# ActiveVisionLab/NeFeS

Hardware: AMD Instinct MI355X
Metric: rays/s (fwd+bwd) at 640x480x(64+128) samples, 8x256 MLP (higher is better)
Workload: dtype f32; 1 GPU; BASELINE configs[1]: 7-Scenes-stairs geometry, 64+128 samples, 8x256 MLP + 16-ch feature head; 640x480, random seed-0 weights, fwd + bwd to the 3x4 pose; parallelism=rows/1

## Files before the change

### include/nefes_hip.h

```cpp
#ifndef NEFES_HIP_H
#define NEFES_HIP_H
#include <stddef.h>
#include <stdint.h>

#ifdef __cplusplus
extern "C" {
#endif

#define NEFES_ABI_VERSION 16

#define NEFES_E_BADARG (-1)
#define NEFES_E_UNSUPPORTED (-2)
#define NEFES_E_BADBLOB (-3)

typedef struct NefesNetDesc {
    int32_t width;
    int32_t feat_dim;
    int32_t has_transient;
    int32_t xyz_encoding;
} NefesNetDesc;
#define NEFES_XYZ_FREQ10 0
#define NEFES_XYZ_EXTERNAL32 1

typedef struct NefesStreamInfo {
    uint64_t slab_off;
    uint32_t n_slabs;
    uint32_t bias_floats;
    uint64_t bias_off;
    uint32_t scale_off;
    uint32_t scale_count;
} NefesStreamInfo;

typedef struct NefesBlobInfo {
    uint64_t total_bytes;
    NefesStreamInfo stream[13];
} NefesBlobInfo;

#define NEFES_COMP_TRANSIENT 1u
#define NEFES_COMP_STATIC_ONLY 2u
#define NEFES_COMP_SIGMA_ONLY 4u
#define NEFES_COMP_WHITE_BKGD 8u
#define NEFES_COMP_FEAT_WEIGHTS_ONLY 16u

#define NEFES_FIELD_SIGMA 0
#define NEFES_FIELD_STATIC 1
#define NEFES_FIELD_FULL 2

int nefes_version(void);

int nefes_blob_info(const NefesNetDesc* desc, NefesBlobInfo* info);
size_t nefes_stream_slab_bytes(const NefesNetDesc* desc, int stream);
int nefes_pack_weights(const NefesNetDesc* desc, const float* const* tensors, int n_tensors, void* blob,
// ... 211 lines not shown
```

### nefes_amd/csrc/field_bwd_h3.hip

```cpp
#if defined(NEFES_TU_PART) && NEFES_TU_PART >= 2 && NEFES_TU_PART % 2 == 0
#define NEFES_SLAB_KIB 16
#define NEFES_ASM_READS_ACC
#define NEFES_ACC_VGPR_FORM
#define NEFES_FENCE_TILES
#else
#define NEFES_SLAB_KIB 32
#if !defined(NEFES_TU_PART) || NEFES_TU_PART == 0 || NEFES_TU_PART == 1 || NEFES_TU_PART == 5
#define H3B_WIDE
#define H3_ACC_READ_ASM
#define NEFES_ASM_READS_ACC
#define NEFES_FENCE_TILES
#define H3_WIDE_ENTRY_FENCE
#else
#define NEFES_H3_WIDE_MIN 99
#endif
#endif
#define NEFES_B_BATCH 2
#define NEFES_B_BATCH_NT8 4
#include "field_common.h"
#include "field_x6.h"
#include "field_h3.h"
#include "hashgrid.h"
#include "../../include/nefes_hip.h"
#define NEFES_XYZ_HASHGRID_FUSED 2
#ifndef H3B_WIDE_LAYERS
#define H3B_WIDE_LAYERS 0x1ff
#endif
#ifndef NEFES_H3B_WG128
#define NEFES_H3B_WG128 2
#endif
#define NEFES_H3B_WG_PER_CU(W) ((W) == 128 ? NEFES_H3B_WG128 : 1)
#define NEFES_H3B_SLOTS 2

struct FieldBwdH3Args {
    const char* stream;
    const int* tab;
    uint32_t n_slabs;
    const float* rays_o;
    const float* rays_d;
    const float* z;
// ... 17 lines not shown
};

template <class Inner>
struct StoringSplitH {
    Inner in;
    float* p;
    float inv;
    __device__ __forceinline__ void stage_a(PairRegs& s, int q, int pp) const {
        in.stage_a(s, q, pp);
        const int e = 8 * q + 2 * pp;
#ifndef NEFES_TRAIN_NO_STORES
        __builtin_nontemporal_store(s.x0 * inv, &p[(e >> 4) * 4096 + nefes_rho(0, e & 15) * 16]);
        __builtin_nontemporal_store(s.x1 * inv, &p[((e + 1) >> 4) * 4096 + nefes_rho(0, (e + 1) & 15) * 16]);
#endif
    }
    __device__ __forceinline__ void stage_b(PairRegs& s) const { in.stage_b(s); }
    template <bool NOP>
    __device__ __forceinline__ void stage_c(Split2& o, int pp, const PairRegs& s) const { in.template stage_c<NOP>(o, pp, s); }
    __device__ __forceinline__ void stage_c1(Split2& o, int pp, const PairRegs& s) const { in.stage_c1(o, pp, s); }
    template <bool NOP>
    __device__ __forceinline__ void stage_c2(Split2& o, int pp, const PairRegs& s) const { in.template stage_c2<NOP>(o, pp, s); }
};
template <bool ON, class Inner>
__device__ __forceinline__ auto wrap_store_h3(const Inner& in, float* p, float inv) {
    if constexpr (ON) return StoringSplitH<Inner>{in, p, inv};
    else return in;
}

template <typename T>
__device__ __forceinline__ T ld_stream(const T* p) {
    return __builtin_nontemporal_load(p);
}

template <int W, int KR16, int ENC, bool HAS_T = true, bool TRAIN = false, bool FH = false>
__global__ __launch_bounds__(256, NEFES_H3B_WG_PER_CU(W)) void field_bwd_h3_kernel(FieldBwdH3Args a) {
    constexpr int NTW = W / 32, NTH = W / 64, HS = W / 2, GS = W / 4;
    constexpr int MW = 8 * (W / 64) + 4 * (W / 128);
    constexpr int WT = (NTW + 1) / 2, WH = (NTH + 1) / 2;
    constexpr int MW_TRUNK = 8 * WT;
    constexpr int NTR = KR16 <= 2 ? 1 : 5;
    constexpr int WIDE_LAYERS = ENC == NEFES_XYZ_HASHGRID_FUSED ? 0 : H3B_WIDE_LAYERS;
    static_assert(KR16 == 2 || KR16 == 9, "head classes of layout.h (nefes_head_kr16 / nefes_head_ntr)");
    const int C3 = 3 + a.C;
    static_assert(MW % 4 == 0, "mask words are staged as 16-byte groups");
    extern __shared__ __attribute__((aligned(16))) char smem[];
    const int lane = threadIdx.x & 63;
    const int wave = __builtin_amdgcn_readfirstlane(threadIdx.x >> 6);
    const int j = lane & 31, h = lane >> 5;
    constexpr int SX = ENC == NEFES_XYZ_HASHGRID_FUSED ? 24 : 8;
    int* tab_i = (int*)(smem + NEFES_H3B_SLOTS * NEFES_SLAB_BYTES + (size_t)4 * (MW + SX) * 256);
    const float* tab_f = (const float*)tab_i;
    if (threadIdx.x < 2 * (HAS_T ? NEFES_H3B_N : NEFES_H3B_N_STATIC)) tab_i[threadIdx.x] = a.tab[threadIdx.x];
    HgGeom* hg_lds = (HgGeom*)(tab_i + 64);
    if constexpr (ENC == NEFES_XYZ_HASHGRID_FUSED) {
        if (threadIdx.x == 0) *hg_lds = a.hg;
    }
    auto wexp = [&](int seg) { return tab_i[nefes_h3_tab_exp(nefes_h3b_seg(HAS_T, seg))]; };
    auto rowb = [&](int seg) { return tab_f[nefes_h3_tab_bound(nefes_h3b_seg(HAS_T, seg))]; };
    StagedRing ring;
    ring.init(a.stream, a.n_slabs, smem, wave, lane);
    const char* ring_lane = smem + lane * 16;
    ring.prime(ring_lane);
    uint32_t* mlds = (uint32_t*)(smem + NEFES_H3B_SLOTS * NEFES_SLAB_BYTES) + wave * ((MW + SX) * 64) + lane * 4;
    auto MASKW = [&](int w) { return mlds[(w >> 2) * 256 + (w & 3)]; };
    float* stash = (float*)mlds;
    auto STASH = [&](int k) -> float& { return stash[((MW + k) >> 2) * 256 + ((MW + k) & 3)]; };

#pragma unroll 1
    for (int tile = blockIdx.x; tile < a.n_tiles; tile += gridDim.x) {
        const long long m_raw = (long long)tile * 128 + wave * 32 + j;
        const bool valid = m_raw < a.M;
        const long long m = valid ? m_raw : a.M - 1;
        const int ray = (int)(m / a.S);
        const int smp = (int)(m - (long long)ray * a.S);
        const size_t chan0 = (size_t)ray * a.R * a.S + smp;

        float in_o[3] = {0.f, 0.f, 0.f}, in_d[3] = {0.f, 0.f, 0.f}, in_z = 0.f, v[3];
        if constexpr (ENC == NEFES_XYZ_EXTERNAL32) {
        } else if (a.pts) {
#pragma unroll
            for (int c = 0; c < 3; ++c) in_o[c] = a.pts[m * 3 + c];
        } else {
            in_z = a.z[m];
#pragma unroll
            for (int c = 0; c < 3; ++c) { in_o[c] = a.rays_o[ray * 3 + c]; in_d[c] = a.rays_d[ray * 3 + c]; }
        }
#pragma unroll
        for (int c = 0; c < 3; ++c) v[c] = a.viewdirs[ray * 3 + c];
        const int cT = C3 + 1;
        float y_th[3] = {0.f, 0.f, 0.f}, g_th[3] = {0.f, 0.f, 0.f}, y_sg, g_sg, dr[8 * KR16];
        if constexpr (HAS_T) {
// ... 163 lines not shown
            load_dg(dgv);
            if constexpr (HAS_T) {
                load_bits(bh, MW_TRUNK + WH, WH);
                mma_run_h3<NTW + 1, GS / 8, 1, true>(ring, ring_lane, wrap_store_h3<TRAIN>(MaskedSplitH<NTH, WH, 0>{T3, bh, pow2i(tau - es3), mt}, gptr(NEFES_TB_T0), pow2i(-es3)), ZeroInit{}, XA);
            }
            load_bits(bh, MW_TRUNK, WH);
#ifdef NEFES_FH_VARIANT_VALU_UPDATE
            if constexpr (FH) {
#pragma unroll
                for (int e = 0; e < 16 * NTH; ++e) G2[e >> 4][e & 15] += dgv[e] * pow2i(es_g2);
                mma_run_h3<NTW + 1, GS / 8, 1, !HAS_T>(ring, ring_lane, MaskedSplitH<NTH, WH, 0>{G2, bh, pow2i(tau - es_g2), mg}, ZeroInit{}, XA);
            } else
#else
            if constexpr (FH)
                mma_run_h3<NTW + 1, GS / 8, 1, !HAS_T>(ring, ring_lane, MaskedAddSplitH<NTH, WH, 0, 16 * NTH>{G2, bh, pow2i(tau - es_g2), mg, dgv, pow2i(es_g2)}, ZeroInit{}, XA);
            else
#endif
            mma_run_h3<NTW + 1, GS / 8, 1, !HAS_T>(ring, ring_lane, wrap_store_h3<TRAIN>(MaskedSplitH<NTH, WH, 0>{G2, bh, pow2i(tau - es_g2), mg}, gptr(NEFES_TB_DIR), pow2i(-es_g2)), ZeroInit{}, XA);
            M = (HAS_T ? rowb(NEFES_H3B_T0) * (pair_max(mt) * pow2i(-es3)) : 0.f) + rowb(NEFES_H3B_DIR) * (pair_max(mg) * pow2i(-es_g2));
        }
        float gv[3];
        {
            float dDv[16], v3[3];
            const float inv = pow2i(-es_dt);
#pragma unroll
            for (int r = 0; r < 16; ++r) dDv[r] = XA[1][r] * inv;
#pragma unroll
            for (int c = 0; c < 3; ++c) v3[c] = STASH(3 + c);
            embed_slots_bwd<NEFES_N_FREQ_DIR>(gv, dDv, v3, h);
            if constexpr (ENC == NEFES_XYZ_HASHGRID_FUSED) {
#pragma unroll
                for (int c = 0; c < 3; ++c) STASH(3 + c) = gv[c];
            }
        }
        int es_b;
        {
            const int ew = wexp(NEFES_H3B_FINAL), tau = tau_of(M, ew);
            float mx = 0.f;
            es_b = tau + ew;
            mma_run_h3<NTW, W / 16, 2, true, 2, (WIDE_LAYERS & 1) != 0>(ring, ring_lane, wrap_store_h3<TRAIN>(IdentSplitH<NTW + 2, 2>{XA, pow2i(tau - es_dt), mx}, gptr(NEFES_TB_FINAL), pow2i(-es_dt)), ZeroInit{}, XB);
            const float dsig = STASH(6);
            float dsg[1];
            dsg[0] = dsig * pow2i(es_b);
#if defined(H3B_WIDE) && defined(H3_WIDE_ENTRY_FENCE)
            mma_run<NTW, 1, 2, false, ((WIDE_LAYERS >> 8) & 1) == 0 || (NTW < NEFES_H3_WIDE_MIN)>(ring, ring_lane, ArrayIn<1>{dsg}, ZeroInit{}, XB);
#else
            mma_run<NTW, 1, 2, false>(ring, ring_lane, ArrayIn<1>{dsg}, ZeroInit{}, XB);
#endif
            M = rowb(NEFES_H3B_FINAL) * (pair_max(mx) * pow2i(-es_dt)) + rowb(NEFES_H3B_SIG) * pair_max(fabsf(dsig));
        }
        int es_a = 0, es_e = 0;
#define NEFES_BWD_LAYER(L, SRC, DST, ES_SRC, ES_DST, NTILES, T0)                                                       \
        {                                                                                                           \
            load_bits(bt, ((L) - 1) * WT, WT);                                                                      \
            const int ew = wexp(NEFES_H3B_L8 + 8 - (L)), tau = tau_of(M, ew);                                       \
            float mx = 0.f;                                                                                         \
            ES_DST = tau + ew;                                                                                      \
            mma_run_h3<NTILES, W / 16, T0, true, 2, ((WIDE_LAYERS >> (L)) & 1) != 0>(ring, ring_lane, wrap_store_h3<TRAIN>(MaskedSplitH<NTW + 2, WT, 2>{SRC, bt, pow2i(tau - ES_SRC), mx}, gptr(NEFES_TB_L1 + (L) - 1), pow2i(-(ES_SRC))), ZeroInit{}, DST); \
            M = rowb(NEFES_H3B_L8 + 8 - (L)) * (pair_max(mx) * pow2i(-(ES_SRC)));                                   \
        }
        NEFES_BWD_LAYER(8, XB, XA, es_b, es_a, NTW, 2)
        NEFES_BWD_LAYER(7, XA, XB, es_a, es_b, NTW, 2)
        NEFES_BWD_LAYER(6, XB, XA, es_b, es_a, NTW, 2)
        NEFES_BWD_LAYER(5, XA, XB, es_a, es_b, NTW + 2, 0)
        es_e = es_b;
        float gx[3] = {0.f, 0.f, 0.f};
        float ge[ENC != NEFES_XYZ_FREQ10 ? NEFES_X_STEPS : 1];
        {
            const float inv = pow2i(-es_e);
            if constexpr (ENC != NEFES_XYZ_FREQ10) {
#pragma unroll
                for (int s_ = 0; s_ < NEFES_X_STEPS; ++s_) ge[s_] = XB[0][s_] * inv;
            } else {
                float dE[32], x3[3];
#pragma unroll
                for (int t = 0; t < 2; ++t)
#pragma unroll
                    for (int r = 0; r < 16; ++r) dE[t * 16 + r] = XB[t][r] * inv;
#pragma unroll
                for (int c = 0; c < 3; ++c) x3[c] = STASH(c);
                embed_slots_bwd<NEFES_N_FREQ_XYZ>(gx, dE, x3, h);
                ge[0] = 0.f;
            }
        }
        NEFES_BWD_LAYER(4, XB, XA, es_b, es_a, NTW, 2)
        NEFES_BWD_LAYER(3, XA, XB, es_a, es_b, NTW, 2)
        NEFES_BWD_LAYER(2, XB, XA, es_b, es_a, NTW, 2)
#undef NEFES_BWD_LAYER
        int es_1;
        {
            load_bits(bt, 0, WT);
            const int ew = wexp(NEFES_H3B_L1), tau = tau_of(M, ew);
            float mx = 0.f;
            es_1 = tau + ew;
            mma_run_h3<2, W / 16, 0, true>(ring, ring_lane, wrap_store_h3<TRAIN>(MaskedSplitH<NTW + 2, WT, 2>{XA, bt, pow2i(tau - es_a), mx}, gptr(NEFES_TB_L1), pow2i(-es_a)), ZeroInit{}, XB);
        }
        const float inv1 = pow2i(-es_1);
        if constexpr (ENC == NEFES_XYZ_HASHGRID_FUSED) {
            float x3[3];
#pragma unroll
            for (int s_ = 0; s_ < NEFES_X_STEPS; ++s_) STASH(8 + s_) = ge[s_] + XB[0][s_] * inv1;
#pragma unroll
            for (int c = 0; c < 3; ++c) x3[c] = STASH(c);
            asm volatile("" : "+v"(x3[0]), "+v"(x3[1]), "+v"(x3[2]));
            hg_encode_slots_bwd(gx, [&](int s_) { return STASH(8 + s_); }, x3, h, *hg_lds, a.hg_table);
#pragma unroll
            for (int c = 0; c < 3; ++c) gv[c] = STASH(3 + c);
        } else if constexpr (ENC == NEFES_XYZ_EXTERNAL32) {
#pragma unroll
            for (int s_ = 0; s_ < NEFES_X_STEPS; ++s_) ge[s_] += XB[0][s_] * inv1;
            if (valid) {
                float* gp = a.g_enc + m * 32 + h;
#pragma unroll
                for (int s_ = 0; s_ < NEFES_X_STEPS; ++s_) gp[2 * s_] = ge[s_];
            }
        } else {
            float dE[32], x3[3], g1[3];
#pragma unroll
            for (int t = 0; t < 2; ++t)
#pragma unroll
                for (int r = 0; r < 16; ++r) dE[t * 16 + r] = XB[t][r] * inv1;
#pragma unroll
            for (int c = 0; c < 3; ++c) x3[c] = STASH(c);
            embed_slots_bwd<NEFES_N_FREQ_XYZ>(g1, dE, x3, h);
#pragma unroll
            for (int c = 0; c < 3; ++c) gx[c] += g1[c];
        }
#pragma unroll
        for (int c = 0; c < 3; ++c) {
            gx[c] += __shfl_xor(gx[c], 32);
            gv[c] += __shfl_xor(gv[c], 32);
        }
        if (valid && h == 0) {
#pragma unroll
            for (int c = 0; c < 3; ++c) {
                if (ENC != NEFES_XYZ_EXTERNAL32) a.g_pts[m * 3 + c] = gx[c];
                a.g_vs[m * 3 + c] = gv[c];
            }
        }
    }
    ring.drain();
}

template <int W, int KR16, int ENC, bool HAS_T = true, bool TRAIN = false, bool FH = false>
static int launch_bwd_h3(const FieldBwdH3Args& a, hipStream_t st) {
    const size_t lds = (size_t)NEFES_H3B_SLOTS * NEFES_SLAB_BYTES
                       + (size_t)4 * (8 * (W / 64) + 4 * (W / 128) + (ENC == NEFES_XYZ_HASHGRID_FUSED ? 24 : 8)) * 256 + 256
                       + (ENC == NEFES_XYZ_HASHGRID_FUSED ? 512 : 0);
    static_assert(sizeof(HgGeom) <= 512 && 2 * NEFES_H3B_N <= 64, "scale table (256 bytes) + the level geometry's LDS slot");
    auto k = field_bwd_h3_kernel<W, KR16, ENC, HAS_T, TRAIN, FH>;
    hipError_t e = hipFuncSetAttribute((const void*)k, hipFuncAttributeMaxDynamicSharedMemorySize, (int)lds);
    if (e != hipSuccess) return (int)e;
    int dev = 0, cus = 256;
    (void)hipGetDevice(&dev);
    (void)hipDeviceGetAttribute(&cus, hipDeviceAttributeMultiprocessorCount, dev);
    const int slots = cus * NEFES_H3B_WG_PER_CU(W);
    int grid = a.n_tiles < slots ? a.n_tiles : slots;
    if (grid < 1) grid = 1;
    hipLaunchKernelGGL(k, dim3(grid), dim3(256), lds, st, a);
    return (int)hipGetLastError();
}

#ifndef NEFES_TU_PART
#define NEFES_TU_PART 0
#endif
enum { BWD_H3_EXT = 0, BWD_H3_FULL, BWD_H3_TRAIN_STATIC, BWD_H3_TRAIN_FULL, BWD_H3_STATIC, BWD_H3_HG, BWD_H3_FH, BWD_H3_TRAIN_EXT_STATIC,
       BWD_H3_TRAIN_EXT_FULL };
int nefes_bwd_h3_launch_part1(int which, const FieldBwdH3Args& a, hipStream_t st);
int nefes_bwd_h3_launch_part2(int which, const FieldBwdH3Args& a, hipStream_t st);
int nefes_bwd_h3_launch_part3(int which, const FieldBwdH3Args& a, hipStream_t st);
int nefes_bwd_h3_launch_part4(int which, const FieldBwdH3Args& a, hipStream_t st);
int nefes_bwd_h3_launch_part5(int which, const FieldBwdH3Args& a, hipStream_t st);
int nefes_bwd_h3_launch_part6(int which, const FieldBwdH3Args& a, hipStream_t st);
int nefes_bwd_h3_launch_part7(int which, const FieldBwdH3Args& a, hipStream_t st);
int nefes_bwd_h3_launch_part8(int which, const FieldBwdH3Args& a, hipStream_t st);

#if NEFES_TU_PART == 1
int nefes_bwd_h3_launch_part1(int which, const FieldBwdH3Args& a, hipStream_t st) {
    if (which == BWD_H3_EXT) return launch_bwd_h3<256, 2, NEFES_XYZ_EXTERNAL32>(a, st);
    if (which == BWD_H3_STATIC) return launch_bwd_h3<256, 2, NEFES_XYZ_FREQ10, false>(a, st);
    if (which == BWD_H3_HG) return launch_bwd_h3<256, 2, NEFES_XYZ_HASHGRID_FUSED>(a, st);
    return NEFES_E_UNSUPPORTED;
}
#elif NEFES_TU_PART == 2
int nefes_bwd_h3_launch_part2(int which, const FieldBwdH3Args& a, hipStream_t st) {
    if (which == BWD_H3_FULL) return launch_bwd_h3<128, 9, NEFES_XYZ_FREQ10>(a, st);
    if (which == BWD_H3_STATIC) return launch_bwd_h3<128, 9, NEFES_XYZ_FREQ10, false>(a, st);
    return NEFES_E_UNSUPPORTED;
}
#elif NEFES_TU_PART == 3
int nefes_bwd_h3_launch_part3(int which, const FieldBwdH3Args& a, hipStream_t st) {
    if (which == BWD_H3_TRAIN_STATIC) return launch_bwd_h3<256, 2, NEFES_XYZ_FREQ10, false, true>(a, st);
    if (which == BWD_H3_TRAIN_FULL) return launch_bwd_h3<256, 2, NEFES_XYZ_FREQ10, true, true>(a, st);
    if (which == BWD_H3_TRAIN_EXT_STATIC) return launch_bwd_h3<256, 2, NEFES_XYZ_EXTERNAL32, false, true>(a, st);
    if (which == BWD_H3_TRAIN_EXT_FULL) return launch_bwd_h3<256, 2, NEFES_XYZ_EXTERNAL32, true, true>(a, st);
    return NEFES_E_UNSUPPORTED;
}
#elif NEFES_TU_PART == 4
int nefes_bwd_h3_launch_part4(int which, const FieldBwdH3Args& a, hipStream_t st) {
    if (which == BWD_H3_TRAIN_STATIC) return launch_bwd_h3<128, 9, NEFES_XYZ_FREQ10, false, true>(a, st);
    if (which == BWD_H3_TRAIN_FULL) return launch_bwd_h3<128, 9, NEFES_XYZ_FREQ10, true, true>(a, st);
    return NEFES_E_UNSUPPORTED;
}
#elif NEFES_TU_PART == 5
int nefes_bwd_h3_launch_part5(int which, const FieldBwdH3Args& a, hipStream_t st) {
    if (which == BWD_H3_FULL) return launch_bwd_h3<256, 9, NEFES_XYZ_FREQ10>(a, st);
    if (which == BWD_H3_STATIC) return launch_bwd_h3<256, 9, NEFES_XYZ_FREQ10, false>(a, st);
    return NEFES_E_UNSUPPORTED;
}
#elif NEFES_TU_PART == 6
int nefes_bwd_h3_launch_part6(int which, const FieldBwdH3Args& a, hipStream_t st) {
    if (which == BWD_H3_FULL) return launch_bwd_h3<128, 2, NEFES_XYZ_FREQ10>(a, st);
    if (which == BWD_H3_STATIC) return launch_bwd_h3<128, 2, NEFES_XYZ_FREQ10, false>(a, st);
    if (which == BWD_H3_FH) return launch_bwd_h3<128, 2, NEFES_XYZ_FREQ10, true, false, true>(a, st);
    return NEFES_E_UNSUPPORTED;
}
#elif NEFES_TU_PART == 7
int nefes_bwd_h3_launch_part7(int which, const FieldBwdH3Args& a, hipStream_t st) {
    if (which == BWD_H3_TRAIN_STATIC) return launch_bwd_h3<256, 9, NEFES_XYZ_FREQ10, false, true>(a, st);
    if (which == BWD_H3_TRAIN_FULL) return launch_bwd_h3<256, 9, NEFES_XYZ_FREQ10, true, true>(a, st);
    return NEFES_E_UNSUPPORTED;
}
#elif NEFES_TU_PART == 8
int nefes_bwd_h3_launch_part8(int which, const FieldBwdH3Args& a, hipStream_t st) {
    if (which == BWD_H3_TRAIN_STATIC) return launch_bwd_h3<128, 2, NEFES_XYZ_FREQ10, false, true>(a, st);
    if (which == BWD_H3_TRAIN_FULL) return launch_bwd_h3<128, 2, NEFES_XYZ_FREQ10, true, true>(a, st);
    return NEFES_E_UNSUPPORTED;
}
#else

extern "C" int nefes_field_bwd_train_h3(const NefesNetDesc* desc, const void* packed, int mode, int N, int S, const float* rays_o,
                                        const float* rays_d, const float* z, const float* viewdirs, const float* raw_t,
                                        const float* g_raw_t, const uint32_t* masks, float* dacts, float* g_pts,
                                        float* g_viewdirs_s, void* stream) {
    if (!desc || !packed || !viewdirs || !raw_t || !g_raw_t || !masks || !dacts || !g_pts || !g_viewdirs_s || N <= 0 || S <= 0)
        return NEFES_E_BADARG;
    if (!(rays_o && rays_d && z)) return NEFES_E_BADARG;
    if (mode != NEFES_FIELD_STATIC && mode != NEFES_FIELD_FULL) return NEFES_E_BADARG;
    const bool full = mode == NEFES_FIELD_FULL;
    if (full && !desc->has_transient) return NEFES_E_UNSUPPORTED;
    const int cls = nefes_head_class(desc->feat_dim);
    if ((desc->width != 256 && desc->width != 128) || cls < 0 || desc->xyz_encoding != NEFES_XYZ_FREQ10) return NEFES_E_UNSUPPORTED;
    NefesBlobInfo info;
    int rc = nefes_blob_info(desc, &info);
    if (rc) return rc;
    const NefesStreamInfo& si = info.stream[full ? NEFES_STREAM_BWD_FULL_H3 : NEFES_STREAM_BWD_STATIC_H3];
    if (si.n_slabs == 0 || si.scale_count < 2 * (uint32_t)(full ? NEFES_H3B_N : NEFES_H3B_N_STATIC)) return NEFES_E_UNSUPPORTED;
    FieldBwdH3Args a;
    a.stream = (const char*)packed + si.slab_off;
    a.tab = (const int*)((const char*)packed + si.bias_off) + si.scale_off;
    a.n_slabs = si.n_slabs;
    a.rays_o = rays_o; a.rays_d = rays_d; a.z = z; a.pts = nullptr; a.viewdirs = viewdirs;
    a.raw_t = raw_t; a.g_raw_t = g_raw_t; a.masks = masks; a.g_pts = g_pts; a.g_enc = nullptr; a.g_vs = g_viewdirs_s;
    a.N = N; a.S = S; a.C = desc->feat_dim; a.R = 3 + a.C + (full ? 6 : 1);
    a.M = (long long)N * S;
    a.n_tiles = (int)((a.M + 127) / 128);
    a.dacts = dacts; a.gout = 0; a.hg_table = nullptr; a.g_gmap = nullptr;
    a.rows = nefes_train_row(desc->width, desc->feat_dim, NEFES_TB_END);
    const int which = full ? BWD_H3_TRAIN_FULL : BWD_H3_TRAIN_STATIC;
    hipStream_t st = (hipStream_t)stream;
    if (desc->width == 256) return cls == 0 ? nefes_bwd_h3_launch_part3(which, a, st) : nefes_bwd_h3_launch_part7(which, a, st);
    return cls == 1 ? nefes_bwd_h3_launch_part4(which, a, st) : nefes_bwd_h3_launch_part8(which, a, st);
}

extern "C" int nefes_field_bwd_train_h3_ext(const NefesNetDesc* desc, const void* packed, int mode, int N, int S, const float* viewdirs,
                                            const float* raw_t, const float* g_raw_t, const uint32_t* masks, float* dacts,
                                            float* g_xyz_enc, float* g_viewdirs_s, void* stream) {
    if (!desc || !packed || !viewdirs || !raw_t || !g_raw_t || !masks || !dacts || !g_xyz_enc || !g_viewdirs_s || N <= 0 || S <= 0)
        return NEFES_E_BADARG;
    if (mode != NEFES_FIELD_STATIC && mode != NEFES_FIELD_FULL) return NEFES_E_BADARG;
    const bool full = mode == NEFES_FIELD_FULL;
    if (full && !desc->has_transient) return NEFES_E_UNSUPPORTED;
    if (desc->width != 256 || nefes_head_class(desc->feat_dim) != 0 || desc->xyz_encoding != NEFES_XYZ_EXTERNAL32) return NEFES_E_UNSUPPORTED;
    NefesBlobInfo info;
    int rc = nefes_blob_info(desc, &info);
    if (rc) return rc;
    const NefesStreamInfo& si = info.stream[full ? NEFES_STREAM_BWD_FULL_H3 : NEFES_STREAM_BWD_STATIC_H3];
    if (si.n_slabs == 0 || si.scale_count < 2 * (uint32_t)(full ? NEFES_H3B_N : NEFES_H3B_N_STATIC)) return NEFES_E_UNSUPPORTED;
    FieldBwdH3Args a;
    a.stream = (const char*)packed + si.slab_off;
    a.tab = (const int*)((const char*)packed + si.bias_off) + si.scale_off;
    a.n_slabs = si.n_slabs;
    a.rays_o = nullptr; a.rays_d = nullptr; a.z = nullptr; a.pts = nullptr; a.viewdirs = viewdirs;
    a.raw_t = raw_t; a.g_raw_t = g_raw_t; a.masks = masks; a.g_pts = nullptr; a.g_enc = g_xyz_enc; a.g_vs = g_viewdirs_s;
    a.N = N; a.S = S; a.C = desc->feat_dim; a.R = 3 + a.C + (full ? 6 : 1);
    a.M = (long long)N * S;
    a.n_tiles = (int)((a.M + 127) / 128);
    a.dacts = dacts; a.gout = 0; a.hg_table = nullptr; a.g_gmap = nullptr;
    a.rows = nefes_train_row(desc->width, desc->feat_dim, NEFES_TB_END);
    return nefes_bwd_h3_launch_part3(full ? BWD_H3_TRAIN_EXT_FULL : BWD_H3_TRAIN_EXT_STATIC, a, (hipStream_t)stream);
}

extern "C" int nefes_field_bwd_static_h3(const NefesNetDesc* desc, const void* packed, int N, int S, const float* rays_o,
                                         const float* rays_d, const float* z, const float* pts, const float* viewdirs,
                                         const float* raw_t, const float* g_raw_t, const uint32_t* masks, float* g_pts,
                                         float* g_viewdirs_s, void* stream) {
    if (!desc || !packed || !viewdirs || !raw_t || !g_raw_t || !masks || !g_pts || !g_viewdirs_s || N <= 0 || S <= 0)
        return NEFES_E_BADARG;
    if (!pts && !(rays_o && rays_d && z)) return NEFES_E_BADARG;
    const int cls = nefes_head_class(desc->feat_dim);
    if ((desc->width != 256 && desc->width != 128) || cls < 0 || desc->xyz_encoding != NEFES_XYZ_FREQ10) return NEFES_E_UNSUPPORTED;
    NefesBlobInfo info;
    int rc = nefes_blob_info(desc, &info);
    if (rc) return rc;
    const NefesStreamInfo& si = info.stream[NEFES_STREAM_BWD_STATIC_H3];
    if (si.n_slabs == 0 || si.scale_count < 2 * (uint32_t)NEFES_H3B_N_STATIC) return NEFES_E_UNSUPPORTED;
    FieldBwdH3Args a;
    a.stream = (const char*)packed + si.slab_off;
    a.tab = (const int*)((const char*)packed + si.bias_off) + si.scale_off;
    a.n_slabs = si.n_slabs;
    a.rays_o = rays_o; a.rays_d = rays_d; a.z = z; a.pts = pts; a.viewdirs = viewdirs;
    a.raw_t = raw_t; a.g_raw_t = g_raw_t; a.masks = masks; a.g_pts = g_pts; a.g_enc = nullptr; a.g_vs = g_viewdirs_s;
    a.N = N; a.S = S; a.C = desc->feat_dim; a.R = 3 + a.C + 1;
    a.M = (long long)N * S;
    a.n_tiles = (int)((a.M + 127) / 128);
    a.dacts = nullptr; a.rows = 0; a.gout = 0; a.hg_table = nullptr; a.g_gmap = nullptr;
    hipStream_t st = (hipStream_t)stream;
    if (desc->width == 256) return cls == 0 ? nefes_bwd_h3_launch_part1(BWD_H3_STATIC, a, st) : nefes_bwd_h3_launch_part5(BWD_H3_STATIC, a, st);
    return cls == 1 ? nefes_bwd_h3_launch_part2(BWD_H3_STATIC, a, st) : nefes_bwd_h3_launch_part6(BWD_H3_STATIC, a, st);
}

static int field_bwd_h3_impl(const NefesNetDesc* desc, const void* packed, int N, int S, const float* rays_o,
                                  const float* rays_d, const float* z, const float* pts, const float* viewdirs,
                                  const float* raw_t, const float* g_raw_t, const uint32_t* masks, float* g_pts,
                                  float* g_xyz_enc, float* g_viewdirs_s, void* stream, const NefesHashGridDesc* grid, const float* table,
                                  bool fh = false, const float* g_gmap = nullptr) {
    if (!desc || !packed || !viewdirs || !raw_t || !g_raw_t || !masks || !g_viewdirs_s || N <= 0 || S <= 0)
        return NEFES_E_BADARG;
    const bool ext = desc->xyz_encoding == NEFES_XYZ_EXTERNAL32;
    const bool fused_grid = ext && table != nullptr;
    if (fused_grid ? !(g_pts && grid && rays_o && rays_d && z) : (ext ? !g_xyz_enc : (!g_pts || (!pts && !(rays_o && rays_d && z))))) return NEFES_E_BADARG;
    if (!desc->has_transient) return NEFES_E_UNSUPPORTED;
    NefesBlobInfo info;
    int rc = nefes_blob_info(desc, &info);
    if (rc) return rc;
    const NefesStreamInfo& si = info.stream[NEFES_STREAM_BWD_FULL_H3];
    if (si.n_slabs == 0 || si.scale_count < 2 * NEFES_H3B_N) return NEFES_E_UNSUPPORTED;
    FieldBwdH3Args a;
    a.stream = (const char*)packed + si.slab_off;
    a.tab = (const int*)((const char*)packed + si.bias_off) + si.scale_off;
    a.n_slabs = si.n_slabs;
    a.rays_o = rays_o; a.rays_d = rays_d; a.z = z; a.pts = pts; a.viewdirs = viewdirs;
    a.raw_t = raw_t; a.g_raw_t = g_raw_t; a.masks = masks; a.g_pts = g_pts; a.g_enc = g_xyz_enc; a.g_vs = g_viewdirs_s;
    a.N = N; a.S = S; a.C = desc->feat_dim; a.R = 3 + a.C + 6;
    a.gout = 0; a.g_gmap = g_gmap;
    if (fh) {
        if (desc->feat_dim != 0 || desc->width != 128 || ext) return NEFES_E_UNSUPPORTED;
        a.gout = desc->width / 2;
        a.C = a.gout + 1;
        a.R = 3 + a.C + 6;
    }
    a.M = (long long)N * S;
    a.n_tiles = (int)((a.M + 127) / 128);
    a.dacts = nullptr; a.rows = 0;
    a.hg_table = (const float2*)table;
    if (fused_grid) {
        rc = hg_geometry(grid, &a.hg, nullptr);
        if (rc) return rc;
        if (a.hg.n_levels != 16) return NEFES_E_UNSUPPORTED;
    }
    hipStream_t st = (hipStream_t)stream;
    const int cls = nefes_head_class(desc->feat_dim);
    if (cls < 0) return NEFES_E_UNSUPPORTED;
    if (fh) return nefes_bwd_h3_launch_part6(BWD_H3_FH, a, st);
    if (desc->width == 256 && fused_grid) return cls == 0 ? nefes_bwd_h3_launch_part1(BWD_H3_HG, a, st) : NEFES_E_UNSUPPORTED;
    if (desc->width == 256 && ext) return cls == 0 ? nefes_bwd_h3_launch_part1(BWD_H3_EXT, a, st) : NEFES_E_UNSUPPORTED;
    if (desc->width == 256) return cls == 0 ? launch_bwd_h3<256, 2, NEFES_XYZ_FREQ10>(a, st) : nefes_bwd_h3_launch_part5(BWD_H3_FULL, a, st);
    if (desc->width == 128 && !ext) return cls == 1 ? nefes_bwd_h3_launch_part2(BWD_H3_FULL, a, st) : nefes_bwd_h3_launch_part6(BWD_H3_FULL, a, st);
    return NEFES_E_UNSUPPORTED;
}

extern "C" int nefes_field_bwd_h3(const NefesNetDesc* desc, const void* packed, int N, int S, const float* rays_o,
                                  const float* rays_d, const float* z, const float* pts, const float* viewdirs,
                                  const float* raw_t, const float* g_raw_t, const uint32_t* masks, float* g_pts,
                                  float* g_xyz_enc, float* g_viewdirs_s, void* stream) {
    return field_bwd_h3_impl(desc, packed, N, S, rays_o, rays_d, z, pts, viewdirs, raw_t, g_raw_t, masks, g_pts, g_xyz_enc, g_viewdirs_s, stream,
                             nullptr, nullptr);
}

extern "C" int nefes_field_bwd_h3_fh(const NefesNetDesc* desc, const void* packed, int N, int S, const float* rays_o, const float* rays_d,
                                     const float* z, const float* viewdirs, const float* raw_t, const float* g_raw_t, const float* g_gmap,
                                     const uint32_t* masks, float* g_pts, float* g_viewdirs_s, void* stream) {
    if (!rays_o || !rays_d || !z) return NEFES_E_BADARG;
    return field_bwd_h3_impl(desc, packed, N, S, rays_o, rays_d, z, nullptr, viewdirs, raw_t, g_raw_t, masks, g_pts, nullptr, g_viewdirs_s, stream,
                             nullptr, nullptr, true, g_gmap);
}

extern "C" int nefes_field_bwd_h3_hashgrid(const NefesNetDesc* desc, const void* packed, const NefesHashGridDesc* grid,
                                           const float* table, int N, int S, const float* rays_o, const float* rays_d, const float* z,
                                           const float* viewdirs, const float* raw_t, const float* g_raw_t, const uint32_t* masks,
                                           float* g_pts, float* g_viewdirs_s, void* stream) {
    if (!desc || desc->xyz_encoding != NEFES_XYZ_EXTERNAL32 || !grid || !table) return NEFES_E_BADARG;
    return field_bwd_h3_impl(desc, packed, N, S, rays_o, rays_d, z, nullptr, viewdirs, raw_t, g_raw_t, masks, g_pts, nullptr, g_viewdirs_s, stream,
                             grid, table);
}
#endif
```

### nefes_amd/csrc/field_fwd_h3.hip

```cpp
#if defined(NEFES_TU_PART) && NEFES_TU_PART >= 2 && NEFES_TU_PART % 2 == 0
#define NEFES_TU_W128
#define NEFES_SLAB_KIB 16
#else
#define NEFES_SLAB_KIB 32
#endif
#include <stdlib.h>
#if defined(NEFES_TU_W128) || !defined(H3_NO_ACC_READ_ASM)
#define NEFES_ASM_READS_ACC
#define NEFES_FENCE_TILES
#endif
#if defined(NEFES_TU_W128)
#define NEFES_ACC_VGPR_FORM
#endif

#ifndef NEFES_FWD_CONSUMER_BIAS
#define NEFES_FWD_CONSUMER_BIAS 1
#endif
#include "field_common.h"
#include "../../include/nefes_hip.h"

#include "field_x6.h"
#include "hashgrid.h"
#define NEFES_XYZ_HASHGRID_FUSED 2
#if !defined(NEFES_TU_W128) && !defined(H3_NO_ACC_READ_ASM)
// ... 9 lines not shown
    const float* rays_o;
    const float* rays_d;
    const float* z;
    const float* pts;
    const float* xyz_enc;
    const float* viewdirs;
    float* raw_t;
    uint32_t* masks;
    int N, S, R, C;
    long long M;
    int n_tiles;
    uint32_t s_magic, s_shift;
    float* acts;
    int rows;
    int z_row;
    const float2* hg_table;
    HgGeom hg;
    int gout;
};

template <int NT, int T0, int NX>
__device__ __forceinline__ void train_save_h3(float* tile_base, uint32_t voff, int row0, const f32x16 (&X)[NX], float inv) {
    float* p = tile_base + (size_t)(row0 >> 5) * 4096 + voff;
#pragma unroll
    for (int t = 0; t < NT; ++t)
#pragma unroll
        for (int r = 0; r < 16; ++r) {
#ifndef NEFES_TRAIN_NO_STORES
            __builtin_nontemporal_store(X[T0 + t][r] * inv, &p[t * 4096 + nefes_rho(0, r) * 16]);
#endif
        }
}

template <int MODE, int ENC, int W = 256, int NTR = 1, bool TRAIN = false, bool FH = false>
__global__ __launch_bounds__(256, W == 128 ? 2 : 1) void field_fwd_h3_kernel(FieldFwdH3Args a) {
    static_assert(NEFES_SLAB_KIB == (W == 128 ? NEFES_H3_FWD_SLAB_KIB_128 : NEFES_H3_FWD_SLAB_KIB), "ring slab size != the packer's for this width");
    constexpr int NTW = W / 32, NTH = W / 64;
    constexpr int ES = ENC != NEFES_XYZ_FREQ10 ? NEFES_X_STEPS : NEFES_E_STEPS;
    constexpr int MW = 8 * (W / 64) + 4 * (W / 128), WT = (NTW + 1) / 2, WH = (NTH + 1) / 2;
    constexpr int NSEG = MODE == NEFES_FIELD_SIGMA ? NEFES_H3F_SIG + 1 : (MODE == NEFES_FIELD_STATIC ? NEFES_H3F_N_STATIC : NEFES_H3F_N);
    extern __shared__ __attribute__((aligned(16))) char smem[];
    char* ring_base = smem;
    float* bias_lds = (float*)(smem + NEFES_H3_SLOTS * NEFES_SLAB_BYTES);
    float* e_lds = bias_lds + ((a.bias_floats + 63) / 64) * 64 + (threadIdx.x >> 6) * (ES * 64) + (threadIdx.x & 63);
    const int lane = threadIdx.x & 63;
    const int wave = __builtin_amdgcn_readfirstlane(threadIdx.x >> 6);
    const int j = lane & 31, h = lane >> 5;
    for (uint32_t i = threadIdx.x; i < a.bias_floats; i += 256) bias_lds[i] = a.bias[i];
    HgGeom* hg_lds = (HgGeom*)(bias_lds + ((a.bias_floats + 63) / 64) * 64 + 4 * ES * 64);
    if constexpr (ENC == NEFES_XYZ_HASHGRID_FUSED) {
        if (threadIdx.x == 0) *hg_lds = a.hg;
    }
    StagedRing ring;
    ring.init(a.stream, a.n_slabs, ring_base, wave, lane);
    const char* ring_lane = ring_base + lane * 16;
    const char* bias_half = (const char*)bias_lds + 16 * h;
    const int* tab_i = (const int*)(bias_lds + a.scale_off);
    const float* tab_f = bias_lds + a.scale_off;
    auto wexp = [&](int seg) { return tab_i[nefes_h3_tab_exp(seg)]; };
    auto rowb = [&](int seg) { return tab_f[nefes_h3_tab_bound(seg)]; };
    auto bmax = [&](int blk) { return tab_f[nefes_h3_tab_bias(NSEG, blk)]; };
    ring.prime(ring_lane);
    constexpr int B_SIG = 8 * W, B_FINAL = B_SIG + 32, B_DIR = B_FINAL + W, B_RGB = B_DIR + W / 2,
                  B_T0 = B_RGB + 32 * NTR, B_T1 = B_T0 + W / 2, B_T2 = B_T1 + W / 2, B_TH = B_T2 + W / 2;
#pragma unroll 1
    for (int tile = blockIdx.x; tile < a.n_tiles; tile += gridDim.x) {
        auto locate = [&](uint32_t& m, uint32_t& ray, uint32_t& smp) {
            const uint32_t m_raw = (uint32_t)tile * 128u + (uint32_t)(wave * 32 + j);
            const bool ok = m_raw < (uint32_t)a.M;
            m = ok ? m_raw : (uint32_t)a.M - 1u;
            ray = a.s_magic ? __umulhi(m, a.s_magic) >> a.s_shift : m;
            smp = m - ray * (uint32_t)a.S;
            return ok;
        };
        uint32_t m, ray, smp;
        locate(m, ray, smp);
        float in_o[3] = {0.f, 0.f, 0.f}, in_d[3] = {0.f, 0.f, 0.f}, in_z = 0.f;
        float E[ES];
        if constexpr (ENC == NEFES_XYZ_EXTERNAL32) {
#pragma unroll
            for (int s = 0; s < ES; ++s) E[s] = a.xyz_enc[(size_t)m * 32 + 2 * s + h];
        } else if (ENC != NEFES_XYZ_HASHGRID_FUSED && a.pts) {
#pragma unroll
            for (int c = 0; c < 3; ++c) in_o[c] = a.pts[(size_t)m * 3 + c];
        } else {
            in_z = a.z[a.z_row ? smp : m];
#pragma unroll
            for (int c = 0; c < 3; ++c) { in_o[c] = a.rays_o[ray * 3 + c]; in_d[c] = a.rays_d[ray * 3 + c]; }
        }
        float mE;
        if constexpr (ENC == NEFES_XYZ_EXTERNAL32) {
            mE = pair_max(array_max(E));
        } else if constexpr (ENC == NEFES_XYZ_HASHGRID_FUSED) {
            float x[3];
#pragma unroll
            for (int c = 0; c < 3; ++c) x[c] = add_rn(in_o[c], mul_rn(in_d[c], in_z));
// ... 63 lines not shown
                const int ch = (MODE == NEFES_FIELD_SIGMA) ? 0 : 3 + a.C;
                __builtin_nontemporal_store(softplus_ref(sg[0][0] * pow2i(-es)), &col[(size_t)ch * a.S]);
            }
        };
        int es_a, es_b = 0;
        float M;
        {
            const int tau = tau_of(mE, wexp(NEFES_H3F_L1));
            es_a = tau + wexp(NEFES_H3F_L1);
            if constexpr (CB) mma_run_h3<NTW, ES / 8, 0, true>(ring, ring_lane, LdsSplitH{e_lds, pow2i(tau)}, ZeroInit{}, A);
            else mma_run_h3<NTW, ES / 8, 0, true>(ring, ring_lane, LdsSplitH{e_lds, pow2i(tau)}, bias_at(0, es_a), A);
            M = rowb(NEFES_H3F_L1) * mE + bmax(NEFES_H3BB_L1);
            save_trunk(1, A, es_a);
        }
#define NEFES_FWD_EVEN_LAYER(L1_, SEG1_)                                                                                       \
        clear_bits();                                                                                                          \
        {                                                                                                                      \
            const int ew = wexp(SEG1_), tau = tau_of(M, ew);                                                                   \
            const float rb_ = rowb(SEG1_), bm_ = bmax((L1_) - 1);           \
            float mx = 0.f;                                                                                                    \
            if constexpr (CB) {                                                                                                \
                const char* bps = bias_half + ((L1_) - 2) * W * 4;                           \
                nbias = ReluBiasSplitH<CAP, NTW, WT>::prime(bps);                                                              \
                mma_run_h3<NTW, W / 16, 0, true>(ring, ring_lane, ReluBiasSplitH<CAP, NTW, WT>{A, bits, pow2i(tau - es_a), mx, bps, pow2i(es_a), nbias}, \
                                                 ZeroInit{}, B);                                                               \
            } else                                                                                                             \
            mma_run_h3<NTW, W / 16, 0, true>(ring, ring_lane, ReluSplitH<CAP, NTW, WT>{A, bits, pow2i(tau - es_a), mx},        \
                                             bias_at(((L1_) - 1) * W, tau + ew), B);                                           \
            M = rb_ * (pair_max(mx) * pow2i(-es_a)) + bm_;                                                                     \
            es_b = tau + ew;                                                                                                   \
            save_trunk(L1_, B, es_b);                                                                                          \
        }                                                                                                                      \
        put_masks(bits, WT);
        constexpr int NPAIRS = MODE == NEFES_FIELD_SIGMA ? 3 : 4;
#pragma unroll 1
        for (int p = 0; p < NPAIRS; ++p) {
            const int l1 = 2 + 2 * p, l2 = l1 + 1;
            const int seg1 = l1 <= 5 ? l1 - 1 : l1;
            const int seg2 = l2 <= 5 ? l2 - 1 : (l2 <= 8 ? l2 : NEFES_H3F_FINAL);
            NEFES_FWD_EVEN_LAYER(l1, seg1)
            clear_bits();
            {
                const int ew = wexp(seg2);
                const int tau = tau_of(p == 1 ? fmaxf(M, mE) : M, ew);
                if (p == 3) sigma_head(B, es_b, tau_of(M, wexp(NEFES_H3F_SIG)));
                const float rb_ = rowb(seg2), bm_ = bmax(l2 <= 8 ? l2 - 1 : NEFES_H3BB_FINAL);
                const float rbe_ = p == 1 ? rowb(NEFES_H3F_L5E) : 0.f;
                float mx = 0.f;
                if constexpr (CB) {
                    const char* bps = bias_half + (l1 - 1) * W * 4;
                    nbias = ReluBiasSplitH<CAP, NTW, WT>::prime(bps);
                    const ReluBiasSplitH<CAP, NTW, WT> src{B, bits, pow2i(tau - es_b), mx, bps, pow2i(es_b), nbias};
                    mma_run_h3<NTW, W / 16, 0, true>(ring, ring_lane, src, ZeroInit{}, A);
                } else
                mma_run_h3<NTW, W / 16, 0, true>(ring, ring_lane, ReluSplitH<CAP, NTW, WT>{B, bits, pow2i(tau - es_b), mx},
                                                 bias_at(l2 <= 8 ? (l2 - 1) * W : B_FINAL, tau + ew), A);
                if (p == 1) mma_run_h3<NTW, ES / 8, 0, false>(ring, ring_lane, LdsSplitH{e_lds, pow2i(tau)}, ZeroInit{}, A);
                M = rb_ * (pair_max(mx) * pow2i(-es_b)) + (p == 1 ? rbe_ * mE : 0.f) + bm_;
                es_a = tau + ew;
                save_trunk(l2, A, es_a);
            }
            put_masks(bits, WT);
        }
        if constexpr (MODE == NEFES_FIELD_SIGMA) { NEFES_FWD_EVEN_LAYER(8, NEFES_H3F_L8) }
#undef NEFES_FWD_EVEN_LAYER
        if constexpr (MODE == NEFES_FIELD_SIGMA) sigma_head(B, es_b, tau_of(M, wexp(NEFES_H3F_SIG)));
        if constexpr (MODE != NEFES_FIELD_SIGMA) {
            constexpr bool FULL = MODE == NEFES_FIELD_FULL;
            constexpr int NDT = FULL ? 2 * NTH : NTH;
            float v[3];
            {
                uint32_t mm, rr, ss;
                locate(mm, rr, ss);
#pragma unroll
                for (int c = 0; c < 3; ++c) v[c] = a.viewdirs[(size_t)rr * 3 + c];
            }
            float Dv[16];
            {
                float d14[NEFES_D_STEPS];
                embed_slots<NEFES_N_FREQ_DIR>(d14, v, h);
#pragma unroll
                for (int s = 0; s < 16; ++s) Dv[s] = s < NEFES_D_STEPS ? d14[s] : 0.f;
            }
            if constexpr (TRAIN) {
                float* pd = act_tile + (size_t)(nefes_train_row(W, 0, NEFES_TB_DV) >> 5) * 4096 + emb_off;
#pragma unroll
                for (int s = 0; s < NEFES_D_STEPS; ++s) __builtin_nontemporal_store(Dv[s], &pd[2 * s * 16]);
            }
            f32x16 dt[NDT];
            uint32_t bits2[WH];
            auto clear2 = [&]() {
#pragma unroll
                for (int w = 0; w < WH; ++w) bits2[w] = 0u;
            };
            struct Bias2 {
                BiasInitScaled a, b;
                __device__ __forceinline__ f32x16 operator()(int t) const { return t < NTH ? a(t) : b(t - NTH); }
            };
            int es_dt;
            {
                const int ew = wexp(NEFES_H3F_DT_H);
                const float mD = pair_max(array_max(Dv));
                const int tau = tau_of(fmaxf(M, mD), ew);
                float mx = 0.f;
                es_dt = tau + ew;
                if constexpr (CB) {
                    const char* bpf = bias_half + B_FINAL * 4;
                    nbias = ReluBiasSplitH<false, 1, 1>::prime(bpf);
                    const IdentBiasSplitH<NTW> srcf{A, pow2i(tau - es_a), mx, bpf, pow2i(es_a), nbias};
                    if constexpr (FULL) mma_run_h3<NDT, W / 16, 0, true>(ring, ring_lane, srcf, Bias2{bias_at(B_DIR, es_dt), bias_at(B_T0, es_dt)}, dt);
                    else mma_run_h3<NDT, W / 16, 0, true>(ring, ring_lane, srcf, bias_at(B_DIR, es_dt), dt);
                } else if constexpr (FULL)
                    mma_run_h3<NDT, W / 16, 0, true>(ring, ring_lane, IdentSplitH<NTW, 0>{A, pow2i(tau - es_a), mx},
                                                     Bias2{bias_at(B_DIR, es_dt), bias_at(B_T0, es_dt)}, dt);
                else
                    mma_run_h3<NDT, W / 16, 0, true>(ring, ring_lane, IdentSplitH<NTW, 0>{A, pow2i(tau - es_a), mx}, bias_at(B_DIR, es_dt), dt);
                mma_run_h3<NDT, 2, 0, false>(ring, ring_lane, ArraySplitH<16>{Dv, pow2i(tau)}, ZeroInit{}, dt);
                M = rowb(NEFES_H3F_DT_H) * (pair_max(mx) * pow2i(-es_a)) + rowb(NEFES_H3F_DT_D) * mD
                    + (FULL ? fmaxf(bmax(NEFES_H3BB_DIR), bmax(NEFES_H3BB_T0)) : bmax(NEFES_H3BB_DIR));
                if constexpr (TRAIN) {
                    train_save_h3<NTH, 0>(act_tile, act_voff, nefes_train_row(W, 0, NEFES_TB_DIR), dt, pow2i(-es_dt));
                    if constexpr (FULL) train_save_h3<NTH, NTH>(act_tile, act_voff, nefes_train_row(W, 0, NEFES_TB_T0), dt, pow2i(-es_dt));
                }
            }
            if constexpr (FH) {
                float* col = raw_col();
                if (col) {
                    int S_g = a.S;
                    asm volatile("" : "+s"(S_g));
                    const float inv = pow2i(-es_dt);
                    float* pg = col + (size_t)(3 + 4 * h) * S_g;
#pragma unroll
                    for (int t = 0; t < NTH; ++t)
// ... 101 lines not shown
    constexpr int ES_ = ENC != NEFES_XYZ_FREQ10 ? NEFES_X_STEPS : NEFES_E_STEPS;
    const size_t lds = (size_t)NEFES_H3_SLOTS * NEFES_SLAB_BYTES + ((a.bias_floats + 63) / 64) * 256 + (size_t)4 * ES_ * 64 * 4
                       + (ENC == NEFES_XYZ_HASHGRID_FUSED ? 512 : 0);
    static_assert(sizeof(HgGeom) <= 512, "the level geometry's LDS slot");
    auto k = field_fwd_h3_kernel<MODE, ENC, W, NTR, TRAIN, FH>;
    hipError_t e = hipFuncSetAttribute((const void*)k, hipFuncAttributeMaxDynamicSharedMemorySize, (int)lds);
    if (e != hipSuccess) return (int)e;
    int dev = 0, cus = 256;
    (void)hipGetDevice(&dev);
    (void)hipDeviceGetAttribute(&cus, hipDeviceAttributeMultiprocessorCount, dev);
    const int per_cu = W == 128 ? 2 : 1;
    int grid = a.n_tiles < cus * per_cu ? a.n_tiles : cus * per_cu;
    if (const char* cap = getenv("NEFES_DEBUG_MAX_GRID")) {
        const int c = atoi(cap);
        if (c > 0 && c < grid) grid = c;
    }
    hipLaunchKernelGGL(k, dim3(grid), dim3(256), lds, st, a);
    return (int)hipGetLastError();
}

#ifndef NEFES_TU_PART
#define NEFES_TU_PART 0
#endif
enum { H3_EXT_SIGMA = 0, H3_EXT_FULL, H3_SIGMA, H3_FULL, H3_TRAIN_STATIC, H3_TRAIN_FULL, H3_STATIC, H3_HG_SIGMA, H3_HG_FULL, H3_FH_FULL,
       H3_TRAIN_EXT_STATIC, H3_TRAIN_EXT_FULL };
int nefes_fwd_h3_launch_part1(int which, const FieldFwdH3Args& a, hipStream_t st);
int nefes_fwd_h3_launch_part2(int which, const FieldFwdH3Args& a, hipStream_t st);
int nefes_fwd_h3_launch_part3(int which, const FieldFwdH3Args& a, hipStream_t st);
int nefes_fwd_h3_launch_part4(int which, const FieldFwdH3Args& a, hipStream_t st);
int nefes_fwd_h3_launch_part5(int which, const FieldFwdH3Args& a, hipStream_t st);
int nefes_fwd_h3_launch_part6(int which, const FieldFwdH3Args& a, hipStream_t st);
int nefes_fwd_h3_launch_part7(int which, const FieldFwdH3Args& a, hipStream_t st);
int nefes_fwd_h3_launch_part8(int which, const FieldFwdH3Args& a, hipStream_t st);


#if NEFES_TU_PART == 1
int nefes_fwd_h3_launch_part1(int which, const FieldFwdH3Args& a, hipStream_t st) {
    switch (which) {
        case H3_EXT_SIGMA: return launch_h3<NEFES_FIELD_SIGMA, NEFES_XYZ_EXTERNAL32>(a, st);
        case H3_EXT_FULL: return launch_h3<NEFES_FIELD_FULL, NEFES_XYZ_EXTERNAL32>(a, st);
        case H3_STATIC: return launch_h3<NEFES_FIELD_STATIC, NEFES_XYZ_FREQ10, 256, 1>(a, st);
        case H3_HG_SIGMA: return launch_h3<NEFES_FIELD_SIGMA, NEFES_XYZ_HASHGRID_FUSED>(a, st);
        case H3_HG_FULL: return launch_h3<NEFES_FIELD_FULL, NEFES_XYZ_HASHGRID_FUSED>(a, st);
    }
    return NEFES_E_UNSUPPORTED;
}
#elif NEFES_TU_PART == 2
int nefes_fwd_h3_launch_part2(int which, const FieldFwdH3Args& a, hipStream_t st) {
    switch (which) {
        case H3_SIGMA: return launch_h3<NEFES_FIELD_SIGMA, NEFES_XYZ_FREQ10, 128, 5>(a, st);
        case H3_FULL: return launch_h3<NEFES_FIELD_FULL, NEFES_XYZ_FREQ10, 128, 5>(a, st);
        case H3_STATIC: return launch_h3<NEFES_FIELD_STATIC, NEFES_XYZ_FREQ10, 128, 5>(a, st);
    }
    return NEFES_E_UNSUPPORTED;
}
#elif NEFES_TU_PART == 3
int nefes_fwd_h3_launch_part3(int which, const FieldFwdH3Args& a, hipStream_t st) {
    switch (which) {
        case H3_TRAIN_STATIC: return launch_h3<NEFES_FIELD_STATIC, NEFES_XYZ_FREQ10, 256, 1, true>(a, st);
        case H3_TRAIN_FULL: return launch_h3<NEFES_FIELD_FULL, NEFES_XYZ_FREQ10, 256, 1, true>(a, st);
        case H3_TRAIN_EXT_STATIC: return launch_h3<NEFES_FIELD_STATIC, NEFES_XYZ_EXTERNAL32, 256, 1, true>(a, st);
        case H3_TRAIN_EXT_FULL: return launch_h3<NEFES_FIELD_FULL, NEFES_XYZ_EXTERNAL32, 256, 1, true>(a, st);
    }
    return NEFES_E_UNSUPPORTED;
}
#elif NEFES_TU_PART == 4
// ... 1 lines not shown
    switch (which) {
        case H3_TRAIN_STATIC: return launch_h3<NEFES_FIELD_STATIC, NEFES_XYZ_FREQ10, 128, 5, true>(a, st);
        case H3_TRAIN_FULL: return launch_h3<NEFES_FIELD_FULL, NEFES_XYZ_FREQ10, 128, 5, true>(a, st);
    }
    return NEFES_E_UNSUPPORTED;
}
#elif NEFES_TU_PART == 5
int nefes_fwd_h3_launch_part5(int which, const FieldFwdH3Args& a, hipStream_t st) {
    if (which == H3_FULL) return launch_h3<NEFES_FIELD_FULL, NEFES_XYZ_FREQ10, 256, 5>(a, st);
    if (which == H3_STATIC) return launch_h3<NEFES_FIELD_STATIC, NEFES_XYZ_FREQ10, 256, 5>(a, st);
    return NEFES_E_UNSUPPORTED;
}
#elif NEFES_TU_PART == 6
int nefes_fwd_h3_launch_part6(int which, const FieldFwdH3Args& a, hipStream_t st) {
    if (which == H3_FULL) return launch_h3<NEFES_FIELD_FULL, NEFES_XYZ_FREQ10, 128, 1>(a, st);
    if (which == H3_STATIC) return launch_h3<NEFES_FIELD_STATIC, NEFES_XYZ_FREQ10, 128, 1>(a, st);
    if (which == H3_FH_FULL) return launch_h3<NEFES_FIELD_FULL, NEFES_XYZ_FREQ10, 128, 1, false, true>(a, st);
    return NEFES_E_UNSUPPORTED;
}
#elif NEFES_TU_PART == 7
int nefes_fwd_h3_launch_part7(int which, const FieldFwdH3Args& a, hipStream_t st) {
    switch (which) {
        case H3_TRAIN_STATIC: return launch_h3<NEFES_FIELD_STATIC, NEFES_XYZ_FREQ10, 256, 5, true>(a, st);
        case H3_TRAIN_FULL: return launch_h3<NEFES_FIELD_FULL, NEFES_XYZ_FREQ10, 256, 5, true>(a, st);
    }
    return NEFES_E_UNSUPPORTED;
}
#elif NEFES_TU_PART == 8
int nefes_fwd_h3_launch_part8(int which, const FieldFwdH3Args& a, hipStream_t st) {
    switch (which) {
        case H3_TRAIN_STATIC: return launch_h3<NEFES_FIELD_STATIC, NEFES_XYZ_FREQ10, 128, 1, true>(a, st);
        case H3_TRAIN_FULL: return launch_h3<NEFES_FIELD_FULL, NEFES_XYZ_FREQ10, 128, 1, true>(a, st);
    }
    return NEFES_E_UNSUPPORTED;
}
#else

extern "C" int nefes_field_fwd_train_h3(const NefesNetDesc* desc, const void* packed, int mode, int N, int S, const float* rays_o,
                                        const float* rays_d, const float* z, const float* pts, const float* viewdirs,
                                        float* raw_t, float* acts, uint32_t* masks, void* stream) {
    if (!desc || !packed || !raw_t || !acts || !viewdirs || N <= 0 || S <= 0) return NEFES_E_BADARG;
    if (!pts && !(rays_o && rays_d && z)) return NEFES_E_BADARG;
    if (mode != NEFES_FIELD_STATIC && mode != NEFES_FIELD_FULL) return NEFES_E_UNSUPPORTED;
    if (mode == NEFES_FIELD_FULL && !desc->has_transient) return NEFES_E_BADARG;
    const int cls = nefes_head_class(desc->feat_dim);
    if ((desc->width != 256 && desc->width != 128) || cls < 0 || desc->xyz_encoding != NEFES_XYZ_FREQ10) return NEFES_E_UNSUPPORTED;
    NefesBlobInfo info;
    int rc = nefes_blob_info(desc, &info);
    if (rc) return rc;
    const NefesStreamInfo& si = info.stream[mode == NEFES_FIELD_STATIC ? NEFES_STREAM_FWD_STATIC_H3 : NEFES_STREAM_FWD_FULL_H3];
    if (si.n_slabs == 0) return NEFES_E_UNSUPPORTED;
    FieldFwdH3Args a;
    a.stream = (const char*)packed + si.slab_off;
    a.bias = (const float*)((const char*)packed + si.bias_off);
    a.n_slabs = si.n_slabs; a.bias_floats = si.bias_floats; a.scale_off = si.scale_off;
    a.rays_o = rays_o; a.rays_d = rays_d; a.z = z; a.pts = pts; a.xyz_enc = nullptr; a.viewdirs = viewdirs; a.raw_t = raw_t; a.masks = masks;
    a.N = N; a.S = S; a.C = desc->feat_dim; a.R = 3 + a.C + (mode == NEFES_FIELD_STATIC ? 1 : 6);
    a.M = (long long)N * S;
    if (a.M >= (1ll << 31) - 256) return NEFES_E_UNSUPPORTED;
    a.n_tiles = (int)((a.M + 127) / 128);
    a.acts = acts;
    a.rows = nefes_train_row(desc->width, desc->feat_dim, NEFES_TB_END);
    a.z_row = 0; a.gout = 0; a.hg_table = nullptr;
    magic_div((uint32_t)S, a.s_magic, a.s_shift);
    const int which = mode == NEFES_FIELD_STATIC ? H3_TRAIN_STATIC : H3_TRAIN_FULL;
    hipStream_t st = (hipStream_t)stream;
    if (desc->width == 256) return cls == 0 ? nefes_fwd_h3_launch_part3(which, a, st) : nefes_fwd_h3_launch_part7(which, a, st);
    return cls == 1 ? nefes_fwd_h3_launch_part4(which, a, st) : nefes_fwd_h3_launch_part8(which, a, st);
}

extern "C" int nefes_field_fwd_train_h3_ext(const NefesNetDesc* desc, const void* packed, int mode, int N, int S, const float* xyz_enc,
                                            const float* viewdirs, float* raw_t, float* acts, uint32_t* masks, void* stream) {
    if (!desc || !packed || !xyz_enc || !raw_t || !acts || !viewdirs || N <= 0 || S <= 0) return NEFES_E_BADARG;
    if (mode != NEFES_FIELD_STATIC && mode != NEFES_FIELD_FULL) return NEFES_E_UNSUPPORTED;
    if (mode == NEFES_FIELD_FULL && !desc->has_transient) return NEFES_E_BADARG;
    if (desc->width != 256 || nefes_head_class(desc->feat_dim) != 0 || desc->xyz_encoding != NEFES_XYZ_EXTERNAL32) return NEFES_E_UNSUPPORTED;
    NefesBlobInfo info;
    int rc = nefes_blob_info(desc, &info);
    if (rc) return rc;
    const NefesStreamInfo& si = info.stream[mode == NEFES_FIELD_STATIC ? NEFES_STREAM_FWD_STATIC_H3 : NEFES_STREAM_FWD_FULL_H3];
    if (si.n_slabs == 0) return NEFES_E_UNSUPPORTED;
    FieldFwdH3Args a;
    a.stream = (const char*)packed + si.slab_off;
    a.bias = (const float*)((const char*)packed + si.bias_off);
    a.n_slabs = si.n_slabs; a.bias_floats = si.bias_floats; a.scale_off = si.scale_off;
    a.rays_o = nullptr; a.rays_d = nullptr; a.z = nullptr; a.pts = nullptr; a.xyz_enc = xyz_enc; a.viewdirs = viewdirs; a.raw_t = raw_t;
    a.masks = masks;
    a.N = N; a.S = S; a.C = desc->feat_dim; a.R = 3 + a.C + (mode == NEFES_FIELD_STATIC ? 1 : 6);
    a.M = (long long)N * S;
    if (a.M >= (1ll << 31) - 256) return NEFES_E_UNSUPPORTED;
    a.n_tiles = (int)((a.M + 127) / 128);
    a.acts = acts;
    a.rows = nefes_train_row(desc->width, desc->feat_dim, NEFES_TB_END);
    a.z_row = 0; a.gout = 0; a.hg_table = nullptr;
    magic_div((uint32_t)S, a.s_magic, a.s_shift);
    return nefes_fwd_h3_launch_part3(mode == NEFES_FIELD_STATIC ? H3_TRAIN_EXT_STATIC : H3_TRAIN_EXT_FULL, a, (hipStream_t)stream);
}

static int field_fwd_h3_impl(const NefesNetDesc* desc, const void* packed, int mode, int N, int S, const float* rays_o,
                             const float* rays_d, const float* z, int z_row, const float* pts, const float* xyz_enc,
                             const float* viewdirs, float* raw_t, uint32_t* masks, void* stream,
                             const NefesHashGridDesc* grid = nullptr, const float* table = nullptr, bool fh = false) {
    if (!desc || !packed || !raw_t || N <= 0 || S <= 0) return NEFES_E_BADARG;
    const bool ext = desc->xyz_encoding == NEFES_XYZ_EXTERNAL32;
    const bool fused_grid = ext && table != nullptr;
    if (fused_grid ? !(rays_o && rays_d && z && grid) : (ext ? !xyz_enc : (!pts && !(rays_o && rays_d && z)))) return NEFES_E_BADARG;
    if (mode != NEFES_FIELD_SIGMA && mode != NEFES_FIELD_FULL && mode != NEFES_FIELD_STATIC) return NEFES_E_UNSUPPORTED;
    if (mode == NEFES_FIELD_FULL && (!viewdirs || !desc->has_transient)) return NEFES_E_BADARG;
    if (mode == NEFES_FIELD_STATIC && (!viewdirs || ext)) return ext ? NEFES_E_UNSUPPORTED : NEFES_E_BADARG;
    const int cls = nefes_head_class(desc->feat_dim);
    const bool big = desc->width == 256, small = desc->width == 128 && !ext;
    if (!(big || small) || cls < 0 || (ext && cls != 0) || (desc->xyz_encoding != NEFES_XYZ_FREQ10 && !ext)) return NEFES_E_UNSUPPORTED;
    NefesBlobInfo info;
    int rc = nefes_blob_info(desc, &info);
    if (rc) return rc;
    const NefesStreamInfo& si = info.stream[mode == NEFES_FIELD_SIGMA ? NEFES_STREAM_FWD_SIGMA_H3
                                            : (mode == NEFES_FIELD_STATIC ? NEFES_STREAM_FWD_STATIC_H3 : NEFES_STREAM_FWD_FULL_H3)];
    if (si.n_slabs == 0) return NEFES_E_UNSUPPORTED;
    FieldFwdH3Args a;
    a.stream = (const char*)packed + si.slab_off;
    a.bias = (const float*)((const char*)packed + si.bias_off);
    a.n_slabs = si.n_slabs; a.bias_floats = si.bias_floats; a.scale_off = si.scale_off;
    a.rays_o = rays_o; a.rays_d = rays_d; a.z = z; a.pts = pts; a.xyz_enc = xyz_enc; a.viewdirs = viewdirs; a.raw_t = raw_t; a.masks = masks;
    a.acts = nullptr; a.rows = 0; a.z_row = z_row;
    a.hg_table = (const float2*)table;
    if (fused_grid) {
        rc = hg_geometry(grid, &a.hg, nullptr);
        if (rc) return rc;
        if (a.hg.n_levels != 16) return NEFES_E_UNSUPPORTED;
    }
    a.N = N; a.S = S; a.C = desc->feat_dim; a.R = mode == NEFES_FIELD_SIGMA ? 1 : 3 + a.C + (mode == NEFES_FIELD_STATIC ? 1 : 6);
    a.gout = 0;
    if (fh) {
        if (desc->feat_dim != 0 || desc->width != 128 || ext || mode != NEFES_FIELD_FULL) return NEFES_E_UNSUPPORTED;
        a.gout = desc->width / 2;
        a.C = a.gout + 1;
        a.R = 3 + a.C + 6;
    }
    a.M = (long long)N * S;
    if (a.M >= (1ll << 31) - 256) return NEFES_E_UNSUPPORTED;
    a.n_tiles = (int)((a.M + 127) / 128);
    magic_div((uint32_t)S, a.s_magic, a.s_shift);
    hipStream_t st = (hipStream_t)stream;
    if (fh) return nefes_fwd_h3_launch_part6(H3_FH_FULL, a, st);
    if (mode == NEFES_FIELD_STATIC) {
        if (big) return cls == 0 ? nefes_fwd_h3_launch_part1(H3_STATIC, a, st) : nefes_fwd_h3_launch_part5(H3_STATIC, a, st);
        return cls == 1 ? nefes_fwd_h3_launch_part2(H3_STATIC, a, st) : nefes_fwd_h3_launch_part6(H3_STATIC, a, st);
    }
    if (fused_grid) return nefes_fwd_h3_launch_part1(mode == NEFES_FIELD_SIGMA ? H3_HG_SIGMA : H3_HG_FULL, a, st);
    if (ext) return nefes_fwd_h3_launch_part1(mode == NEFES_FIELD_SIGMA ? H3_EXT_SIGMA : H3_EXT_FULL, a, st);
    if (small) {
        if (mode == NEFES_FIELD_SIGMA) return nefes_fwd_h3_launch_part2(H3_SIGMA, a, st);
        return cls == 1 ? nefes_fwd_h3_launch_part2(H3_FULL, a, st) : nefes_fwd_h3_launch_part6(H3_FULL, a, st);
    }
    if (mode == NEFES_FIELD_SIGMA) return launch_h3<NEFES_FIELD_SIGMA, NEFES_XYZ_FREQ10>(a, st);
    return cls == 0 ? launch_h3<NEFES_FIELD_FULL, NEFES_XYZ_FREQ10>(a, st) : nefes_fwd_h3_launch_part5(H3_FULL, a, st);
}

extern "C" int nefes_field_fwd_h3(const NefesNetDesc* desc, const void* packed, int mode, int N, int S, const float* rays_o,
                                  const float* rays_d, const float* z, const float* pts, const float* xyz_enc,
                                  const float* viewdirs, float* raw_t, uint32_t* masks, void* stream) {
    return field_fwd_h3_impl(desc, packed, mode, N, S, rays_o, rays_d, z, 0, pts, xyz_enc, viewdirs, raw_t, masks, stream);
}

extern "C" int nefes_field_fwd_h3_hashgrid(const NefesNetDesc* desc, const void* packed, const NefesHashGridDesc* grid,
                                           const float* table, int mode, int N, int S, const float* rays_o, const float* rays_d,
                                           const float* z, int z_is_row, const float* viewdirs, float* raw_t, uint32_t* masks,
                                           void* stream) {
    if (!desc || desc->xyz_encoding != NEFES_XYZ_EXTERNAL32 || !grid || !table) return NEFES_E_BADARG;
    return field_fwd_h3_impl(desc, packed, mode, N, S, rays_o, rays_d, z, z_is_row ? 1 : 0, nullptr, nullptr, viewdirs, raw_t, masks, stream,
                             grid, table);
}

extern "C" int nefes_field_fwd_h3_fh(const NefesNetDesc* desc, const void* packed, int mode, int N, int S, const float* rays_o,
                                     const float* rays_d, const float* z, const float* viewdirs, float* raw_t, uint32_t* masks,
                                     void* stream) {
    if (!rays_o || !rays_d || !z) return NEFES_E_BADARG;
    return field_fwd_h3_impl(desc, packed, mode, N, S, rays_o, rays_d, z, 0, nullptr, nullptr, viewdirs, raw_t, masks, stream, nullptr, nullptr, true);
}

extern "C" int nefes_field_fwd_h3_zrow(const NefesNetDesc* desc, const void* packed, int mode, int N, int S, const float* rays_o,
                                       const float* rays_d, const float* z_row, const float* viewdirs, float* raw_t, uint32_t* masks,
                                       void* stream) {
    if (!rays_o || !rays_d || !z_row) return NEFES_E_BADARG;
    if (desc && desc->xyz_encoding != NEFES_XYZ_FREQ10) return NEFES_E_UNSUPPORTED;
    return field_fwd_h3_impl(desc, packed, mode, N, S, rays_o, rays_d, z_row, 1, nullptr, nullptr, viewdirs, raw_t, masks, stream);
}
#endif
// ... 1 lines not shown
```

### nefes_amd/csrc/layout.h

```cpp
#pragma once
#include <stdint.h>

#if defined(__HIP__)
#define NEFES_HD __host__ __device__ inline __attribute__((always_inline))
#else
#define NEFES_HD inline
#endif

#ifndef NEFES_FWD_SLAB_KIB
#define NEFES_FWD_SLAB_KIB 32
#endif
#ifndef NEFES_BWD_SLAB_KIB
#define NEFES_BWD_SLAB_KIB 32
#endif
#define NEFES_FRAGS_OF_KIB(kib) ((kib) * 4)
#define NEFES_SLAB_BYTES (NEFES_SLAB_KIB * 1024)
#define NEFES_SLAB_FRAGS NEFES_FRAGS_OF_KIB(NEFES_SLAB_KIB)
#define NEFES_SLAB_PIECES (NEFES_SLAB_BYTES / 4096)
#define NEFES_RING_SLOTS (128 / NEFES_FWD_SLAB_KIB)
#define NEFES_BWD_SLOTS (96 / NEFES_BWD_SLAB_KIB)
#define NEFES_N_FREQ_XYZ 10
#define NEFES_N_FREQ_DIR 4
#define NEFES_E_STEPS 32
#define NEFES_D_STEPS 14
// ... 24 lines not shown
       NEFES_STREAM_FWD_SIGMA_H3 = 8, NEFES_STREAM_FWD_FULL_H3 = 9, NEFES_STREAM_BWD_FULL_H3 = 10,
       NEFES_STREAM_FWD_STATIC_H3 = 11, NEFES_STREAM_BWD_STATIC_H3 = 12,
       NEFES_N_STREAMS = 13 };
#define NEFES_X6_SLAB_KIB 48
#define NEFES_H3_FWD_SLAB_KIB 32
#define NEFES_H3_FWD_SLAB_KIB_128 16
#define NEFES_H3_BWD_SLAB_KIB 32
#define NEFES_H3_BWD_SLAB_KIB_128 16
#define NEFES_H3_TARGET_EXP 14
NEFES_HD int nefes_stream_slab_kib(int stream, int width) {
    if (stream == NEFES_STREAM_BWD_FULL || stream == NEFES_STREAM_BWD_FULL_X6 || stream == NEFES_STREAM_BWD_STATIC) return NEFES_BWD_SLAB_KIB;
    if (stream == NEFES_STREAM_BWD_FULL_H3 || stream == NEFES_STREAM_BWD_STATIC_H3) return width == 128 ? NEFES_H3_BWD_SLAB_KIB_128 : NEFES_H3_BWD_SLAB_KIB;
    if (stream == NEFES_STREAM_FWD_SIGMA_H3 || stream == NEFES_STREAM_FWD_FULL_H3 || stream == NEFES_STREAM_FWD_STATIC_H3)
        return width == 128 ? NEFES_H3_FWD_SLAB_KIB_128 : NEFES_H3_FWD_SLAB_KIB;
    return stream >= NEFES_STREAM_FWD_SIGMA_X6 ? NEFES_X6_SLAB_KIB : NEFES_FWD_SLAB_KIB;
}
#define NEFES_PACK_KEEP 0xffffffffu
#define NEFES_BLOB_HEADER_BYTES 512

enum { NEFES_H3F_L1 = 0, NEFES_H3F_L2, NEFES_H3F_L3, NEFES_H3F_L4, NEFES_H3F_L5H, NEFES_H3F_L5E, NEFES_H3F_L6, NEFES_H3F_L7,
       NEFES_H3F_L8, NEFES_H3F_SIG, NEFES_H3F_FINAL, NEFES_H3F_DT_H, NEFES_H3F_DT_D, NEFES_H3F_RGB, NEFES_H3F_T1, NEFES_H3F_T2,
       NEFES_H3F_TH, NEFES_H3F_N };
NEFES_HD int nefes_h3_tab_exp(int seg) { return 2 * seg; }
NEFES_HD int nefes_h3_tab_bound(int seg) { return 2 * seg + 1; }
NEFES_HD int nefes_h3_tab_bias(int n_segs, int block) { return 2 * n_segs + block; }
enum { NEFES_H3BB_L1 = 0, NEFES_H3BB_SIG = 8, NEFES_H3BB_FINAL, NEFES_H3BB_DIR, NEFES_H3BB_RGB, NEFES_H3BB_T0, NEFES_H3BB_T1,
       NEFES_H3BB_T2, NEFES_H3BB_TH };
enum { NEFES_H3B_RGB = 0, NEFES_H3B_TH, NEFES_H3B_T2, NEFES_H3B_T1, NEFES_H3B_T0, NEFES_H3B_DIR, NEFES_H3B_FINAL, NEFES_H3B_SIG,
       NEFES_H3B_L8, NEFES_H3B_L7, NEFES_H3B_L6, NEFES_H3B_L5, NEFES_H3B_L4, NEFES_H3B_L3, NEFES_H3B_L2, NEFES_H3B_L1,
       NEFES_H3B_N };
#define NEFES_H3F_N_STATIC (NEFES_H3F_RGB + 1)
#define NEFES_H3B_N_STATIC (NEFES_H3B_N - 4)
NEFES_HD int nefes_h3b_seg(int has_transient, int seg) { return (has_transient || seg == NEFES_H3B_RGB) ? seg : seg - 4; }

NEFES_HD int nefes_mask_words(int W) { return 8 * (W / 64) + 4 * (W / 128); }

enum { NEFES_TB_E = 0, NEFES_TB_DV = 1, NEFES_TB_L1 = 2 , NEFES_TB_FINAL = 10, NEFES_TB_DIR = 11,
       NEFES_TB_T0 = 12, NEFES_TB_T1 = 13, NEFES_TB_T2 = 14, NEFES_TB_RGB = 15, NEFES_TB_SIG = 16, NEFES_TB_TH = 17,
       NEFES_TB_END = 18 };
NEFES_HD size_t nefes_train_off(int row, int sample) {
    return ((size_t)(row >> 5) * 8 + (size_t)(sample >> 4)) * 512 + (size_t)(row & 31) * 16 + (size_t)(sample & 15);
}
NEFES_HD uint32_t nefes_train_lane_off(int wave, int j, int h) { return (uint32_t)(((wave * 32 + j) >> 4) * 512 + 4 * h * 16 + (j & 15)); }
NEFES_HD int nefes_train_row(int W, int C, int block) {
    const int ntr = nefes_head_ntr(C);
    int r = 0;
    if (block == NEFES_TB_E) return r;
    r += 2 * NEFES_E_STEPS;
    if (block == NEFES_TB_DV) return r;
    r += 32;
    if (block >= NEFES_TB_L1 && block <= NEFES_TB_FINAL) return r + (block - NEFES_TB_L1) * W;
    r += 9 * W;
    if (block >= NEFES_TB_DIR && block <= NEFES_TB_T2) return r + (block - NEFES_TB_DIR) * (W / 2);
    r += 4 * (W / 2);
    if (block == NEFES_TB_RGB) return r;
    r += 32 * ntr;
    if (block == NEFES_TB_SIG) return r;
    r += 32;
    if (block == NEFES_TB_TH) return r;
    return r + 32;
}
```

### nefes_amd/csrc/pack.cpp

```cpp
#include <math.h>
#include <string.h>

#include <vector>

#include "../../include/nefes_hip.h"
#include "layout.h"

namespace {

enum { L_XYZ1 = 0, L_FINAL = 8, L_DIR = 9, L_SIGMA = 10, L_RGB = 11, L_T0 = 12, L_T1 = 13, L_T2 = 14, L_TSIGMA = 15,
       L_TRGB = 16, L_TBETA = 17 };

struct Seg {
    int nt = 0, ks = 0;
    std::vector<int> kidx;
    std::vector<int> ridx;
    const float* W = nullptr;
    int ld = 0;
    bool transposed = false;
    bool x6 = false;
    bool h3 = false;
    int wexp = 0;
    float at(int s, int t, int lane) const {
        const int i = lane & 31, h = lane >> 5;
// ... 58 lines not shown
    if (x >= 0x47800000u) return (uint16_t)(sign | (x > 0x7f800000u ? 0x7e00u : 0x7c00u));
    if (x < 0x38800000u) {
        float a;
        memcpy(&a, &x, 4);
        return (uint16_t)(sign | (uint32_t)nearbyintf(a * 16777216.0f));
    }
    const uint32_t mant = x & 0x7fffffu, e = (x >> 23) - 112u;
    uint32_t h = (e << 10) | (mant >> 13);
    const uint32_t rem = mant & 0x1fffu;
    if (rem > 0x1000u || (rem == 0x1000u && (h & 1u))) ++h;
    return (uint16_t)(sign | h);
}
static float f16_value(uint16_t h) {
    const int e = (h >> 10) & 31, m = h & 1023;
    float v = e == 0 ? ldexpf((float)m, -24) : ldexpf((float)(1024 + m), e - 25);
    return (h & 0x8000u) ? -v : v;
}
static void split_f16x2(float w, int e, uint16_t (&part)[2]) {
    const float y = ldexpf(w, e);
    part[0] = rne_f16(y);
    part[1] = rne_f16(y - f16_value(part[0]));
}
static int scale_exp(float amax) {
    if (!(amax > 0.f) || !isfinite(amax)) return 0;
    int e;
    frexpf(amax, &e);
    int r = NEFES_H3_TARGET_EXP + 1 - e;
    return r < -60 ? -60 : (r > 60 ? 60 : r);
}

struct BiasBlk {
    const float* b;
    std::vector<int> ridx;
};

struct Stream {
    std::vector<Seg> segs;
    std::vector<BiasBlk> bias;
    bool h3 = false;
    int n_slabs(int slab_frags) const {
        int n = 0;
        for (auto& s : segs) n += s.slabs(slab_frags);
        return n;
    }
    int bias_only() const {
        int n = 0;
        for (auto& b : bias) n += (int)b.ridx.size();
        return n;
    }
    int scale_count() const { return h3 ? (2 * (int)segs.size() + (int)bias.size() + 3) / 4 * 4 : 0; }
    int bias_floats() const { return bias_only() + scale_count(); }
};

std::vector<int> rows_natural(int nt, int limit) {
    std::vector<int> r(nt * 32);
    for (int i = 0; i < nt * 32; ++i) r[i] = i < limit ? i : -1;
    return r;
}
std::vector<int> k_natural(int ks, int base) {
    std::vector<int> k(ks * 2);
    for (int s = 0; s < ks; ++s)
        for (int h = 0; h < 2; ++h) k[s * 2 + h] = base + nefes_nat_slot(s, h);
    return k;
}
std::vector<int> k_emb(int L, int ks, int base) {
    std::vector<int> k(ks * 2);
// ... 1 lines not shown
        for (int h = 0; h < 2; ++h) {
            const int e = nefes_emb_slot(L, s, h);
            k[s * 2 + h] = e < 0 ? -1 : base + e;
        }
    return k;
}
std::vector<int> k_compact(int ks, int limit) {
    std::vector<int> k(ks * 2);
    for (int i = 0; i < ks * 2; ++i) k[i] = i < limit ? i : -1;
    return k;
}
std::vector<int> rows_emb(int L, int ntiles, int base) {
    std::vector<int> r(ntiles * 32);
    for (int t = 0; t < ntiles; ++t)
        for (int i = 0; i < 32; ++i) {
            const int e = nefes_emb_slot(L, 16 * t + nefes_row_reg(i), nefes_row_half(i));
            r[t * 32 + i] = e < 0 ? -1 : base + e;
        }
    return r;
}
std::vector<int> concat(std::vector<int> a, const std::vector<int>& b) {
    a.insert(a.end(), b.begin(), b.end());
    return a;
}

struct Net {
    int W, W2, C, NTW, NTH, NTR;
    bool transient;
    bool ext;
    int in_xyz, e_steps;
    const float* const* t;
    std::vector<float> th_w, th_b;
    std::vector<float> dt_w;
    const float* w(int l) const { return t[2 * l]; }
    const float* b(int l) const { return t[2 * l + 1]; }
};

Seg seg(int nt, int ks, std::vector<int> kidx, std::vector<int> ridx, const float* W, int ld, bool tr = false) {
    Seg s;
    s.nt = nt; s.ks = ks; s.kidx = std::move(kidx); s.ridx = std::move(ridx); s.W = W; s.ld = ld; s.transposed = tr;
    return s;
}

std::vector<int> k_xyz(const Net& n, int base) {
    return n.ext ? [&] { auto k = k_compact(n.e_steps, n.in_xyz); for (auto& v : k) if (v >= 0) v += base; return k; }()
                 : k_emb(10, n.e_steps, base);
}
std::vector<int> rows_xyz(const Net& n, int base) {
    if (!n.ext) return rows_emb(10, 2, base);
    std::vector<int> r(64, -1);
    for (int i = 0; i < 32; ++i) r[i] = base + 2 * nefes_row_reg(i) + nefes_row_half(i);
    return r;
}

static void mark(Seg& s, int kind) {
    s.x6 = kind != 0;
    s.h3 = kind == 2;
}

void add_trunk(const Net& n, Stream& st, int x6 = 0) {
    const int W = n.W, NT = n.NTW;
    for (int l = 0; l < 8; ++l) {
        if (l == 0) {
            st.segs.push_back(seg(NT, n.e_steps, k_xyz(n, 0), rows_natural(NT, W), n.w(0), n.in_xyz));
            mark(st.segs.back(), x6);
        } else if (l == 4) {
            st.segs.push_back(seg(NT, W / 2, k_natural(W / 2, n.in_xyz), rows_natural(NT, W), n.w(4), n.in_xyz + W));
            mark(st.segs.back(), x6);
            st.segs.push_back(seg(NT, n.e_steps, k_xyz(n, 0), rows_natural(NT, W), n.w(4), n.in_xyz + W));
            mark(st.segs.back(), x6);
        } else {
            st.segs.push_back(seg(NT, W / 2, k_natural(W / 2, 0), rows_natural(NT, W), n.w(l), W));
            mark(st.segs.back(), x6);
        }
        st.bias.push_back({n.b(l), rows_natural(NT, W)});
    }
    st.segs.push_back(seg(1, W / 2, k_natural(W / 2, 0), rows_natural(1, 1), n.w(L_SIGMA), W));
    mark(st.segs.back(), x6);
    st.bias.push_back({n.b(L_SIGMA), rows_natural(1, 1)});
}

void add_static_head(const Net& n, Stream& st, int x6 = 0) {
    const int W = n.W, W2 = n.W2;
    st.segs.push_back(seg(n.NTW, W / 2, k_natural(W / 2, 0), rows_natural(n.NTW, W), n.w(L_FINAL), W));
    mark(st.segs.back(), x6);
    st.bias.push_back({n.b(L_FINAL), rows_natural(n.NTW, W)});
    st.segs.push_back(seg(n.NTH, W / 2, k_natural(W / 2, 0), rows_natural(n.NTH, W2), n.w(L_DIR), W + 27));
    mark(st.segs.back(), x6);
    st.segs.push_back(seg(n.NTH, NEFES_D_STEPS, k_emb(4, NEFES_D_STEPS, W), rows_natural(n.NTH, W2), n.w(L_DIR), W + 27));
    st.bias.push_back({n.b(L_DIR), rows_natural(n.NTH, W2)});
    st.segs.push_back(seg(n.NTR, W2 / 2, k_natural(W2 / 2, 0), rows_natural(n.NTR, 3 + n.C), n.w(L_RGB), W2));
    st.bias.push_back({n.b(L_RGB), rows_natural(n.NTR, 3 + n.C)});
}

void add_static_head_h3(const Net& n, Stream& st) {
    const int W = n.W, W2 = n.W2;
    st.segs.push_back(seg(n.NTW, W / 2, k_natural(W / 2, 0), rows_natural(n.NTW, W), n.w(L_FINAL), W));
    mark(st.segs.back(), 2);
    st.bias.push_back({n.b(L_FINAL), rows_natural(n.NTW, W)});
    st.segs.push_back(seg(n.NTH, W / 2, k_natural(W / 2, 0), rows_natural(n.NTH, W2), n.w(L_DIR), W + 27));
    mark(st.segs.back(), 2);
    st.segs.push_back(seg(n.NTH, 16, k_emb(4, 16, W), rows_natural(n.NTH, W2), n.w(L_DIR), W + 27));
    mark(st.segs.back(), 2);
    st.bias.push_back({n.b(L_DIR), rows_natural(n.NTH, W2)});
    st.segs.push_back(seg(n.NTR, W2 / 2, k_natural(W2 / 2, 0), rows_natural(n.NTR, 3 + n.C), n.w(L_RGB), W2));
    mark(st.segs.back(), 2);
    st.bias.push_back({n.b(L_RGB), rows_natural(n.NTR, 3 + n.C)});
}

void add_heads_x6(const Net& n, Stream& st, int kind = 1) {
    const int W = n.W, W2 = n.W2;
    st.segs.push_back(seg(n.NTW, W / 2, k_natural(W / 2, 0), rows_natural(n.NTW, W), n.w(L_FINAL), W));
    mark(st.segs.back(), kind);
    st.bias.push_back({n.b(L_FINAL), rows_natural(n.NTW, W)});
    st.segs.push_back(seg(2 * n.NTH, W / 2, k_natural(W / 2, 0), rows_natural(2 * n.NTH, 2 * W2), n.dt_w.data(), W + 27));
    mark(st.segs.back(), kind);
    st.segs.push_back(seg(2 * n.NTH, 16, k_emb(4, 16, W), rows_natural(2 * n.NTH, 2 * W2), n.dt_w.data(), W + 27));
    mark(st.segs.back(), kind);
    st.bias.push_back({n.b(L_DIR), rows_natural(n.NTH, W2)});
    st.segs.push_back(seg(n.NTR, W2 / 2, k_natural(W2 / 2, 0), rows_natural(n.NTR, 3 + n.C), n.w(L_RGB), W2));
    mark(st.segs.back(), kind);
    st.bias.push_back({n.b(L_RGB), rows_natural(n.NTR, 3 + n.C)});
    st.bias.push_back({n.b(L_T0), rows_natural(n.NTH, W2)});
    for (int l = L_T1; l <= L_T2; ++l) {
        st.segs.push_back(seg(n.NTH, W2 / 2, k_natural(W2 / 2, 0), rows_natural(n.NTH, W2), n.w(l), W2));
        mark(st.segs.back(), kind);
        st.bias.push_back({n.b(l), rows_natural(n.NTH, W2)});
    }
    st.segs.push_back(seg(1, W2 / 2, k_natural(W2 / 2, 0), rows_natural(1, 5), n.th_w.data(), W2));
    mark(st.segs.back(), kind);
    st.bias.push_back({n.th_b.data(), rows_natural(1, 5)});
}

void add_transient_head(const Net& n, Stream& st, int x6 = 0) {
    const int W = n.W, W2 = n.W2;
    st.segs.push_back(seg(n.NTH, W / 2, k_natural(W / 2, 0), rows_natural(n.NTH, W2), n.w(L_T0), W + 27));
    st.segs.push_back(seg(n.NTH, NEFES_D_STEPS, k_emb(4, NEFES_D_STEPS, W), rows_natural(n.NTH, W2), n.w(L_T0), W + 27));
    st.bias.push_back({n.b(L_T0), rows_natural(n.NTH, W2)});
    for (int l = L_T1; l <= L_T2; ++l) {
        st.segs.push_back(seg(n.NTH, W2 / 2, k_natural(W2 / 2, 0), rows_natural(n.NTH, W2), n.w(l), W2));
        mark(st.segs.back(), x6);
        st.bias.push_back({n.b(l), rows_natural(n.NTH, W2)});
    }
    st.segs.push_back(seg(1, W2 / 2, k_natural(W2 / 2, 0), rows_natural(1, 5), n.th_w.data(), W2));
    st.bias.push_back({n.th_b.data(), rows_natural(1, 5)});
}

void add_backward(const Net& n, Stream& st, int x6 = 0, bool transient = true) {
    const int W = n.W, W2 = n.W2, NTW = n.NTW, NTH = n.NTH;
    if (x6 == 2) {
        const int ks = 8 * nefes_head_kr16(n.C);
        std::vector<int> k = k_natural(ks, 0);
        for (auto& v : k) if (v >= 3 + n.C) v = -1;
        st.segs.push_back(seg(NTH, ks, k, rows_natural(NTH, W2), n.w(L_RGB), W2, true));
        mark(st.segs.back(), 2);
    } else {
        const int kr = (3 + n.C + 1) / 2;
        st.segs.push_back(seg(NTH, kr, k_compact(kr, 3 + n.C), rows_natural(NTH, W2), n.w(L_RGB), W2, true));
    }
    if (transient) {
    st.segs.push_back(seg(NTH, 3, k_compact(3, 5), rows_natural(NTH, W2), n.th_w.data(), W2, true));
    st.segs.push_back(seg(NTH, W2 / 2, k_natural(W2 / 2, 0), rows_natural(NTH, W2), n.w(L_T2), W2, true));
    mark(st.segs.back(), x6);
    st.segs.push_back(seg(NTH, W2 / 2, k_natural(W2 / 2, 0), rows_natural(NTH, W2), n.w(L_T1), W2, true));
    mark(st.segs.back(), x6);
    }
    std::vector<int> rows_fd = concat(rows_emb(4, 1, W), rows_natural(NTW, W));
    if (transient) {
        st.segs.push_back(seg(NTW + 1, W2 / 2, k_natural(W2 / 2, 0), rows_fd, n.w(L_T0), W + 27, true));
        mark(st.segs.back(), x6);
    }
    st.segs.push_back(seg(NTW + 1, W2 / 2, k_natural(W2 / 2, 0), rows_fd, n.w(L_DIR), W + 27, true));
    mark(st.segs.back(), x6);
    st.segs.push_back(seg(NTW, W / 2, k_natural(W / 2, 0), rows_natural(NTW, W), n.w(L_FINAL), W, true));
    mark(st.segs.back(), x6);
    st.segs.push_back(seg(NTW, 1, k_compact(1, 1), rows_natural(NTW, W), n.w(L_SIGMA), W, true));
    for (int l = 7; l >= 0; --l) {
        if (l == 4) {
            const std::vector<int> re = rows_xyz(n, 0);
            std::vector<int> rows = concat(re, rows_natural(NTW, W));
            for (int i = (int)re.size(); i < (int)rows.size(); ++i) rows[i] += n.in_xyz;
            st.segs.push_back(seg(NTW + (int)re.size() / 32, W / 2, k_natural(W / 2, 0), rows, n.w(4), n.in_xyz + W, true));
            mark(st.segs.back(), x6);
        } else if (l == 0) {
            const std::vector<int> re = rows_xyz(n, 0);
            st.segs.push_back(seg((int)re.size() / 32, W / 2, k_natural(W / 2, 0), re, n.w(0), n.in_xyz, true));
            mark(st.segs.back(), x6);
        } else {
            st.segs.push_back(seg(NTW, W / 2, k_natural(W / 2, 0), rows_natural(NTW, W), n.w(l), W, true));
            mark(st.segs.back(), x6);
        }
    }
}

static size_t matrix_elems(const Net& n, const float* Wm) {
    if (Wm == n.th_w.data()) return n.th_w.size();
    if (Wm == n.dt_w.data()) return n.dt_w.size();
    const int W = n.W, W2 = n.W2;
    for (int l = 0; l < 18; ++l) {
        if (n.t[2 * l] != Wm) continue;
        if (l < 8) return (size_t)W * (l == 0 ? n.in_xyz : (l == 4 ? n.in_xyz + W : W));
        if (l == L_FINAL) return (size_t)W * W;
        if (l == L_DIR || l == L_T0) return (size_t)W2 * (W + 27);
        if (l == L_SIGMA) return (size_t)W;
        if (l == L_RGB) return (size_t)(3 + n.C) * W2;
        if (l == L_T1 || l == L_T2) return (size_t)W2 * W2;
        if (l == L_TRGB) return (size_t)3 * W2;
        return (size_t)W2;
    }
    return 0;
}
static float abs_max(const float* p, size_t cnt) {
    float m = 0.f;
    for (size_t i = 0; i < cnt; ++i) {
        const float a = fabsf(p[i]);
        if (a > m) m = a;
    }
    return m;
}
static void assign_weight_exponents(const Net& n, Stream (&st)[NEFES_N_STREAMS]) {
    const int e_dt = n.transient ? scale_exp(abs_max(n.dt_w.data(), n.dt_w.size())) : 0;
    for (auto& stream : st)
        for (auto& sg : stream.segs) {
            if (!sg.h3 || !sg.W) continue;
            const bool dt = sg.W == n.dt_w.data() || (n.transient && (sg.W == n.w(L_DIR) || sg.W == n.w(L_T0)));
            sg.wexp = dt ? e_dt : scale_exp(abs_max(sg.W, matrix_elems(n, sg.W)));
        }
}

static int group_of(const Net& n, const float* Wm) {
    if (!Wm) return -1;
    if (Wm == n.th_w.data()) return L_TRGB;
    if (Wm == n.dt_w.data()) return L_DIR;
    for (int l = 0; l < 18; ++l)
        if (n.t[2 * l] == Wm) return (n.transient && l == L_T0) ? (int)L_DIR : ((l == L_TSIGMA || l == L_TBETA) ? (int)L_TRGB : l);
    return -1;
}

bool build(const NefesNetDesc* d, const float* const* tensors, Net& n, Stream (&st)[NEFES_N_STREAMS]) {
    if (!d) return false;
    if (d->width != 128 && d->width != 256) return false;
    if (nefes_head_class(d->feat_dim) < 0) return false;
    n.W = d->width; n.W2 = n.W / 2; n.C = d->feat_dim;
    n.NTW = n.W / 32; n.NTH = n.W2 / 32; n.NTR = nefes_head_ntr(n.C);
    n.transient = d->has_transient != 0;
    n.ext = d->xyz_encoding == NEFES_XYZ_EXTERNAL32;
    if (d->xyz_encoding != NEFES_XYZ_FREQ10 && !n.ext) return false;
    n.in_xyz = n.ext ? 32 : 63;
    n.e_steps = n.ext ? NEFES_X_STEPS : NEFES_E_STEPS;
    n.t = tensors;
    if (tensors && n.transient) {
        n.th_w.assign((size_t)5 * n.W2, 0.f);
        n.th_b.assign(5, 0.f);
        memcpy(&n.th_w[0], n.w(L_TRGB), sizeof(float) * 3 * n.W2);
        memcpy(&n.th_w[(size_t)3 * n.W2], n.w(L_TSIGMA), sizeof(float) * n.W2);
        memcpy(&n.th_w[(size_t)4 * n.W2], n.w(L_TBETA), sizeof(float) * n.W2);
        memcpy(&n.th_b[0], n.b(L_TRGB), sizeof(float) * 3);
        n.th_b[3] = n.b(L_TSIGMA)[0];
        n.th_b[4] = n.b(L_TBETA)[0];
        n.dt_w.resize((size_t)2 * n.W2 * (n.W + 27));
        memcpy(&n.dt_w[0], n.w(L_DIR), sizeof(float) * n.W2 * (n.W + 27));
        memcpy(&n.dt_w[(size_t)n.W2 * (n.W + 27)], n.w(L_T0), sizeof(float) * n.W2 * (n.W + 27));
    } else {
        n.dt_w.assign((size_t)2 * n.W2 * (n.W + 27), 0.f);
        n.th_w.assign((size_t)5 * n.W2, 0.f);
        n.th_b.assign(5, 0.f);
    }
    static const float* dummy[36] = {nullptr};
    if (!tensors) n.t = dummy;
    add_trunk(n, st[NEFES_STREAM_FWD_SIGMA]);
    add_trunk(n, st[NEFES_STREAM_FWD_STATIC]);
    add_static_head(n, st[NEFES_STREAM_FWD_STATIC]);
    add_backward(n, st[NEFES_STREAM_BWD_STATIC], false, false);
    if (n.transient) {
        add_trunk(n, st[NEFES_STREAM_FWD_FULL]);
        add_static_head(n, st[NEFES_STREAM_FWD_FULL]);
        add_transient_head(n, st[NEFES_STREAM_FWD_FULL]);
        add_backward(n, st[NEFES_STREAM_BWD_FULL]);
    }
    const bool big = n.W == 256, small = n.W == 128 && n.C == 128 && !n.ext;
    const bool h3_shape = !n.ext || (n.W == 256 && nefes_head_class(n.C) == 0);
    if (big || small) add_trunk(n, st[NEFES_STREAM_FWD_SIGMA_X6], 1);
    if (n.transient && (big || small) && (small || n.C == 16)) {
        add_trunk(n, st[NEFES_STREAM_FWD_FULL_X6], 1);
        add_heads_x6(n, st[NEFES_STREAM_FWD_FULL_X6]);
        add_backward(n, st[NEFES_STREAM_BWD_FULL_X6], 1);
    }
    if (h3_shape) {
        add_trunk(n, st[NEFES_STREAM_FWD_SIGMA_H3], 2);
        st[NEFES_STREAM_FWD_SIGMA_H3].h3 = true;
        {
            add_trunk(n, st[NEFES_STREAM_FWD_STATIC_H3], 2);
            add_static_head_h3(n, st[NEFES_STREAM_FWD_STATIC_H3]);
            add_backward(n, st[NEFES_STREAM_BWD_STATIC_H3], 2, false);
            st[NEFES_STREAM_FWD_STATIC_H3].h3 = st[NEFES_STREAM_BWD_STATIC_H3].h3 = true;
        }
        if (n.transient) {
            add_trunk(n, st[NEFES_STREAM_FWD_FULL_H3], 2);
            add_heads_x6(n, st[NEFES_STREAM_FWD_FULL_H3], 2);
// ... 58 lines not shown
    else if (l == L_TRGB) { out = 3; in = n.W2; }
    else { out = 1; in = n.W2; }
    return bias ? out : (int64_t)out * in;
}

static int pack_walk(const NefesNetDesc* desc, const Net& n, char* base, uint32_t* map, const NefesBlobInfo& info,
                     Stream (&st)[NEFES_N_STREAMS]) {
    auto code = [](float v, int part) { return v == 0.f ? 0u : (((uint32_t)v) << 3 | (uint32_t)part); };
    auto code16 = [](float v, int part, int group) { return v == 0.f ? 0u : ((uint32_t)group << 27 | ((uint32_t)v) << 3 | (uint32_t)part); };
    for (int k = 0; k < NEFES_N_STREAMS; ++k) {
        const NefesStreamInfo& si = info.stream[k];
        if (si.n_slabs == 0) continue;
        uint64_t boff = si.bias_off;
        for (auto& bb : st[k].bias)
            for (int r : bb.ridx) {
                const float v = r < 0 ? 0.f : bb.b[r];
                if (base) memcpy(base + boff, &v, 4);
                if (map) { map[boff / 2] = code(v, 0); map[boff / 2 + 1] = code(v, 1); }
                boff += 4;
            }
        if (st[k].h3) {
            const int ns = (int)st[k].segs.size(), nb = (int)st[k].bias.size();
            for (int i = 0; i < st[k].scale_count(); ++i) {
                uint32_t word = 0;
                if (!map && i < 2 * ns) {
                    const Seg& sg = st[k].segs[i / 2];
                    if (i % 2 == 0) { const int32_t e = sg.wexp; memcpy(&word, &e, 4); }
                    else { const float b = sg.row_bound(); memcpy(&word, &b, 4); }
                } else if (!map && i < 2 * ns + nb) {
                    const BiasBlk& bb = st[k].bias[i - 2 * ns];
                    float m = 0.f;
                    for (int r : bb.ridx)
                        if (r >= 0 && fabsf(bb.b[r]) > m) m = fabsf(bb.b[r]);
                    memcpy(&word, &m, 4);
                }
                if (base) memcpy(base + boff, &word, 4);
                if (map) {
                    uint32_t lo = 0, hi = 0;
                    if (i < 2 * ns && i % 2 == 0) {
                        const Seg& sg = st[k].segs[i / 2];
                        const int g = sg.h3 ? group_of(n, sg.W) : -1;
                        if (g >= 0) { lo = (uint32_t)g << 27 | 1u << 3 | 7u; hi = (uint32_t)g << 27 | 2u << 3 | 7u; }
                    } else if (i < 2 * ns + nb) {
                        lo = hi = NEFES_PACK_KEEP;
                    }
                    map[boff / 2] = lo; map[boff / 2 + 1] = hi;
                }
                boff += 4;
            }
        }
        uint64_t soff = si.slab_off;
        const int frags = NEFES_FRAGS_OF_KIB(nefes_stream_slab_kib(k, desc->width));
        const uint64_t slab_bytes = (uint64_t)frags * 256;
        for (auto& sg : st[k].segs) {
            if (sg.h3) {
                const int ups = (frags / 4) / 2;
                for (int sl = 0; sl < sg.slabs(frags); ++sl, soff += slab_bytes) {
                    for (int uu = 0; uu < ups && sl * ups + uu < sg.units(); ++uu) {
                        const int u = sl * ups + uu, q = u / sg.nt, t = u % sg.nt;
                        const uint64_t grp = soff + (uint64_t)uu * 2048;
                        for (int lane = 0; lane < 64; ++lane)
                            for (int i = 0; i < 8; ++i) {
                                const float v = sg.at16(q, i, t, lane);
                                uint16_t part[2] = {0, 0};
                                if (!map) split_f16x2(v, sg.wexp, part);
                                for (int pp = 0; pp < 2; ++pp) {
// ... 49 lines not shown
extern "C" int nefes_pack_weights(const NefesNetDesc* desc, const float* const* tensors, int n_tensors, void* blob,
                                  size_t blob_bytes) {
    if (!desc || !tensors || !blob) return NEFES_E_BADARG;
    const int need = desc->has_transient ? 36 : 24;
    if (n_tensors < need) return NEFES_E_BADARG;
    for (int i = 0; i < need; ++i)
        if (!tensors[i]) return NEFES_E_BADARG;
    Net n;
    Stream st[NEFES_N_STREAMS];
    if (!build(desc, tensors, n, st)) return NEFES_E_UNSUPPORTED;
    NefesBlobInfo info;
    fill_info(st, desc->width, &info);
    if (blob_bytes < info.total_bytes) return NEFES_E_BADBLOB;
    char* base = (char*)blob;
    memset(base, 0, info.total_bytes);
    uint32_t* hdr = (uint32_t*)base;
    hdr[0] = 0x5346454eu;
    hdr[1] = NEFES_ABI_VERSION;
    memcpy(hdr + 2, desc, sizeof(*desc));
    memcpy(hdr + 8, &info, sizeof(info));
    return pack_walk(desc, n, base, nullptr, info, st);
}

struct Indexed {
    std::vector<std::vector<float>> idx;
    const float* ptrs[36] = {nullptr};
    int64_t off[37] = {0};
    int need = 0;
    Net n;
    Stream st[NEFES_N_STREAMS];
    NefesBlobInfo info;
};
static int build_indexed(const NefesNetDesc* desc, Indexed& x, int64_t* tensor_elems_out) {
    {
        Stream tmp[NEFES_N_STREAMS];
        if (!build(desc, nullptr, x.n, tmp)) return NEFES_E_UNSUPPORTED;
    }
    x.need = desc->has_transient ? 36 : 24;
    x.idx.resize(x.need);
    int64_t flat = 0;
    for (int i = 0; i < x.need; ++i) {
        const int64_t ne = tensor_elems(x.n, i);
        if (tensor_elems_out) tensor_elems_out[i] = ne;
        x.idx[i].resize((size_t)ne);
        for (int64_t e = 0; e < ne; ++e) x.idx[i][(size_t)e] = (float)(flat + e + 1);
        x.off[i] = flat;
        flat += ne;
        x.ptrs[i] = x.idx[i].data();
    }
    x.off[x.need] = flat;
    if (flat + 1 >= (1 << 24)) return NEFES_E_UNSUPPORTED;
    if (!build(desc, x.ptrs, x.n, x.st)) return NEFES_E_UNSUPPORTED;
    fill_info(x.st, desc->width, &x.info);
    return 0;
}

extern "C" int nefes_pack_map(const NefesNetDesc* desc, uint32_t* map, size_t n_entries, int64_t* tensor_elems_out) {
    if (!desc || !map) return NEFES_E_BADARG;
    Indexed x;
    const int rc = build_indexed(desc, x, tensor_elems_out);
    if (rc) return rc;
    if (n_entries < x.info.total_bytes / 2) return NEFES_E_BADBLOB;
    memset(map, 0, sizeof(uint32_t) * (x.info.total_bytes / 2));
    return pack_walk(desc, x.n, nullptr, map, x.info, x.st);
}

// ... 68 lines not shown
```

### nefes_amd/field.py

```python
import os

import torch
import torch.nn as nn

from . import lib as L
from . import ops

FEATURE_DIM = 128


class FusionNet(nn.Module):
    mean = [0.485, 0.456, 0.406]
    std = [0.229, 0.224, 0.225]

    def __init__(self, f_dim, fusion_residule=False, no_BN=False):
        super().__init__()
        self.fusion_residule, self.no_BN = fusion_residule, no_BN
        layers = [nn.Conv2d(3 + f_dim, 64, 3, 1, 1), nn.ReLU(), nn.Conv2d(64, 64, 3, 1, 1), nn.ReLU(),
                  nn.Conv2d(64, 64, 3, 1, 1), nn.ReLU(), nn.Conv2d(64, f_dim, 5, 1, 2)]
        if not no_BN:
            layers.append(nn.BatchNorm2d(f_dim))
        self.net = nn.Sequential(*layers)
        self._norm = {}

# ... 108 lines not shown
        self.encode_transient = False if typ == 'coarse' else encode_transient
        self.beta_min = beta_min
        self.W_features = f_dim
        self.out_ch_size = out_ch_size + f_dim
        self.fusion_residule, self.no_BN = fusion_residule, no_BN
        for i in range(D):
            n_in = in_channels_xyz if i == 0 else (W + in_channels_xyz if i in self.skips else W)
            setattr(self, f"xyz_encoding_{i + 1}", nn.Sequential(nn.Linear(n_in, W), nn.ReLU(True)))
        self.xyz_encoding_final = nn.Linear(W, W)
        self.dir_encoding = nn.Sequential(nn.Linear(W + in_channels_dir, W // 2), nn.ReLU(True))
        self.static_sigma = nn.Sequential(nn.Linear(W, 1), nn.Softplus())
        if self.out_ch_size == 3:
            self.static_rgb = nn.Sequential(nn.Linear(W // 2, 3), nn.Sigmoid())
        else:
            self.static_rgb = nn.Sequential(nn.Linear(W // 2, self.out_ch_size))
        if self.encode_transient:
            self.transient_encoding = nn.Sequential(nn.Linear(W + in_channels_dir, W // 2), nn.ReLU(True),
                                                    nn.Linear(W // 2, W // 2), nn.ReLU(True),
                                                    nn.Linear(W // 2, W // 2), nn.ReLU(True))
            self.transient_sigma = nn.Sequential(nn.Linear(W // 2, 1), nn.Softplus())
            if out_ch_size == 3:
                self.transient_rgb = nn.Sequential(nn.Linear(W // 2, 3), nn.Sigmoid())
            else:
                self.transient_rgb = nn.Sequential(nn.Linear(W // 2, self.out_ch_size))
            self.transient_beta = nn.Sequential(nn.Linear(W // 2, 1), nn.Softplus())
        if typ == 'coarse':
            self.fusion_net = FusionNet(self.W_features, fusion_residule, no_BN)
            self.exposure_embedding = ExposureMLP(10, 12)
            self.sigmoid = nn.Sigmoid()
        self._pk = None
        self._pk_key = None
        self._pk_gen = None
        self._pk_gen_key = None

    def _supported(self):
        freq_xyz = self.in_channels_xyz in range(3, 64, 6)
        return (self.D == 8 and self.skips == [4] and (freq_xyz or self.in_channels_xyz == 32) and self.in_channels_dir in range(3, 28, 6)
                and self.W in (128, 256) and self.out_ch_size != 3 and 0 < self.W_features <= ops.HEAD_MAX_C
                and (freq_xyz or (self.W == 256 and ops.head_class(self.W_features) == 0)))

    def _embedding_columns(self):
        ex, ed, W = self.in_channels_xyz, self.in_channels_dir, self.W
        cols = []
        if ex != 32 and ex < 63:
            cols += [("xyz_encoding_1.0.weight", 0, ex, 63), ("xyz_encoding_5.0.weight", 0, ex, 63)]
        if ed < 27:
            cols += [("dir_encoding.0.weight", W, ed, 27)]
            if self.encode_transient:
                cols += [("transient_encoding.0.weight", W, ed, 27)]
        return cols

    def _kernel_params(self, sd):
        cols = self._embedding_columns()
        if not cols:
            return sd
        out = dict(sd)
        for name, at, have, want in cols:
            w = sd[name]
            out[name] = torch.cat([w[:, :at + have], w.new_zeros(w.shape[0], want - have), w[:, at + have:]], 1)
        return out

    def shrink_grads(self, g):
        for name, at, have, want in self._embedding_columns():
            if name in g:
                g[name] = torch.cat([g[name][:, :at + have], g[name][:, at + want:]], 1)
        return g
# ... 20 lines not shown
    def packed_generic(self) -> ops.PackedGeneric:
        if not self._generic_supported():
            raise RuntimeError(f"nefes_amd: no field kernel serves {self._shape()}.  Compiled: {ops.COMPILED_SET}")
        names = ops.PackedGeneric.layer_names(self.D, self.encode_transient)
        sd = dict(self.named_parameters())
        prm = [sd[n + s] for n in names for s in (".weight", ".bias")]
        key = tuple((p.data_ptr(), p._version, str(p.device)) for p in prm)
        if self._pk_gen is None or key != self._pk_gen_key:
            dev = prm[0].device if prm[0].is_cuda else torch.device("cuda")
            ksd = {n: p.detach() for n, p in sd.items()}
            for name, at, have, want in self._generic_embedding_columns():
                w = ksd[name]
                ksd[name] = torch.cat([w[:, :at + have], w.new_zeros(w.shape[0], want - have), w[:, at + have:]], 1)
            skip = 4 if (4 in self.skips and self.D > 4) else -1
            self._pk_gen = ops.PackedGeneric(ksd, self.W, self.D, skip, self.W_features, self.encode_transient, dev)
            self._pk_gen_key = key
        return self._pk_gen

    def uses_generic(self):
        if self._supported() and not (ops.FIELD_GENERIC and self._generic_supported()):
            return False
        return True

    def packed_any(self):
        return self.packed_generic() if self.uses_generic() else self.packed()

    def require_frozen_for_generic(self, what):
        raise NotImplementedError(f"nefes_amd: {what} is not built for the generic field kernels ({self._shape()}); they serve frozen "
                                  f"weights with the frequency embedding only.  Tuned instances: {ops.COMPILED_SET}")

    def invalidate_packed(self):
        self._pk_key = None
        self._pk_gen_key = None

    def packed(self) -> ops.PackedField:
        if not self._supported():
            raise RuntimeError(f"nefes_amd: the HIP field kernels are built for D=8, skips=[4], frequency encodings of up to 10 / 4 "
                               f"octaves (3 + 6k inputs, k <= 10 / 4) and a feature head (f_dim>0); got D={self.D}, skips={self.skips}, "
                               f"W={self.W}, f_dim={self.W_features}, in_channels_xyz={self.in_channels_xyz}, "
                               f"in_channels_dir={self.in_channels_dir}.  Compiled: {ops.COMPILED_SET}")
        names = ops.PackedField.LAYERS_FINE if self.encode_transient else ops.PackedField.LAYERS_COARSE
        sd = dict(self.named_parameters())
        prm = [sd[n + s] for n in names for s in (".weight", ".bias")]
        key = tuple((p.data_ptr(), p._version, str(p.device)) for p in prm)
        pad = bool(self._embedding_columns())
        if os.environ.get("NEFES_DEBUG_PACK_CHECKSUM", "0") == "1":
            key += (float(sum(p.detach().double().sum() for p in prm)),)
        if (self._pk is not None and key != self._pk_key and any(p.requires_grad for p in prm)
                and all(p.is_cuda and p.device == self._pk.blob.device for p in prm)):
            if pad:
                ksd = self._kernel_params(sd)
                self._pk.repack([ksd[n + s_] for n in names for s_ in (".weight", ".bias")])
            else:
                self._pk.repack(prm)
            self._pk_key = key
        elif self._pk is None or key != self._pk_key:
            dev = prm[0].device if prm[0].is_cuda else torch.device("cuda")
            enc = L.XYZ_EXTERNAL32 if self.in_channels_xyz == 32 else L.XYZ_FREQ10
            self._pk = ops.PackedField(self._kernel_params({n: p.detach() for n, p in sd.items()}), self.W, self.W_features,
                                       self.encode_transient, dev, enc)
            self._pk_key = key
        return self._pk

    def factored_head_ok(self):
        return (ops.FACTORED_HEAD and not ops.FIELD_GENERIC and self.encode_transient and self.W == 128 and self.in_channels_xyz != 32 and self._supported()
                and 3 + self.W_features > 3 + self.W // 2 + 1 and ops.SPLIT == "h3"
                and not any(p.requires_grad for n, p in self.named_parameters()
                            if not n.startswith(("fusion_net", "exposure_embedding"))))

    def packed_fh(self):
        names = ops.PackedField.LAYERS_FINE
        sd = dict(self.named_parameters())
        prm = [sd[n + s] for n in names for s in (".weight", ".bias")]
        key = tuple((p.data_ptr(), p._version, str(p.device)) for p in prm)
        if getattr(self, "_pk_fh", None) is None or key != self._pk_fh_key:
            dev = prm[0].device if prm[0].is_cuda else torch.device("cuda")
            ksd = dict(self._kernel_params({n: p.detach() for n, p in sd.items()}))
            w, b = ksd["static_rgb.0.weight"], ksd["static_rgb.0.bias"]
            ksd["static_rgb.0.weight"], ksd["static_rgb.0.bias"] = w[:3].contiguous(), b[:3].contiguous()
            pk = ops.PackedField(ksd, self.W, 0, True, dev, L.XYZ_FREQ10)
            w_f = w[3:].to(dev, torch.float32).contiguous()
            self._pk_fh = (pk, w_f, w_f.t().contiguous(), b[3:].to(dev, torch.float32).contiguous())
            self._pk_fh_key = key
        return self._pk_fh

    def forward(self, x, sigma_only=False, output_transient=True):
        if sigma_only:
            input_xyz = x
        else:
            input_xyz, input_dir_a = torch.split(x, [self.in_channels_xyz, self.in_channels_dir], dim=-1)
        h = input_xyz
        for i in range(self.D):
            if i in self.skips:
                h = torch.cat([input_xyz, h], 1)
            h = getattr(self, f"xyz_encoding_{i + 1}")(h)
        static_sigma = self.static_sigma(h)
        if sigma_only:
            return static_sigma
        final = self.xyz_encoding_final(h)
        head_in = torch.cat([final, input_dir_a], 1)
        static = torch.cat([self.static_rgb(self.dir_encoding(head_in)), static_sigma], 1)
# ... 81 lines not shown
```

### nefes_amd/lib.py

```python
import ctypes as C
import os

import torch

_HERE = os.path.dirname(os.path.abspath(__file__))
LIB_PATH = os.environ.get("NEFES_HIP_LIB") or os.path.join(_HERE, "libnefes_hip.so")


class NefesNetDesc(C.Structure):
    _fields_ = [("width", C.c_int32), ("feat_dim", C.c_int32), ("has_transient", C.c_int32), ("xyz_encoding", C.c_int32)]


class NefesGenericNetDesc(C.Structure):
    _fields_ = [("width", C.c_int32), ("depth", C.c_int32), ("skip", C.c_int32), ("feat_dim", C.c_int32), ("has_transient", C.c_int32)]


class NefesStreamInfo(C.Structure):
    _fields_ = [("slab_off", C.c_uint64), ("n_slabs", C.c_uint32), ("bias_floats", C.c_uint32), ("bias_off", C.c_uint64),
                ("scale_off", C.c_uint32), ("scale_count", C.c_uint32)]


class NefesBlobInfo(C.Structure):
    _fields_ = [("total_bytes", C.c_uint64), ("stream", NefesStreamInfo * 13)]


class NefesHashGridDesc(C.Structure):
    _fields_ = [("n_levels", C.c_int32), ("n_features", C.c_int32), ("log2_hashmap_size", C.c_int32),
                ("base_resolution", C.c_int32), ("per_level_scale", C.c_float), ("bound", C.c_float)]


ABI_VERSION = 16
STREAM_FWD_SIGMA, STREAM_FWD_STATIC, STREAM_FWD_FULL, STREAM_BWD_FULL, STREAM_FWD_SIGMA_X6, STREAM_FWD_FULL_X6, STREAM_BWD_FULL_X6, STREAM_BWD_STATIC = 0, 1, 2, 3, 4, 5, 6, 7
STREAM_FWD_SIGMA_H3, STREAM_FWD_FULL_H3, STREAM_BWD_FULL_H3, STREAM_FWD_STATIC_H3, STREAM_BWD_STATIC_H3 = 8, 9, 10, 11, 12
FIELD_SIGMA, FIELD_STATIC, FIELD_FULL = 0, 1, 2
XYZ_FREQ10, XYZ_EXTERNAL32 = 0, 1
(TB_E, TB_DV, TB_L1, TB_FINAL, TB_DIR, TB_T0, TB_T1, TB_T2, TB_RGB, TB_SIG, TB_TH, TB_END) = (0, 1, 2, 10, 11, 12, 13, 14, 15, 16,
                                                                                              17, 18)
COMP_TRANSIENT, COMP_STATIC_ONLY, COMP_SIGMA_ONLY, COMP_WHITE_BKGD, COMP_FEAT_WEIGHTS_ONLY = 1, 2, 4, 8, 16

_p, _i, _f, _u32, _sz = C.c_void_p, C.c_int, C.c_float, C.c_uint32, C.c_size_t
_desc = C.POINTER(NefesNetDesc)
_gdesc = C.POINTER(NefesGenericNetDesc)

SIGNATURES = {
    "nefes_version": (_i, []),
    "nefes_blob_info": (_i, [_desc, C.POINTER(NefesBlobInfo)]),
    "nefes_stream_slab_bytes": (_sz, [_desc, _i]),
    "nefes_fusion_input_fwd": (_i, [_i, _i, _i, _p, _p, _p, C.POINTER(_f), C.POINTER(_f), _p, _p, _p]),
    "nefes_fusion_input_bwd": (_i, [_i, _i, _i, _p, _p, _p, C.POINTER(_f), _p, _p, _p]),
    "nefes_upcos_loss_fwd": (_i, [_i, _i, _i, _i, _i, _i, _p, _p, _p, _p, _p]),
    "nefes_upcos_loss_bwd": (_i, [_i, _i, _i, _i, _i, _i, _p, _p, _p, _p, _p, _p, _p, _p, _p, _p, _i, _p, _p, _p]),
    "nefes_bicubic_gather_table": (_i, [_i, _i, _i, _i, _i, _p, _p, _p, _p]),
    "nefes_bicubic_gram": (_i, [_i, _i, _i, _i, _p, _p]),
    "nefes_bn_train_fwd": (_i, [_i, _i, C.c_int64, _i, _p, _p, _p, C.c_double, C.c_double, _p, _p, _p, _p, _p, _p]),
    "nefes_bn_train_bwd": (_i, [_i, _i, C.c_int64, _i, _p, _p, _p, _p, _p, _p]),
    "nefes_svd_reg_fwd": (_i, [_i, _p, _p, _p, _p]),
    "nefes_svd_reg_bwd": (_i, [_i, _p, _p, _p, _p]),
    "nefes_regressed_pose_fwd": (_i, [_i, _p, _i, _f, _f, _f, _f, _p, _p, _p]),
    "nefes_regressed_pose_bwd": (_i, [_i, _p, _i, _f, _p, _p, _p]),
    "nefes_upcos_prepare": (_i, [_i, _i, _i, _i, _i, _i, _p, _p, _p, _p, _p, _p, _p, _i, _p, _p, _p, _p]),
    "nefes_upcos_gram_fwd": (_i, [_i, _i, _i, _p, _p, _p, _p, _p, _i, _p, _p, _p, _p]),
    "nefes_upcos_gram_bwd": (_i, [_i, _i, _i, _p, _p, _p, _p, _p, _p]),
    "nefes_upcos_gram_lds_bytes": (_sz, [_i, _i, _i]),
    "nefes_adam_step": (_i, [_i, _p, _p, _p, _p, _p, _p, C.c_double, C.c_double, C.c_double, _p]),
# ... 106 lines not shown
```

### nefes_amd/ops.py

```python
import ctypes as C
from typing import Optional

import os

import torch

from . import lib as L


def _stream():
    return C.c_void_p(torch.cuda.current_stream().cuda_stream)


TIMERS = None


class _timed:
    def __init__(self, name):
        self.name = name

    def __enter__(self):
        if TIMERS is not None:
            self.t0 = torch.cuda.Event(enable_timing=True)
            self.t1 = torch.cuda.Event(enable_timing=True)
# ... 169 lines not shown
    with _timed("field_fwd[sigma,h3]"):
        L.check(L.load().nefes_field_fwd_h3_zrow(pk.desc, _chk(pk.blob, "blob", torch.uint8), L.FIELD_SIGMA, N, S, _chk(rays_o, "rays_o"),
                                                 _chk(rays_d, "rays_d"), _chk(z_row, "z_row"), None, _chk(raw_t, "raw_t"), None, _stream()),
                "nefes_field_fwd_h3_zrow")
    return raw_t


def coarse_sample(sigma, z, Ni, u=None, want_samples=True, want_weights=False):
    sigma, z = _f32(sigma), _f32(z)
    N, Nc = sigma.shape[0], sigma.shape[-1]
    dev = sigma.device
    if u is None:
        u = _linspace01(Ni, dev)
    u = _f32(u)
    z_fine = torch.empty(N, Nc + Ni, device=dev)
    z_samples = torch.empty(N, Ni, device=dev) if want_samples else None
    weights = torch.empty(N, Nc, device=dev) if want_weights else None
    with _timed("coarse_sample"):
        L.check(L.load().nefes_coarse_sample(N, Nc, Ni, _chk(sigma, "sigma"), _chk(z, "z"), 1 if z.dim() == 1 else 0, _chk(u, "u"),
                                             1 if u.dim() == 2 else 0, _chk(z_fine, "z_fine"), _chk(z_samples, "z_samples"),
                                             _chk(weights, "weights"), _stream()), "nefes_coarse_sample")
    _tap("z_fine", z_fine)
    _tap("z_samples", z_samples)
    return (z_fine, z_samples, weights) if want_weights else (z_fine, z_samples)


class PackedField:

    LAYERS_COARSE = [f"xyz_encoding_{i}.0" for i in range(1, 9)] + ["xyz_encoding_final", "dir_encoding.0",
                                                                    "static_sigma.0", "static_rgb.0"]
    LAYERS_FINE = LAYERS_COARSE + ["transient_encoding.0", "transient_encoding.2", "transient_encoding.4",
                                   "transient_sigma.0", "transient_rgb.0", "transient_beta.0"]

    def __init__(self, state_dict, width, feat_dim, has_transient, device, xyz_encoding=0):
        lib = L.load()
        self.desc = L.NefesNetDesc(int(width), int(feat_dim), 1 if has_transient else 0, int(xyz_encoding))
        self.xyz_encoding = int(xyz_encoding)
        self.width, self.feat_dim, self.has_transient = int(width), int(feat_dim), bool(has_transient)
        info = L.NefesBlobInfo()
        L.check(lib.nefes_blob_info(self.desc, info), "nefes_blob_info")
        names = self.LAYERS_FINE if has_transient else self.LAYERS_COARSE
        host = []
        for n in names:
            host.append(state_dict[n + ".weight"].detach().to("cpu", torch.float32).contiguous())
            host.append(state_dict[n + ".bias"].detach().to("cpu", torch.float32).contiguous())
        ptrs = (C.c_void_p * len(host))(*[t.data_ptr() for t in host])
        blob = torch.zeros(info.total_bytes, dtype=torch.uint8)
        L.check(lib.nefes_pack_weights(self.desc, ptrs, len(host), C.c_void_p(blob.data_ptr()), blob.numel()),
                "nefes_pack_weights")
        self.blob = blob.to(device)
        self.info = info
        self.generation = 0
        self.h3_valid = True
        self._map = None

    def repack(self, params):
        lib = L.load()
        if self._map is None:
            n = self.info.total_bytes // 2
            host_map = torch.zeros(n, dtype=torch.int32)
            elems = (C.c_int64 * 36)()
            L.check(lib.nefes_pack_map(self.desc, C.c_void_p(host_map.data_ptr()), n, C.cast(elems, C.c_void_p)), "nefes_pack_map")
            self._map = host_map.to(self.blob.device)
            self._elems = list(elems)[:36 if self.has_transient else 24]
            need = C.c_size_t(0)
            L.check(lib.nefes_pack_h3_plan(self.desc, None, 0, C.byref(need)), "nefes_pack_h3_plan")
            plan = torch.zeros(int(need.value), dtype=torch.int32)
            L.check(lib.nefes_pack_h3_plan(self.desc, C.c_void_p(plan.data_ptr()), plan.numel(), None), "nefes_pack_h3_plan")
            self._plan_jobs = int(plan[0])
            self._plan = plan.to(self.blob.device)
            self._plan_scratch = torch.zeros(32, dtype=torch.int32, device=self.blob.device)
        if [int(p.numel()) for p in params] != self._elems:
            raise RuntimeError("nefes_amd: parameter shapes do not match the packed network description")
        flat = torch.cat([p.detach().reshape(-1) for p in params]).to(torch.float32)
        h3 = REPACK_H3 and self._plan_jobs > 0
        L.check(lib.nefes_pack_device(flat.data_ptr(), flat.numel(), self._map.data_ptr(), self._map.numel(),
                                      self._plan.data_ptr() if h3 else None, self._plan_jobs if h3 else 0,
                                      self._plan_scratch.data_ptr() if h3 else None, self.blob.data_ptr(), _stream()),
                "nefes_pack_device")
        self.generation += 1
        if not h3:
            self.h3_valid = False

    def h3_byte_ranges(self):
        out = []
        for k in (L.STREAM_FWD_SIGMA_H3, L.STREAM_FWD_FULL_H3, L.STREAM_BWD_FULL_H3, L.STREAM_FWD_STATIC_H3, L.STREAM_BWD_STATIC_H3):
            si = self.info.stream[k]
            if si.n_slabs:
                slab = int(L.load().nefes_stream_slab_bytes(self.desc, k))
                out.append((int(si.slab_off), int(si.slab_off + si.n_slabs * slab)))
# ... 26 lines not shown
                                     _chk(rays_d, "rays_d"), _chk(z, "z"), _chk(pts, "pts"), _chk(xyz_enc, "xyz_enc"),
                                     _chk(viewdirs, "viewdirs"), _chk(raw_t, "raw_t"), _chk(masks, "masks", torch.int32),
                                     _stream()), "nefes_field_fwd")
    if masks is not None:
        _tap("masks", (masks, N, S, pk.width, mode))
    return raw_t, masks


SPLIT = os.environ.get("NEFES_SPLIT", "h3")
REPACK_H3 = os.environ.get("NEFES_REPACK_H3", "1") != "0"
USE_X6 = os.environ.get("NEFES_X6", "1") != "0"
FUSED_COARSE = os.environ.get("NEFES_FUSED_COARSE", "1") != "0"


HEAD_MAX_C = 141
COMPILED_SET = L.COMPILED_SET


def head_class(C):
    return -1 if C < 0 else (0 if 3 + C <= 32 else (1 if 3 + C <= 144 else -1))


def canonical_shape(pk: PackedField):
    return (pk.width == 256 and pk.feat_dim == 16) or (pk.width == 128 and pk.feat_dim == 128 and pk.xyz_encoding == L.XYZ_FREQ10)


def h3_shape(pk: PackedField):
    cls = head_class(pk.feat_dim)
    if pk.width not in (128, 256) or cls < 0:
        return False
    return True if pk.xyz_encoding == L.XYZ_FREQ10 else (pk.width == 256 and cls == 0)


def x6_supported(pk: PackedField, mode, forward=True):
    if mode == L.FIELD_STATIC:
        return static_h3(pk)
    ok = canonical_shape(pk) or (_h3(pk) and h3_shape(pk))
    return ok and (mode == L.FIELD_SIGMA or (mode == L.FIELD_FULL and pk.has_transient))


def static_h3(pk: PackedField):
    return _h3(pk) and h3_shape(pk) and pk.xyz_encoding == L.XYZ_FREQ10


def _h3(pk):
    if SPLIT not in ("h3", "x6", "f32"):
        raise ValueError("nefes_amd.ops.SPLIT must be 'h3', 'x6' or 'f32'")
    return SPLIT == "h3" and pk.h3_valid


def require_instance(pk: PackedField, what):
    if canonical_shape(pk) or (_h3(pk) and h3_shape(pk)):
        return
    raise RuntimeError(f"nefes_amd: no kernel instance serves {what} for W={pk.width}, f_dim={pk.feat_dim}, "
                       f"xyz_encoding={pk.xyz_encoding} with NEFES_SPLIT={SPLIT}"
                       f"{'' if pk.h3_valid else ' (fp16 streams stale: NEFES_REPACK_H3=0)'}.  Compiled: {COMPILED_SET}")


def field_fwd_x6(pk: PackedField, mode, N, S, rays_o=None, rays_d=None, z=None, viewdirs=None, want_masks=False, xyz_enc=None,
                 pts=None):
    dev = pk.blob.device
    raw_t = torch.empty(N, pk.n_raw(mode), S, device=dev)
    masks = torch.empty(pk.mask_bytes(N * S) // 4, dtype=torch.int32, device=dev) if want_masks else None
    h3 = _h3(pk) and h3_shape(pk) and N * S < (1 << 31) - 256
    if mode == L.FIELD_STATIC and not h3:
        return field_fwd(pk, mode, N, S, rays_o=rays_o, rays_d=rays_d, z=z, pts=pts, viewdirs=viewdirs, want_masks=want_masks, xyz_enc=xyz_enc)
    if not h3 and not canonical_shape(pk):
        raise RuntimeError(f"nefes_amd: {N * S} samples in one launch exceed the fp16 two-part kernels' 32-bit sample index and "
                           f"W={pk.width}, f_dim={pk.feat_dim} has no other instance; render fewer rays per launch")
    fn = L.load().nefes_field_fwd_h3 if h3 else L.load().nefes_field_fwd_x6
    with _timed(f"field_fwd[{('sigma', 'static', 'full')[mode]},{'h3' if h3 else 'x6'}]"):
        L.check(fn(pk.desc, _chk(pk.blob, "blob", torch.uint8), mode, N, S, _chk(rays_o, "rays_o"),
                                            _chk(rays_d, "rays_d"), _chk(z, "z"), _chk(pts, "pts"), _chk(xyz_enc, "xyz_enc"),
                                            _chk(viewdirs, "viewdirs"),
                                            _chk(raw_t, "raw_t"), _chk(masks, "masks", torch.int32), _stream()),
                "nefes_field_fwd_x6")
    if masks is not None:
        _tap("masks", (masks, N, S, pk.width, mode))
    return raw_t, masks


def field_bwd(pk: PackedField, N, S, raw_t, g_raw_t, masks, rays_o=None, rays_d=None, z=None, pts=None, viewdirs=None,
              mode=L.FIELD_FULL):
    dev = pk.blob.device
    ext = pk.xyz_encoding == L.XYZ_EXTERNAL32
    if mode == L.FIELD_STATIC and USE_X6 and SPLIT != "f32" and static_h3(pk) and N * S < (1 << 31) - 256:
        g_pts, g_vs = torch.empty(N * S, 3, device=dev), torch.empty(N * S, 3, device=dev)
        with _timed("field_bwd[static,h3]"):
            L.check(L.load().nefes_field_bwd_static_h3(pk.desc, _chk(pk.blob, "blob", torch.uint8), N, S, _chk(rays_o, "rays_o"),
                                                       _chk(rays_d, "rays_d"), _chk(z, "z"), _chk(pts, "pts"), _chk(viewdirs, "viewdirs"),
                                                       _chk(raw_t, "raw_t"), _chk(g_raw_t, "g_raw_t"), _chk(masks, "masks", torch.int32),
                                                       _chk(g_pts, "g_pts"), _chk(g_vs, "g_vs"), _stream()), "nefes_field_bwd_static_h3")
        return g_pts, g_vs
    if mode == L.FIELD_STATIC:
        if not canonical_shape(pk):
            raise RuntimeError(f"nefes_amd: the static-head backward of W={pk.width}, f_dim={pk.feat_dim} was routed to the fp32-MFMA "
                               f"instances (NEFES_SPLIT={SPLIT}), which exist for the canonical shapes only.  Compiled: {COMPILED_SET}")
        g_pts, g_vs = torch.empty(N * S, 3, device=dev), torch.empty(N * S, 3, device=dev)
        with _timed("field_bwd[static]"):
            L.check(L.load().nefes_field_bwd_static(pk.desc, _chk(pk.blob, "blob", torch.uint8), N, S, _chk(rays_o, "rays_o"),
                                                    _chk(rays_d, "rays_d"), _chk(z, "z"), _chk(pts, "pts"), _chk(viewdirs, "viewdirs"),
                                                    _chk(raw_t, "raw_t"), _chk(g_raw_t, "g_raw_t"), _chk(masks, "masks", torch.int32),
                                                    _chk(g_pts, "g_pts"), _chk(g_vs, "g_vs"), _stream()), "nefes_field_bwd_static")
        return g_pts, g_vs
    g_pts = None if ext else torch.empty(N * S, 3, device=dev)
    g_enc = torch.empty(N * S, 32, device=dev) if ext else None
    g_vs = torch.empty(N * S, 3, device=dev)
    if USE_X6 and SPLIT != "f32" and x6_supported(pk, L.FIELD_FULL, forward=False):
        h3 = _h3(pk)
        fn = L.load().nefes_field_bwd_h3 if h3 else L.load().nefes_field_bwd_x6
        with _timed("field_bwd[h3]" if h3 else "field_bwd[x6]"):
            L.check(fn(pk.desc, _chk(pk.blob, "blob", torch.uint8), N, S, _chk(rays_o, "rays_o"),
                                                _chk(rays_d, "rays_d"), _chk(z, "z"), _chk(pts, "pts"), _chk(viewdirs, "viewdirs"),
                                                _chk(raw_t, "raw_t"), _chk(g_raw_t, "g_raw_t"), _chk(masks, "masks", torch.int32),
                                                _chk(g_pts, "g_pts"), _chk(g_enc, "g_enc"), _chk(g_vs, "g_vs"), _stream()),
                    "nefes_field_bwd_x6")
        return (g_enc if ext else g_pts), g_vs
    with _timed("field_bwd"):
      L.check(L.load().nefes_field_bwd(pk.desc, _chk(pk.blob, "blob", torch.uint8), N, S, _chk(rays_o, "rays_o"),
                                     _chk(rays_d, "rays_d"), _chk(z, "z"), _chk(pts, "pts"), _chk(viewdirs, "viewdirs"),
                                     _chk(raw_t, "raw_t"), _chk(g_raw_t, "g_raw_t"), _chk(masks, "masks", torch.int32),
                                     _chk(g_pts, "g_pts"), _chk(g_enc, "g_enc"), _chk(g_vs, "g_vs"), _stream()),
              "nefes_field_bwd")
    return (g_enc if ext else g_pts), g_vs


def ray_grad_reduce(N, S, z, g_pts, g_vs):
    dev = g_pts.device
    g_o, g_d, g_v = (torch.empty(N, 3, device=dev) for _ in range(3))
    with _timed("ray_grad_reduce"):
      L.check(L.load().nefes_ray_grad_reduce(N, S, _chk(z, "z"), _chk(g_pts, "g_pts"), _chk(g_vs, "g_vs"), _chk(g_o, "g_o"),
                                           _chk(g_d, "g_d"), _chk(g_v, "g_v"), _stream()), "nefes_ray_grad_reduce")
    return g_o, g_d, g_v


class FieldFromRays(torch.autograd.Function):

    @staticmethod
    def forward(ctx, rays_o, rays_d, viewdirs, z, pk, mode):
        rays_o, rays_d, viewdirs, z = _f32(rays_o), _f32(rays_d), _f32(viewdirs), _f32(z)
        N, S = z.shape
        need = mode in (L.FIELD_FULL, L.FIELD_STATIC) and any(ctx.needs_input_grad[:3])
        if USE_X6 and SPLIT != "f32" and x6_supported(pk, mode):
            raw_t, masks = field_fwd_x6(pk, mode, N, S, rays_o, rays_d, z, viewdirs=viewdirs, want_masks=need)
# ... 1084 lines not shown
```

### nefes_amd/render.py

```python
import types

import torch

from . import lib as L
from . import ops

_DEV = "cuda"
MAX_RAYS_PER_LAUNCH = 1 << 22
MEMORY_FRACTION = 0.6


_STEP = {}
_PER_RAY = {}


def rays_per_launch(cfg, network_fn, network_fine, device, train=False):
    net = network_fine if (network_fine is not None and cfg.N_importance > 0) else network_fn
    S = cfg.N_samples + cfg.N_importance if not cfg.use_fine_only or cfg.N_importance == 0 else cfg.N_importance
    Wd, C = net.W, net.W_features
    dev = torch.device(device)
    key = (Wd, C, S, cfg.N_samples, bool(train), dev.type, dev.index)
    if key in _STEP:
        return _STEP[key]
    R = 3 + C + 6
# ... 114 lines not shown
    u = None if cfg.perturb == 0. else torch.rand(N, Ni, device=dev)
    z_fine, z_samples = ops.sample_pdf_merge(z, w0.detach(), Ni, u=u)
    return _fine_pass(rays_o, rays_d, viewdirs, z_fine, z_samples, network_fine, cfg, C, field, (rgb0, feat0, disp0, acc0))


def _noise(shape, device):
    return torch.randn(tuple(shape), device=device)


def _with_density_noise(raw, C, std):
    noise = torch.zeros_like(raw)
    noise[:, 3 + C] = _noise((raw.shape[0], raw.shape[2]), raw.device) * std
    return raw + noise


def _fine_pass(rays_o, rays_d, viewdirs, z_fine, z_samples, network_fine, cfg, C, field, coarse_maps):
    rgb0, feat0, disp0, acc0 = coarse_maps if coarse_maps is not None else (None, None, None, None)
    z_f = z_samples if cfg.use_fine_only else z_fine
    flags = 0
    if (cfg.test_time and cfg.NeRFW and cfg.nerfh_nff and cfg.xyz_encoder is None and cfg.raw_noise_std == 0.
            and z_f.shape[0] * z_f.shape[1] < (1 << 31) - 256 and network_fine.factored_head_ok()):
        pk_fh, w_f, w_f_t, b_f = network_fine.packed_fh()
        flags |= L.COMP_TRANSIENT
        if not cfg.transient_at_test:
            flags |= L.COMP_STATIC_ONLY
        if cfg.white_bkgd:
            flags |= L.COMP_WHITE_BKGD
        rgb, feat, disp, acc = ops.RenderFineFH.apply(rays_o, rays_d, viewdirs, z_f, pk_fh, w_f, w_f_t, b_f, flags, float(network_fine.beta_min),
                                                      cfg.feat_as_gmap)
        ret = {"rgb_map": rgb, "disp_map": disp, "acc_map": acc, "feat_map": feat}
        if cfg.feat_as_gmap:
            ret["feat_is_gmap"] = True
        return ret
    pk_f = network_fine.packed_any()
    mode = L.FIELD_FULL if cfg.NeRFW else L.FIELD_STATIC
    raw_f = field(network_fine, pk_f, mode, z_f)
    if cfg.raw_noise_std > 0. and not cfg.NeRFW:
        raw_f = _with_density_noise(raw_f, C, cfg.raw_noise_std)
    if cfg.NeRFW:
        flags |= L.COMP_TRANSIENT
        if cfg.test_time and not cfg.transient_at_test:
            flags |= L.COMP_STATIC_ONLY
    if cfg.white_bkgd:
        flags |= L.COMP_WHITE_BKGD
    rgb, feat, disp, acc, depth, weights, beta = ops.Composite.apply(raw_f, z_f, C, flags, float(network_fine.beta_min))
    ret = {"rgb_map": rgb, "disp_map": disp, "acc_map": acc}
    if cfg.nerfh_nff:
        ret["feat_map"] = feat
    if not cfg.test_time:
        ret["rgb0"], ret["disp0"], ret["acc0"] = rgb0, disp0, acc0
        ret["z_std"] = torch.std(z_samples, dim=-1, unbiased=False)
        if cfg.NeRFW:
            ret["transient_sigmas"] = raw_f[:, 3 + C + 4, :]
            ret["beta"] = beta
        if cfg.nerfh_nff and feat0 is not None:
            ret["feat0"] = feat0
    return ret


def render_rays(ray_batch, network_fn, network_query_fn=None, N_samples=64, retraw=False, lindisp=False, perturb=0.,
                N_importance=0, network_fine=None, white_bkgd=False, raw_noise_std=0., verbose=False, pytest=False,
                i_epoch=-1, embedding_a=None, embedding_t=None, test_time=False, args=None, volume=None):
    if ray_batch.shape[-1] < 11:
        raise NotImplementedError("nefes_amd: the NeFeS field always uses view directions (ray batch needs >= 11 columns)")
    ray_batch = ray_batch.to(_DEV, torch.float32)
    rays_o, rays_d = ray_batch[:, 0:3].contiguous(), ray_batch[:, 3:6].contiguous()
    viewdirs = ray_batch[:, 8:11].contiguous()
    cfg = _cfg(dict(N_samples=N_samples, N_importance=N_importance, perturb=perturb, lindisp=lindisp,
# ... 87 lines not shown
```

Baseline: 731,400 rays/s.

## Fold the linear final layer into downstream heads for frozen W=256 networks

Adds a 'fold_final' packing mode that pre-multiplies the trunk's linear final layer into the direction and transient head weights, so both the forward and backward h3 kernels skip one 256x256 GEMM per sample. New kernel instances (TU parts 9 and 11) and segment remapping handle the folded pack. The path is used only for frozen networks on the full fine pass, is on by default through NEFES_FOLD_FINAL, and cannot be re-packed on device. Running the folded product weights through fp16 can change numerics slightly.

Result: faster. 797,100 rays/s, median of 6 (+9.0%).

```diff
diff --git a/include/nefes_hip.h b/include/nefes_hip.h
--- a/include/nefes_hip.h
+++ b/include/nefes_hip.h
@@ -7,7 +7,7 @@
 extern "C" {
 #endif
 
-#define NEFES_ABI_VERSION 16
+#define NEFES_ABI_VERSION 17
 
 #define NEFES_E_BADARG (-1)
 #define NEFES_E_UNSUPPORTED (-2)
@@ -18,6 +18,7 @@
     int32_t feat_dim;
     int32_t has_transient;
     int32_t xyz_encoding;
+    int32_t fold_final;
 } NefesNetDesc;
 #define NEFES_XYZ_FREQ10 0
 #define NEFES_XYZ_EXTERNAL32 1
diff --git a/nefes_amd/csrc/field_bwd_h3.hip b/nefes_amd/csrc/field_bwd_h3.hip
--- a/nefes_amd/csrc/field_bwd_h3.hip
+++ b/nefes_amd/csrc/field_bwd_h3.hip
@@ -5,7 +5,7 @@
 #define NEFES_FENCE_TILES
 #else
 #define NEFES_SLAB_KIB 32
-#if !defined(NEFES_TU_PART) || NEFES_TU_PART == 0 || NEFES_TU_PART == 1 || NEFES_TU_PART == 5
+#if !defined(NEFES_TU_PART) || NEFES_TU_PART == 0 || NEFES_TU_PART == 1 || NEFES_TU_PART == 5 || NEFES_TU_PART == 9 || NEFES_TU_PART == 11
 #define H3B_WIDE
 #define H3_ACC_READ_ASM
 #define NEFES_ASM_READS_ACC
@@ -89,8 +89,12 @@
     return __builtin_nontemporal_load(p);
 }
 
-template <int W, int KR16, int ENC, bool HAS_T = true, bool TRAIN = false, bool FH = false>
+#define NEFES_H3B_FOLD 16
+template <int W, int KRF, int ENC, bool HAS_T = true, bool TRAIN = false, bool FH = false>
 __global__ __launch_bounds__(256, NEFES_H3B_WG_PER_CU(W)) void field_bwd_h3_kernel(FieldBwdH3Args a) {
+    constexpr bool FOLD = (KRF & NEFES_H3B_FOLD) != 0;
+    constexpr int KR16 = KRF & ~NEFES_H3B_FOLD;
+    static_assert(!FOLD || (!TRAIN && !FH), "the fold serves frozen networks with their own feature head");
     constexpr int NTW = W / 32, NTH = W / 64, HS = W / 2, GS = W / 4;
     constexpr int MW = 8 * (W / 64) + 4 * (W / 128);
     constexpr int WT = (NTW + 1) / 2, WH = (NTH + 1) / 2;
@@ -107,13 +111,13 @@
     constexpr int SX = ENC == NEFES_XYZ_HASHGRID_FUSED ? 24 : 8;
     int* tab_i = (int*)(smem + NEFES_H3B_SLOTS * NEFES_SLAB_BYTES + (size_t)4 * (MW + SX) * 256);
     const float* tab_f = (const float*)tab_i;
-    if (threadIdx.x < 2 * (HAS_T ? NEFES_H3B_N : NEFES_H3B_N_STATIC)) tab_i[threadIdx.x] = a.tab[threadIdx.x];
+    if (threadIdx.x < 2 * ((HAS_T ? NEFES_H3B_N : NEFES_H3B_N_STATIC) - (FOLD ? 1 : 0))) tab_i[threadIdx.x] = a.tab[threadIdx.x];
     HgGeom* hg_lds = (HgGeom*)(tab_i + 64);
     if constexpr (ENC == NEFES_XYZ_HASHGRID_FUSED) {
         if (threadIdx.x == 0) *hg_lds = a.hg;
     }
-    auto wexp = [&](int seg) { return tab_i[nefes_h3_tab_exp(nefes_h3b_seg(HAS_T, seg))]; };
-    auto rowb = [&](int seg) { return tab_f[nefes_h3_tab_bound(nefes_h3b_seg(HAS_T, seg))]; };
+    auto wexp = [&](int seg) { return tab_i[nefes_h3_tab_exp(nefes_h3b_seg(HAS_T, nefes_h3b_fold_seg(FOLD, seg)))]; };
+    auto rowb = [&](int seg) { return tab_f[nefes_h3_tab_bound(nefes_h3b_seg(HAS_T, nefes_h3b_fold_seg(FOLD, seg)))]; };
     StagedRing ring;
     ring.init(a.stream, a.n_slabs, smem, wave, lane);
     const char* ring_lane = smem + lane * 16;
@@ -343,9 +347,23 @@
 #pragma unroll
                 for (int c = 0; c < 3; ++c) STASH(3 + c) = gv[c];
             }
-        }
+            if constexpr (FOLD) asm volatile("" : "+v"(gv[0]), "+v"(gv[1]), "+v"(gv[2]));
+        }
+        f32x16 (&XP)[NTW + 2] = FOLD ? XA : XB;
+        f32x16 (&XQ)[NTW + 2] = FOLD ? XB : XA;
         int es_b;
-        {
+        if constexpr (FOLD) {
+            es_b = es_dt;
+            const float dsig = STASH(6);
+            float dsg[1];
+            dsg[0] = dsig * pow2i(es_b);
+#if defined(H3B_WIDE) && defined(H3_WIDE_ENTRY_FENCE)
+            mma_run<NTW, 1, 2, false, ((WIDE_LAYERS >> 8) & 1) == 0 || (NTW < NEFES_H3_WIDE_MIN)>(ring, ring_lane, ArrayIn<1>{dsg}, ZeroInit{}, XA);
+#else
+            mma_run<NTW, 1, 2, false>(ring, ring_lane, ArrayIn<1>{dsg}, ZeroInit{}, XA);
+#endif
+            M += rowb(NEFES_H3B_SIG) * pair_max(fabsf(dsig));
+        } else {
             const int ew = wexp(NEFES_H3B_FINAL), tau = tau_of(M, ew);
             float mx = 0.f;
             es_b = tau + ew;
@@ -370,10 +388,10 @@
             mma_run_h3<NTILES, W / 16, T0, true, 2, ((WIDE_LAYERS >> (L)) & 1) != 0>(ring, ring_lane, wrap_store_h3<TRAIN>(MaskedSplitH<NTW + 2, WT, 2>{SRC, bt, pow2i(tau - ES_SRC), mx}, gptr(NEFES_TB_L1 + (L) - 1), pow2i(-(ES_SRC))), ZeroInit{}, DST); \
             M = rowb(NEFES_H3B_L8 + 8 - (L)) * (pair_max(mx) * pow2i(-(ES_SRC)));                                   \
         }
-        NEFES_BWD_LAYER(8, XB, XA, es_b, es_a, NTW, 2)
-        NEFES_BWD_LAYER(7, XA, XB, es_a, es_b, NTW, 2)
-        NEFES_BWD_LAYER(6, XB, XA, es_b, es_a, NTW, 2)
-        NEFES_BWD_LAYER(5, XA, XB, es_a, es_b, NTW + 2, 0)
+        NEFES_BWD_LAYER(8, XP, XQ, es_b, es_a, NTW, 2)
+        NEFES_BWD_LAYER(7, XQ, XP, es_a, es_b, NTW, 2)
+        NEFES_BWD_LAYER(6, XP, XQ, es_b, es_a, NTW, 2)
+        NEFES_BWD_LAYER(5, XQ, XP, es_a, es_b, NTW + 2, 0)
         es_e = es_b;
         float gx[3] = {0.f, 0.f, 0.f};
         float ge[ENC != NEFES_XYZ_FREQ10 ? NEFES_X_STEPS : 1];
@@ -381,22 +399,22 @@
             const float inv = pow2i(-es_e);
             if constexpr (ENC != NEFES_XYZ_FREQ10) {
 #pragma unroll
-                for (int s_ = 0; s_ < NEFES_X_STEPS; ++s_) ge[s_] = XB[0][s_] * inv;
+                for (int s_ = 0; s_ < NEFES_X_STEPS; ++s_) ge[s_] = XP[0][s_] * inv;
             } else {
                 float dE[32], x3[3];
 #pragma unroll
                 for (int t = 0; t < 2; ++t)
 #pragma unroll
-                    for (int r = 0; r < 16; ++r) dE[t * 16 + r] = XB[t][r] * inv;
+                    for (int r = 0; r < 16; ++r) dE[t * 16 + r] = XP[t][r] * inv;
 #pragma unroll
                 for (int c = 0; c < 3; ++c) x3[c] = STASH(c);
                 embed_slots_bwd<NEFES_N_FREQ_XYZ>(gx, dE, x3, h);
                 ge[0] = 0.f;
             }
         }
-        NEFES_BWD_LAYER(4, XB, XA, es_b, es_a, NTW, 2)
-        NEFES_BWD_LAYER(3, XA, XB, es_a, es_b, NTW, 2)
-        NEFES_BWD_LAYER(2, XB, XA, es_b, es_a, NTW, 2)
+        NEFES_BWD_LAYER(4, XP, XQ, es_b, es_a, NTW, 2)
+        NEFES_BWD_LAYER(3, XQ, XP, es_a, es_b, NTW, 2)
+        NEFES_BWD_LAYER(2, XP, XQ, es_b, es_a, NTW, 2)
 #undef NEFES_BWD_LAYER
         int es_1;
         {
@@ -404,13 +422,13 @@
             const int ew = wexp(NEFES_H3B_L1), tau = tau_of(M, ew);
             float mx = 0.f;
             es_1 = tau + ew;
-            mma_run_h3<2, W / 16, 0, true>(ring, ring_lane, wrap_store_h3<TRAIN>(MaskedSplitH<NTW + 2, WT, 2>{XA, bt, pow2i(tau - es_a), mx}, gptr(NEFES_TB_L1), pow2i(-es_a)), ZeroInit{}, XB);
+            mma_run_h3<2, W / 16, 0, true>(ring, ring_lane, wrap_store_h3<TRAIN>(MaskedSplitH<NTW + 2, WT, 2>{XQ, bt, pow2i(tau - es_a), mx}, gptr(NEFES_TB_L1), pow2i(-es_a)), ZeroInit{}, XP);
         }
         const float inv1 = pow2i(-es_1);
         if constexpr (ENC == NEFES_XYZ_HASHGRID_FUSED) {
             float x3[3];
 #pragma unroll
-            for (int s_ = 0; s_ < NEFES_X_STEPS; ++s_) STASH(8 + s_) = ge[s_] + XB[0][s_] * inv1;
+            for (int s_ = 0; s_ < NEFES_X_STEPS; ++s_) STASH(8 + s_) = ge[s_] + XP[0][s_] * inv1;
 #pragma unroll
             for (int c = 0; c < 3; ++c) x3[c] = STASH(c);
             asm volatile("" : "+v"(x3[0]), "+v"(x3[1]), "+v"(x3[2]));
@@ -419,7 +437,7 @@
             for (int c = 0; c < 3; ++c) gv[c] = STASH(3 + c);
         } else if constexpr (ENC == NEFES_XYZ_EXTERNAL32) {
 #pragma unroll
-            for (int s_ = 0; s_ < NEFES_X_STEPS; ++s_) ge[s_] += XB[0][s_] * inv1;
+            for (int s_ = 0; s_ < NEFES_X_STEPS; ++s_) ge[s_] += XP[0][s_] * inv1;
             if (valid) {
                 float* gp = a.g_enc + m * 32 + h;
 #pragma unroll
@@ -430,7 +448,7 @@
 #pragma unroll
             for (int t = 0; t < 2; ++t)
 #pragma unroll
-                for (int r = 0; r < 16; ++r) dE[t * 16 + r] = XB[t][r] * inv1;
+                for (int r = 0; r < 16; ++r) dE[t * 16 + r] = XP[t][r] * inv1;
 #pragma unroll
             for (int c = 0; c < 3; ++c) x3[c] = STASH(c);
             embed_slots_bwd<NEFES_N_FREQ_XYZ>(g1, dE, x3, h);
@@ -485,6 +503,8 @@
 int nefes_bwd_h3_launch_part6(int which, const FieldBwdH3Args& a, hipStream_t st);
 int nefes_bwd_h3_launch_part7(int which, const FieldBwdH3Args& a, hipStream_t st);
 int nefes_bwd_h3_launch_part8(int which, const FieldBwdH3Args& a, hipStream_t st);
+int nefes_bwd_h3_launch_part9(int which, const FieldBwdH3Args& a, hipStream_t st);
+int nefes_bwd_h3_launch_part11(int which, const FieldBwdH3Args& a, hipStream_t st);
 
 #if NEFES_TU_PART == 1
 int nefes_bwd_h3_launch_part1(int which, const FieldBwdH3Args& a, hipStream_t st) {
@@ -536,6 +556,16 @@
 int nefes_bwd_h3_launch_part8(int which, const FieldBwdH3Args& a, hipStream_t st) {
     if (which == BWD_H3_TRAIN_STATIC) return launch_bwd_h3<128, 2, NEFES_XYZ_FREQ10, false, true>(a, st);
     if (which == BWD_H3_TRAIN_FULL) return launch_bwd_h3<128, 2, NEFES_XYZ_FREQ10, true, true>(a, st);
+    return NEFES_E_UNSUPPORTED;
+}
+#elif NEFES_TU_PART == 9
+int nefes_bwd_h3_launch_part9(int which, const FieldBwdH3Args& a, hipStream_t st) {
+    if (which == BWD_H3_FULL) return launch_bwd_h3<256, 2 | NEFES_H3B_FOLD, NEFES_XYZ_FREQ10>(a, st);
+    return NEFES_E_UNSUPPORTED;
+}
+#elif NEFES_TU_PART == 11
+int nefes_bwd_h3_launch_part11(int which, const FieldBwdH3Args& a, hipStream_t st) {
+    if (which == BWD_H3_FULL) return launch_bwd_h3<256, 9 | NEFES_H3B_FOLD, NEFES_XYZ_FREQ10>(a, st);
     return NEFES_E_UNSUPPORTED;
 }
 #else
@@ -552,6 +582,7 @@
     if (full && !desc->has_transient) return NEFES_E_UNSUPPORTED;
     const int cls = nefes_head_class(desc->feat_dim);
     if ((desc->width != 256 && desc->width != 128) || cls < 0 || desc->xyz_encoding != NEFES_XYZ_FREQ10) return NEFES_E_UNSUPPORTED;
+    if (desc->fold_final) return NEFES_E_UNSUPPORTED;
     NefesBlobInfo info;
     int rc = nefes_blob_info(desc, &info);
     if (rc) return rc;
@@ -583,6 +614,7 @@
     const bool full = mode == NEFES_FIELD_FULL;
     if (full && !desc->has_transient) return NEFES_E_UNSUPPORTED;
     if (desc->width != 256 || nefes_head_class(desc->feat_dim) != 0 || desc->xyz_encoding != NEFES_XYZ_EXTERNAL32) return NEFES_E_UNSUPPORTED;
+    if (desc->fold_final) return NEFES_E_UNSUPPORTED;
     NefesBlobInfo info;
     int rc = nefes_blob_info(desc, &info);
     if (rc) return rc;
@@ -611,6 +643,7 @@
     if (!pts && !(rays_o && rays_d && z)) return NEFES_E_BADARG;
     const int cls = nefes_head_class(desc->feat_dim);
     if ((desc->width != 256 && desc->width != 128) || cls < 0 || desc->xyz_encoding != NEFES_XYZ_FREQ10) return NEFES_E_UNSUPPORTED;
+    if (desc->fold_final) return NEFES_E_UNSUPPORTED;
     NefesBlobInfo info;
     int rc = nefes_blob_info(desc, &info);
     if (rc) return rc;
@@ -642,11 +675,13 @@
     const bool fused_grid = ext && table != nullptr;
     if (fused_grid ? !(g_pts && grid && rays_o && rays_d && z) : (ext ? !g_xyz_enc : (!g_pts || (!pts && !(rays_o && rays_d && z))))) return NEFES_E_BADARG;
     if (!desc->has_transient) return NEFES_E_UNSUPPORTED;
+    const bool fold = desc->fold_final != 0;
+    if (fold && (desc->width != 256 || ext || fh)) return NEFES_E_UNSUPPORTED;
     NefesBlobInfo info;
     int rc = nefes_blob_info(desc, &info);
     if (rc) return rc;
     const NefesStreamInfo& si = info.stream[NEFES_STREAM_BWD_FULL_H3];
-    if (si.n_slabs == 0 || si.scale_count < 2 * NEFES_H3B_N) return NEFES_E_UNSUPPORTED;
+    if (si.n_slabs == 0 || si.scale_count < 2 * (uint32_t)(fold ? NEFES_H3BF_N : NEFES_H3B_N)) return NEFES_E_UNSUPPORTED;
     FieldBwdH3Args a;
     a.stream = (const char*)packed + si.slab_off;
     a.tab = (const int*)((const char*)packed + si.bias_off) + si.scale_off;
@@ -676,6 +711,7 @@
     if (fh) return nefes_bwd_h3_launch_part6(BWD_H3_FH, a, st);
     if (desc->width == 256 && fused_grid) return cls == 0 ? nefes_bwd_h3_launch_part1(BWD_H3_HG, a, st) : NEFES_E_UNSUPPORTED;
     if (desc->width == 256 && ext) return cls == 0 ? nefes_bwd_h3_launch_part1(BWD_H3_EXT, a, st) : NEFES_E_UNSUPPORTED;
+    if (desc->width == 256 && fold) return cls == 0 ? nefes_bwd_h3_launch_part9(BWD_H3_FULL, a, st) : nefes_bwd_h3_launch_part11(BWD_H3_FULL, a, st);
     if (desc->width == 256) return cls == 0 ? launch_bwd_h3<256, 2, NEFES_XYZ_FREQ10>(a, st) : nefes_bwd_h3_launch_part5(BWD_H3_FULL, a, st);
     if (desc->width == 128 && !ext) return cls == 1 ? nefes_bwd_h3_launch_part2(BWD_H3_FULL, a, st) : nefes_bwd_h3_launch_part6(BWD_H3_FULL, a, st);
     return NEFES_E_UNSUPPORTED;
diff --git a/nefes_amd/csrc/field_fwd_h3.hip b/nefes_amd/csrc/field_fwd_h3.hip
--- a/nefes_amd/csrc/field_fwd_h3.hip
+++ b/nefes_amd/csrc/field_fwd_h3.hip
@@ -65,13 +65,18 @@
         }
 }
 
-template <int MODE, int ENC, int W = 256, int NTR = 1, bool TRAIN = false, bool FH = false>
+#define NEFES_FIELD_FULL_FOLD 3
+template <int MODEF, int ENC, int W = 256, int NTR = 1, bool TRAIN = false, bool FH = false>
 __global__ __launch_bounds__(256, W == 128 ? 2 : 1) void field_fwd_h3_kernel(FieldFwdH3Args a) {
+    constexpr bool FOLD = MODEF == NEFES_FIELD_FULL_FOLD;
+    constexpr int MODE = FOLD ? NEFES_FIELD_FULL : MODEF;
     static_assert(NEFES_SLAB_KIB == (W == 128 ? NEFES_H3_FWD_SLAB_KIB_128 : NEFES_H3_FWD_SLAB_KIB), "ring slab size != the packer's for this width");
+    static_assert(!FOLD || (MODE != NEFES_FIELD_SIGMA && !TRAIN), "the fold serves the head products of frozen networks");
     constexpr int NTW = W / 32, NTH = W / 64;
     constexpr int ES = ENC != NEFES_XYZ_FREQ10 ? NEFES_X_STEPS : NEFES_E_STEPS;
     constexpr int MW = 8 * (W / 64) + 4 * (W / 128), WT = (NTW + 1) / 2, WH = (NTH + 1) / 2;
-    constexpr int NSEG = MODE == NEFES_FIELD_SIGMA ? NEFES_H3F_SIG + 1 : (MODE == NEFES_FIELD_STATIC ? NEFES_H3F_N_STATIC : NEFES_H3F_N);
+    constexpr int NSEG = MODE == NEFES_FIELD_SIGMA ? NEFES_H3F_SIG + 1
+                         : (MODE == NEFES_FIELD_STATIC ? NEFES_H3F_N_STATIC : (FOLD ? NEFES_H3FF_N : NEFES_H3F_N));
     extern __shared__ __attribute__((aligned(16))) char smem[];
     char* ring_base = smem;
     float* bias_lds = (float*)(smem + NEFES_H3_SLOTS * NEFES_SLAB_BYTES);
@@ -90,11 +95,11 @@
     const char* bias_half = (const char*)bias_lds + 16 * h;
     const int* tab_i = (const int*)(bias_lds + a.scale_off);
     const float* tab_f = bias_lds + a.scale_off;
-    auto wexp = [&](int seg) { return tab_i[nefes_h3_tab_exp(seg)]; };
-    auto rowb = [&](int seg) { return tab_f[nefes_h3_tab_bound(seg)]; };
-    auto bmax = [&](int blk) { return tab_f[nefes_h3_tab_bias(NSEG, blk)]; };
+    auto wexp = [&](int seg) { return tab_i[nefes_h3_tab_exp(nefes_h3f_seg(FOLD, seg))]; };
+    auto rowb = [&](int seg) { return tab_f[nefes_h3_tab_bound(nefes_h3f_seg(FOLD, seg))]; };
+    auto bmax = [&](int blk) { return tab_f[nefes_h3_tab_bias(NSEG, nefes_h3f_bias(FOLD, blk))]; };
     ring.prime(ring_lane);
-    constexpr int B_SIG = 8 * W, B_FINAL = B_SIG + 32, B_DIR = B_FINAL + W, B_RGB = B_DIR + W / 2,
+    constexpr int B_SIG = 8 * W, B_FINAL = B_SIG + 32, B_DIR = B_FINAL + (FOLD ? 0 : W), B_RGB = B_DIR + W / 2,
                   B_T0 = B_RGB + 32 * NTR, B_T1 = B_T0 + W / 2, B_T2 = B_T1 + W / 2, B_TH = B_T2 + W / 2;
 #pragma unroll 1
     for (int tile = blockIdx.x; tile < a.n_tiles; tile += gridDim.x) {
@@ -224,7 +229,8 @@
             save_trunk(L1_, B, es_b);                                                                                          \
         }                                                                                                                      \
         put_masks(bits, WT);
-        constexpr int NPAIRS = MODE == NEFES_FIELD_SIGMA ? 3 : 4;
+        constexpr bool END8 = MODE == NEFES_FIELD_SIGMA || FOLD;
+        constexpr int NPAIRS = END8 ? 3 : 4;
 #pragma unroll 1
         for (int p = 0; p < NPAIRS; ++p) {
             const int l1 = 2 + 2 * p, l2 = l1 + 1;
@@ -254,7 +260,7 @@
             }
             put_masks(bits, WT);
         }
-        if constexpr (MODE == NEFES_FIELD_SIGMA) { NEFES_FWD_EVEN_LAYER(8, NEFES_H3F_L8) }
+        if constexpr (END8) { NEFES_FWD_EVEN_LAYER(8, NEFES_H3F_L8) }
 #undef NEFES_FWD_EVEN_LAYER
         if constexpr (MODE == NEFES_FIELD_SIGMA) sigma_head(B, es_b, tau_of(M, wexp(NEFES_H3F_SIG)));
         if constexpr (MODE != NEFES_FIELD_SIGMA) {
@@ -290,7 +296,29 @@
                 __device__ __forceinline__ f32x16 operator()(int t) const { return t < NTH ? a(t) : b(t - NTH); }
             };
             int es_dt;
-            {
+            if constexpr (FOLD) {
+                sigma_head(B, es_b, tau_of(M, wexp(NEFES_H3F_SIG)));
+                const int ew = wexp(NEFES_H3F_DT_H);
+                const float mD = pair_max(array_max(Dv));
+                const int tau = tau_of(fmaxf(M, mD), ew);
+                const float rbh_ = rowb(NEFES_H3F_DT_H), rbd_ = rowb(NEFES_H3F_DT_D);
+                const float bm_ = fmaxf(bmax(NEFES_H3BB_DIR), bmax(NEFES_H3BB_T0));
+                float mx = 0.f;
+                es_dt = tau + ew;
+                clear_bits();
+                if constexpr (CB) {
+                    const char* bp8 = bias_half + 7 * W * 4;
+                    nbias = ReluBiasSplitH<CAP, NTW, WT>::prime(bp8);
+                    const ReluBiasSplitH<CAP, NTW, WT> src8{B, bits, pow2i(tau - es_b), mx, bp8, pow2i(es_b), nbias};
+                    mma_run_h3<NDT, W / 16, 0, true>(ring, ring_lane, src8, Bias2{bias_at(B_DIR, es_dt), bias_at(B_T0, es_dt)}, dt);
+                } else {
+                    const ReluSplitH<CAP, NTW, WT> src8{B, bits, pow2i(tau - es_b), mx};
+                    mma_run_h3<NDT, W / 16, 0, true>(ring, ring_lane, src8, Bias2{bias_at(B_DIR, es_dt), bias_at(B_T0, es_dt)}, dt);
+                }
+                mma_run_h3<NDT, 2, 0, false>(ring, ring_lane, ArraySplitH<16>{Dv, pow2i(tau)}, ZeroInit{}, dt);
+                M = rbh_ * (pair_max(mx) * pow2i(-es_b)) + rbd_ * mD + bm_;
+                put_masks(bits, WT);
+            } else {
                 const int ew = wexp(NEFES_H3F_DT_H);
                 const float mD = pair_max(array_max(Dv));
                 const int tau = tau_of(fmaxf(M, mD), ew);
@@ -458,6 +486,8 @@
 int nefes_fwd_h3_launch_part6(int which, const FieldFwdH3Args& a, hipStream_t st);
 int nefes_fwd_h3_launch_part7(int which, const FieldFwdH3Args& a, hipStream_t st);
 int nefes_fwd_h3_launch_part8(int which, const FieldFwdH3Args& a, hipStream_t st);
+int nefes_fwd_h3_launch_part9(int which, const FieldFwdH3Args& a, hipStream_t st);
+int nefes_fwd_h3_launch_part11(int which, const FieldFwdH3Args& a, hipStream_t st);
 
 
 #if NEFES_TU_PART == 1
@@ -525,6 +555,16 @@
         case H3_TRAIN_STATIC: return launch_h3<NEFES_FIELD_STATIC, NEFES_XYZ_FREQ10, 128, 1, true>(a, st);
         case H3_TRAIN_FULL: return launch_h3<NEFES_FIELD_FULL, NEFES_XYZ_FREQ10, 128, 1, true>(a, st);
     }
+    return NEFES_E_UNSUPPORTED;
+}
+#elif NEFES_TU_PART == 9
+int nefes_fwd_h3_launch_part9(int which, const FieldFwdH3Args& a, hipStream_t st) {
+    if (which == H3_FULL) return launch_h3<NEFES_FIELD_FULL_FOLD, NEFES_XYZ_FREQ10, 256, 1>(a, st);
+    return NEFES_E_UNSUPPORTED;
+}
+#elif NEFES_TU_PART == 11
+int nefes_fwd_h3_launch_part11(int which, const FieldFwdH3Args& a, hipStream_t st) {
+    if (which == H3_FULL) return launch_h3<NEFES_FIELD_FULL_FOLD, NEFES_XYZ_FREQ10, 256, 5>(a, st);
     return NEFES_E_UNSUPPORTED;
 }
 #else
@@ -538,6 +578,7 @@
     if (mode == NEFES_FIELD_FULL && !desc->has_transient) return NEFES_E_BADARG;
     const int cls = nefes_head_class(desc->feat_dim);
     if ((desc->width != 256 && desc->width != 128) || cls < 0 || desc->xyz_encoding != NEFES_XYZ_FREQ10) return NEFES_E_UNSUPPORTED;
+    if (desc->fold_final) return NEFES_E_UNSUPPORTED;
     NefesBlobInfo info;
     int rc = nefes_blob_info(desc, &info);
     if (rc) return rc;
@@ -568,6 +609,7 @@
     if (mode != NEFES_FIELD_STATIC && mode != NEFES_FIELD_FULL) return NEFES_E_UNSUPPORTED;
     if (mode == NEFES_FIELD_FULL && !desc->has_transient) return NEFES_E_BADARG;
     if (desc->width != 256 || nefes_head_class(desc->feat_dim) != 0 || desc->xyz_encoding != NEFES_XYZ_EXTERNAL32) return NEFES_E_UNSUPPORTED;
+    if (desc->fold_final) return NEFES_E_UNSUPPORTED;
     NefesBlobInfo info;
     int rc = nefes_blob_info(desc, &info);
     if (rc) return rc;
@@ -604,6 +646,8 @@
     const int cls = nefes_head_class(desc->feat_dim);
     const bool big = desc->width == 256, small = desc->width == 128 && !ext;
     if (!(big || small) || cls < 0 || (ext && cls != 0) || (desc->xyz_encoding != NEFES_XYZ_FREQ10 && !ext)) return NEFES_E_UNSUPPORTED;
+    const bool fold = desc->fold_final != 0;
+    if (fold && mode != NEFES_FIELD_SIGMA && !(mode == NEFES_FIELD_FULL && big && !ext && !fh)) return NEFES_E_UNSUPPORTED;
     NefesBlobInfo info;
     int rc = nefes_blob_info(desc, &info);
     if (rc) return rc;
@@ -647,6 +691,7 @@
         return cls == 1 ? nefes_fwd_h3_launch_part2(H3_FULL, a, st) : nefes_fwd_h3_launch_part6(H3_FULL, a, st);
     }
     if (mode == NEFES_FIELD_SIGMA) return launch_h3<NEFES_FIELD_SIGMA, NEFES_XYZ_FREQ10>(a, st);
+    if (fold) return cls == 0 ? nefes_fwd_h3_launch_part9(H3_FULL, a, st) : nefes_fwd_h3_launch_part11(H3_FULL, a, st);
     return cls == 0 ? launch_h3<NEFES_FIELD_FULL, NEFES_XYZ_FREQ10>(a, st) : nefes_fwd_h3_launch_part5(H3_FULL, a, st);
 }
 
diff --git a/nefes_amd/csrc/layout.h b/nefes_amd/csrc/layout.h
--- a/nefes_amd/csrc/layout.h
+++ b/nefes_amd/csrc/layout.h
@@ -80,6 +80,19 @@
 #define NEFES_H3F_N_STATIC (NEFES_H3F_RGB + 1)
 #define NEFES_H3B_N_STATIC (NEFES_H3B_N - 4)
 NEFES_HD int nefes_h3b_seg(int has_transient, int seg) { return (has_transient || seg == NEFES_H3B_RGB) ? seg : seg - 4; }
+enum { NEFES_H3FF_SIG = NEFES_H3F_SIG, NEFES_H3FF_DT_H, NEFES_H3FF_DT_D, NEFES_H3FF_RGB, NEFES_H3FF_T1, NEFES_H3FF_T2, NEFES_H3FF_TH,
+       NEFES_H3FF_N };
+enum { NEFES_H3FBB_SIG = NEFES_H3BB_SIG, NEFES_H3FBB_DIR, NEFES_H3FBB_RGB, NEFES_H3FBB_T0, NEFES_H3FBB_T1, NEFES_H3FBB_T2, NEFES_H3FBB_TH };
+enum { NEFES_H3BF_RGB = 0, NEFES_H3BF_TH, NEFES_H3BF_T2, NEFES_H3BF_T1, NEFES_H3BF_T0, NEFES_H3BF_DIR, NEFES_H3BF_SIG, NEFES_H3BF_L8,
+       NEFES_H3BF_L7, NEFES_H3BF_L6, NEFES_H3BF_L5, NEFES_H3BF_L4, NEFES_H3BF_L3, NEFES_H3BF_L2, NEFES_H3BF_L1, NEFES_H3BF_N };
+#define NEFES_H3FF_N_STATIC (NEFES_H3FF_RGB + 1)
+#define NEFES_H3BF_N_STATIC (NEFES_H3BF_N - 4)
+NEFES_HD int nefes_h3f_seg(int fold, int seg) { return (fold && seg > NEFES_H3F_FINAL) ? seg - 1 : seg; }
+NEFES_HD int nefes_h3f_bias(int fold, int block) { return (fold && block > NEFES_H3BB_FINAL) ? block - 1 : block; }
+NEFES_HD int nefes_h3b_fold_seg(int fold, int seg) { return (fold && seg > NEFES_H3B_FINAL) ? seg - 1 : seg; }
+static_assert(NEFES_H3FF_DT_H == NEFES_H3F_DT_H - 1 && NEFES_H3FF_TH == NEFES_H3F_TH - 1 && NEFES_H3FBB_DIR == NEFES_H3BB_DIR - 1 &&
+              NEFES_H3FBB_TH == NEFES_H3BB_TH - 1 && NEFES_H3BF_SIG == NEFES_H3B_SIG - 1 && NEFES_H3BF_L1 == NEFES_H3B_L1 - 1,
+              "folded ordinals = the unfolded ones with FINAL taken out");
 
 NEFES_HD int nefes_mask_words(int W) { return 8 * (W / 64) + 4 * (W / 128); }
 
diff --git a/nefes_amd/csrc/pack.cpp b/nefes_amd/csrc/pack.cpp
--- a/nefes_amd/csrc/pack.cpp
+++ b/nefes_amd/csrc/pack.cpp
@@ -114,6 +114,7 @@
 struct BiasBlk {
     const float* b;
     std::vector<int> ridx;
+    bool folded = false;
 };
 
 struct Stream {
@@ -181,6 +182,13 @@
     const float* const* t;
     std::vector<float> th_w, th_b;
     std::vector<float> dt_w;
+    bool fold = false;
+    std::vector<float> fd_w, ft_w, fdt_w, fd_b, ft_b;
+    const float* w_dir(bool h3) const { return fold && h3 ? fd_w.data() : w(L_DIR); }
+    const float* w_t0(bool h3) const { return fold && h3 ? ft_w.data() : w(L_T0); }
+    const float* w_dt(bool h3) const { return fold && h3 ? fdt_w.data() : dt_w.data(); }
+    const float* b_dir(bool h3) const { return fold && h3 ? fd_b.data() : b(L_DIR); }
+    const float* b_t0(bool h3) const { return fold && h3 ? ft_b.data() : b(L_T0); }
     const float* w(int l) const { return t[2 * l]; }
     const float* b(int l) const { return t[2 * l + 1]; }
 };
@@ -244,14 +252,16 @@
 
 void add_static_head_h3(const Net& n, Stream& st) {
     const int W = n.W, W2 = n.W2;
-    st.segs.push_back(seg(n.NTW, W / 2, k_natural(W / 2, 0), rows_natural(n.NTW, W), n.w(L_FINAL), W));
+    if (!n.fold) {
+        st.segs.push_back(seg(n.NTW, W / 2, k_natural(W / 2, 0), rows_natural(n.NTW, W), n.w(L_FINAL), W));
+        mark(st.segs.back(), 2);
+        st.bias.push_back({n.b(L_FINAL), rows_natural(n.NTW, W)});
+    }
+    st.segs.push_back(seg(n.NTH, W / 2, k_natural(W / 2, 0), rows_natural(n.NTH, W2), n.w_dir(true), W + 27));
     mark(st.segs.back(), 2);
-    st.bias.push_back({n.b(L_FINAL), rows_natural(n.NTW, W)});
-    st.segs.push_back(seg(n.NTH, W / 2, k_natural(W / 2, 0), rows_natural(n.NTH, W2), n.w(L_DIR), W + 27));
+    st.segs.push_back(seg(n.NTH, 16, k_emb(4, 16, W), rows_natural(n.NTH, W2), n.w_dir(true), W + 27));
     mark(st.segs.back(), 2);
-    st.segs.push_back(seg(n.NTH, 16, k_emb(4, 16, W), rows_natural(n.NTH, W2), n.w(L_DIR), W + 27));
-    mark(st.segs.back(), 2);
-    st.bias.push_back({n.b(L_DIR), rows_natural(n.NTH, W2)});
+    st.bias.push_back({n.b_dir(true), rows_natural(n.NTH, W2), n.fold});
     st.segs.push_back(seg(n.NTR, W2 / 2, k_natural(W2 / 2, 0), rows_natural(n.NTR, 3 + n.C), n.w(L_RGB), W2));
     mark(st.segs.back(), 2);
     st.bias.push_back({n.b(L_RGB), rows_natural(n.NTR, 3 + n.C)});
@@ -259,18 +269,21 @@
 
 void add_heads_x6(const Net& n, Stream& st, int kind = 1) {
     const int W = n.W, W2 = n.W2;
-    st.segs.push_back(seg(n.NTW, W / 2, k_natural(W / 2, 0), rows_natural(n.NTW, W), n.w(L_FINAL), W));
+    const bool h3 = kind == 2, fold = n.fold && h3;
+    if (!fold) {
+        st.segs.push_back(seg(n.NTW, W / 2, k_natural(W / 2, 0), rows_natural(n.NTW, W), n.w(L_FINAL), W));
+        mark(st.segs.back(), kind);
+        st.bias.push_back({n.b(L_FINAL), rows_natural(n.NTW, W)});
+    }
+    st.segs.push_back(seg(2 * n.NTH, W / 2, k_natural(W / 2, 0), rows_natural(2 * n.NTH, 2 * W2), n.w_dt(h3), W + 27));
     mark(st.segs.back(), kind);
-    st.bias.push_back({n.b(L_FINAL), rows_natural(n.NTW, W)});
-    st.segs.push_back(seg(2 * n.NTH, W / 2, k_natural(W / 2, 0), rows_natural(2 * n.NTH, 2 * W2), n.dt_w.data(), W + 27));
+    st.segs.push_back(seg(2 * n.NTH, 16, k_emb(4, 16, W), rows_natural(2 * n.NTH, 2 * W2), n.w_dt(h3), W + 27));
     mark(st.segs.back(), kind);
-    st.segs.push_back(seg(2 * n.NTH, 16, k_emb(4, 16, W), rows_natural(2 * n.NTH, 2 * W2), n.dt_w.data(), W + 27));
-    mark(st.segs.back(), kind);
-    st.bias.push_back({n.b(L_DIR), rows_natural(n.NTH, W2)});
+    st.bias.push_back({n.b_dir(h3), rows_natural(n.NTH, W2), fold});
     st.segs.push_back(seg(n.NTR, W2 / 2, k_natural(W2 / 2, 0), rows_natural(n.NTR, 3 + n.C), n.w(L_RGB), W2));
     mark(st.segs.back(), kind);
     st.bias.push_back({n.b(L_RGB), rows_natural(n.NTR, 3 + n.C)});
-    st.bias.push_back({n.b(L_T0), rows_natural(n.NTH, W2)});
+    st.bias.push_back({n.b_t0(h3), rows_natural(n.NTH, W2), fold});
     for (int l = L_T1; l <= L_T2; ++l) {
         st.segs.push_back(seg(n.NTH, W2 / 2, k_natural(W2 / 2, 0), rows_natural(n.NTH, W2), n.w(l), W2));
         mark(st.segs.back(), kind);
@@ -316,13 +329,15 @@
     }
     std::vector<int> rows_fd = concat(rows_emb(4, 1, W), rows_natural(NTW, W));
     if (transient) {
-        st.segs.push_back(seg(NTW + 1, W2 / 2, k_natural(W2 / 2, 0), rows_fd, n.w(L_T0), W + 27, true));
+        st.segs.push_back(seg(NTW + 1, W2 / 2, k_natural(W2 / 2, 0), rows_fd, n.w_t0(x6 == 2), W + 27, true));
         mark(st.segs.back(), x6);
     }
-    st.segs.push_back(seg(NTW + 1, W2 / 2, k_natural(W2 / 2, 0), rows_fd, n.w(L_DIR), W + 27, true));
+    st.segs.push_back(seg(NTW + 1, W2 / 2, k_natural(W2 / 2, 0), rows_fd, n.w_dir(x6 == 2), W + 27, true));
     mark(st.segs.back(), x6);
-    st.segs.push_back(seg(NTW, W / 2, k_natural(W / 2, 0), rows_natural(NTW, W), n.w(L_FINAL), W, true));
-    mark(st.segs.back(), x6);
+    if (!(n.fold && x6 == 2)) {
+        st.segs.push_back(seg(NTW, W / 2, k_natural(W / 2, 0), rows_natural(NTW, W), n.w(L_FINAL), W, true));
+        mark(st.segs.back(), x6);
+    }
     st.segs.push_back(seg(NTW, 1, k_compact(1, 1), rows_natural(NTW, W), n.w(L_SIGMA), W, true));
     for (int l = 7; l >= 0; --l) {
         if (l == 4) {
@@ -344,6 +359,8 @@
 
 static size_t matrix_elems(const Net& n, const float* Wm) {
     if (Wm == n.th_w.data()) return n.th_w.size();
+    if (n.fold && Wm == n.fdt_w.data()) return n.fdt_w.size();
+    if (n.fold && (Wm == n.fd_w.data() || Wm == n.ft_w.data())) return n.fd_w.size();
     if (Wm == n.dt_w.data()) return n.dt_w.size();
     const int W = n.W, W2 = n.W2;
     for (int l = 0; l < 18; ++l) {
@@ -369,9 +386,11 @@
 }
 static void assign_weight_exponents(const Net& n, Stream (&st)[NEFES_N_STREAMS]) {
     const int e_dt = n.transient ? scale_exp(abs_max(n.dt_w.data(), n.dt_w.size())) : 0;
+    const int e_fdt = n.fold ? scale_exp(abs_max(n.fdt_w.data(), n.fdt_w.size())) : 0;
     for (auto& stream : st)
         for (auto& sg : stream.segs) {
             if (!sg.h3 || !sg.W) continue;
+            if (n.fold && (sg.W == n.fdt_w.data() || sg.W == n.fd_w.data() || sg.W == n.ft_w.data())) { sg.wexp = e_fdt; continue; }
             const bool dt = sg.W == n.dt_w.data() || (n.transient && (sg.W == n.w(L_DIR) || sg.W == n.w(L_T0)));
             sg.wexp = dt ? e_dt : scale_exp(abs_max(sg.W, matrix_elems(n, sg.W)));
         }
@@ -386,8 +405,28 @@
     return -1;
 }
 
+static void fold_head(const Net& n, const float* Wh, const float* bh, float* out, float* out_b) {
+    const int W = n.W, W2 = n.W2, K = n.W + 27;
+    const float *Wf = n.w(L_FINAL), *bf = n.b(L_FINAL);
+    std::vector<double> row((size_t)W);
+    for (int r = 0; r < W2; ++r) {
+        for (int c = 0; c < W; ++c) row[c] = 0.0;
+        double bsum = (double)bh[r];
+        for (int k = 0; k < W; ++k) {
+            const double a = (double)Wh[(size_t)r * K + k];
+            const float* wf = Wf + (size_t)k * W;
+            for (int c = 0; c < W; ++c) row[c] += a * (double)wf[c];
+            bsum += a * (double)bf[k];
+        }
+        for (int c = 0; c < W; ++c) out[(size_t)r * K + c] = (float)row[c];
+        for (int c = W; c < K; ++c) out[(size_t)r * K + c] = Wh[(size_t)r * K + c];
+        out_b[r] = (float)bsum;
+    }
+}
+
 bool build(const NefesNetDesc* d, const float* const* tensors, Net& n, Stream (&st)[NEFES_N_STREAMS]) {
     if (!d) return false;
+    if (d->fold_final != 0 && d->fold_final != 1) return false;
     if (d->width != 128 && d->width != 256) return false;
     if (nefes_head_class(d->feat_dim) < 0) return false;
     n.W = d->width; n.W2 = n.W / 2; n.C = d->feat_dim;
@@ -414,6 +453,19 @@
         n.dt_w.assign((size_t)2 * n.W2 * (n.W + 27), 0.f);
         n.th_w.assign((size_t)5 * n.W2, 0.f);
         n.th_b.assign(5, 0.f);
+    }
+    n.fold = d->fold_final != 0;
+    if (n.fold) {
+        if (n.ext && !(n.W == 256 && nefes_head_class(n.C) == 0)) return false;
+        const size_t me = (size_t)n.W2 * (n.W + 27);
+        n.fd_w.assign(me, 0.f); n.ft_w.assign(me, 0.f); n.fdt_w.assign(2 * me, 0.f);
+        n.fd_b.assign(n.W2, 0.f); n.ft_b.assign(n.W2, 0.f);
+        if (tensors) {
+            fold_head(n, n.w(L_DIR), n.b(L_DIR), n.fd_w.data(), n.fd_b.data());
+            if (n.transient) fold_head(n, n.w(L_T0), n.b(L_T0), n.ft_w.data(), n.ft_b.data());
+            memcpy(&n.fdt_w[0], n.fd_w.data(), sizeof(float) * me);
+            memcpy(&n.fdt_w[me], n.ft_w.data(), sizeof(float) * me);
+        }
     }
     static const float* dummy[36] = {nullptr};
     if (!tensors) n.t = dummy;
@@ -538,6 +590,7 @@
                     float m = 0.f;
                     for (int r : bb.ridx)
                         if (r >= 0 && fabsf(bb.b[r]) > m) m = fabsf(bb.b[r]);
+                    if (bb.folded) m = nextafterf(m, INFINITY);
                     memcpy(&word, &m, 4);
                 }
                 if (base) memcpy(base + boff, &word, 4);
@@ -653,6 +706,7 @@
     NefesBlobInfo info;
 };
 static int build_indexed(const NefesNetDesc* desc, Indexed& x, int64_t* tensor_elems_out) {
+    if (desc && desc->fold_final) return NEFES_E_UNSUPPORTED;
     {
         Stream tmp[NEFES_N_STREAMS];
         if (!build(desc, nullptr, x.n, tmp)) return NEFES_E_UNSUPPORTED;
diff --git a/nefes_amd/field.py b/nefes_amd/field.py
--- a/nefes_amd/field.py
+++ b/nefes_amd/field.py
@@ -164,6 +164,8 @@
         self._pk_key = None
         self._pk_gen = None
         self._pk_gen_key = None
+        self._pk_fold = None
+        self._pk_fold_key = None
 
     def _supported(self):
         freq_xyz = self.in_channels_xyz in range(3, 64, 6)
@@ -250,6 +252,7 @@
     def invalidate_packed(self):
         self._pk_key = None
         self._pk_gen_key = None
+        self._pk_fold_key = None
 
     def packed(self) -> ops.PackedField:
         if not self._supported():
@@ -280,11 +283,30 @@
             self._pk_key = key
         return self._pk
 
+    def _field_frozen(self):
+        return not any(p.requires_grad for n, p in self.named_parameters()
+                       if not n.startswith(("fusion_net", "exposure_embedding")))
+
+    def fold_ok(self):
+        return (ops.FOLD_FINAL and ops.SPLIT == "h3" and ops.USE_X6 and not ops.FIELD_GENERIC and self.encode_transient and self._supported()
+                and ops.fold_shape(self.W, self.W_features, L.XYZ_EXTERNAL32 if self.in_channels_xyz == 32 else L.XYZ_FREQ10)
+                and self._field_frozen())
+
+    def packed_folded(self) -> ops.PackedField:
+        names = ops.PackedField.LAYERS_FINE
+        sd = dict(self.named_parameters())
+        prm = [sd[n + s] for n in names for s in (".weight", ".bias")]
+        key = tuple((p.data_ptr(), p._version, str(p.device)) for p in prm)
+        if self._pk_fold is None or key != self._pk_fold_key:
+            dev = prm[0].device if prm[0].is_cuda else torch.device("cuda")
+            self._pk_fold = ops.PackedField(self._kernel_params({n: p.detach() for n, p in sd.items()}), self.W, self.W_features,
+                                            True, dev, L.XYZ_FREQ10, fold_final=True)
+            self._pk_fold_key = key
+        return self._pk_fold
+
     def factored_head_ok(self):
         return (ops.FACTORED_HEAD and not ops.FIELD_GENERIC and self.encode_transient and self.W == 128 and self.in_channels_xyz != 32 and self._supported()
-                and 3 + self.W_features > 3 + self.W // 2 + 1 and ops.SPLIT == "h3"
-                and not any(p.requires_grad for n, p in self.named_parameters()
-                            if not n.startswith(("fusion_net", "exposure_embedding"))))
+                and 3 + self.W_features > 3 + self.W // 2 + 1 and ops.SPLIT == "h3" and self._field_frozen())
 
     def packed_fh(self):
         names = ops.PackedField.LAYERS_FINE
diff --git a/nefes_amd/lib.py b/nefes_amd/lib.py
--- a/nefes_amd/lib.py
+++ b/nefes_amd/lib.py
@@ -8,7 +8,8 @@
 
 
 class NefesNetDesc(C.Structure):
-    _fields_ = [("width", C.c_int32), ("feat_dim", C.c_int32), ("has_transient", C.c_int32), ("xyz_encoding", C.c_int32)]
+    _fields_ = [("width", C.c_int32), ("feat_dim", C.c_int32), ("has_transient", C.c_int32), ("xyz_encoding", C.c_int32),
+                ("fold_final", C.c_int32)]
 
 
 class NefesGenericNetDesc(C.Structure):
@@ -29,7 +30,7 @@
                 ("base_resolution", C.c_int32), ("per_level_scale", C.c_float), ("bound", C.c_float)]
 
 
-ABI_VERSION = 16
+ABI_VERSION = 17
 STREAM_FWD_SIGMA, STREAM_FWD_STATIC, STREAM_FWD_FULL, STREAM_BWD_FULL, STREAM_FWD_SIGMA_X6, STREAM_FWD_FULL_X6, STREAM_BWD_FULL_X6, STREAM_BWD_STATIC = 0, 1, 2, 3, 4, 5, 6, 7
 STREAM_FWD_SIGMA_H3, STREAM_FWD_FULL_H3, STREAM_BWD_FULL_H3, STREAM_FWD_STATIC_H3, STREAM_BWD_STATIC_H3 = 8, 9, 10, 11, 12
 FIELD_SIGMA, FIELD_STATIC, FIELD_FULL = 0, 1, 2
diff --git a/nefes_amd/ops.py b/nefes_amd/ops.py
--- a/nefes_amd/ops.py
+++ b/nefes_amd/ops.py
@@ -225,9 +225,10 @@
     LAYERS_FINE = LAYERS_COARSE + ["transient_encoding.0", "transient_encoding.2", "transient_encoding.4",
                                    "transient_sigma.0", "transient_rgb.0", "transient_beta.0"]
 
-    def __init__(self, state_dict, width, feat_dim, has_transient, device, xyz_encoding=0):
+    def __init__(self, state_dict, width, feat_dim, has_transient, device, xyz_encoding=0, fold_final=False):
         lib = L.load()
-        self.desc = L.NefesNetDesc(int(width), int(feat_dim), 1 if has_transient else 0, int(xyz_encoding))
+        self.desc = L.NefesNetDesc(int(width), int(feat_dim), 1 if has_transient else 0, int(xyz_encoding), 1 if fold_final else 0)
+        self.fold = bool(fold_final)
         self.xyz_encoding = int(xyz_encoding)
         self.width, self.feat_dim, self.has_transient = int(width), int(feat_dim), bool(has_transient)
         info = L.NefesBlobInfo()
@@ -249,6 +250,9 @@
 
     def repack(self, params):
         lib = L.load()
+        if self.fold:
+            raise RuntimeError("nefes_amd: a folded pack (fold_final) holds products of parameters and is not re-packed on the device; "
+                               "trainable networks take NeRFH_NFF.packed()")
         if self._map is None:
             n = self.info.total_bytes // 2
             host_map = torch.zeros(n, dtype=torch.int32)
@@ -341,6 +345,13 @@
     return True if pk.xyz_encoding == L.XYZ_FREQ10 else (pk.width == 256 and cls == 0)
 
 
+FOLD_FINAL = os.environ.get("NEFES_FOLD_FINAL", "1") != "0"
+
+
+def fold_shape(width, feat_dim, xyz_encoding=L.XYZ_FREQ10):
+    return width == 256 and head_class(feat_dim) >= 0 and xyz_encoding == L.XYZ_FREQ10
+
+
 def x6_supported(pk: PackedField, mode, forward=True):
     if mode == L.FIELD_STATIC:
         return static_h3(pk)
@@ -377,8 +388,11 @@
     if not h3 and not canonical_shape(pk):
         raise RuntimeError(f"nefes_amd: {N * S} samples in one launch exceed the fp16 two-part kernels' 32-bit sample index and "
                            f"W={pk.width}, f_dim={pk.feat_dim} has no other instance; render fewer rays per launch")
+    fold = getattr(pk, "fold", False)
+    if fold and not (h3 and mode == L.FIELD_FULL):
+        raise RuntimeError("nefes_amd: a folded pack serves the full pass on the fp16 two-part kernels only")
     fn = L.load().nefes_field_fwd_h3 if h3 else L.load().nefes_field_fwd_x6
-    with _timed(f"field_fwd[{('sigma', 'static', 'full')[mode]},{'h3' if h3 else 'x6'}]"):
+    with _timed(f"field_fwd[{('sigma', 'static', 'full')[mode]},{'h3' if h3 else 'x6'}{',fold' if fold else ''}]"):
         L.check(fn(pk.desc, _chk(pk.blob, "blob", torch.uint8), mode, N, S, _chk(rays_o, "rays_o"),
                                             _chk(rays_d, "rays_d"), _chk(z, "z"), _chk(pts, "pts"), _chk(xyz_enc, "xyz_enc"),
                                             _chk(viewdirs, "viewdirs"),
@@ -417,8 +431,11 @@
     g_vs = torch.empty(N * S, 3, device=dev)
     if USE_X6 and SPLIT != "f32" and x6_supported(pk, L.FIELD_FULL, forward=False):
         h3 = _h3(pk)
+        fold = getattr(pk, "fold", False)
+        if fold and not h3:
+            raise RuntimeError("nefes_amd: a folded pack serves the fp16 two-part kernels only")
         fn = L.load().nefes_field_bwd_h3 if h3 else L.load().nefes_field_bwd_x6
-        with _timed("field_bwd[h3]" if h3 else "field_bwd[x6]"):
+        with _timed(("field_bwd[h3,fold]" if fold else "field_bwd[h3]") if h3 else "field_bwd[x6]"):
             L.check(fn(pk.desc, _chk(pk.blob, "blob", torch.uint8), N, S, _chk(rays_o, "rays_o"),
                                                 _chk(rays_d, "rays_d"), _chk(z, "z"), _chk(pts, "pts"), _chk(viewdirs, "viewdirs"),
                                                 _chk(raw_t, "raw_t"), _chk(g_raw_t, "g_raw_t"), _chk(masks, "masks", torch.int32),
diff --git a/nefes_amd/render.py b/nefes_amd/render.py
--- a/nefes_amd/render.py
+++ b/nefes_amd/render.py
@@ -170,8 +170,12 @@
         if cfg.feat_as_gmap:
             ret["feat_is_gmap"] = True
         return ret
-    pk_f = network_fine.packed_any()
     mode = L.FIELD_FULL if cfg.NeRFW else L.FIELD_STATIC
+    if (mode == L.FIELD_FULL and cfg.xyz_encoder is None and z_f.shape[0] * z_f.shape[1] < (1 << 31) - 256
+            and network_fine.fold_ok()):
+        pk_f = network_fine.packed_folded()
+    else:
+        pk_f = network_fine.packed_any()
     raw_f = field(network_fine, pk_f, mode, z_f)
     if cfg.raw_noise_std > 0. and not cfg.NeRFW:
         raw_f = _with_density_noise(raw_f, C, cfg.raw_noise_std)
```
